# weimengmeng1999/AdapterSIS

Hardware: AMD Instinct MI355X
Metric: training images/sec, ViT-L/14 588^2 adapter fine-tune (higher is better)
Workload: dtype f16; 1 GPU; vit_large/14 frozen + CAViT/CACNN adapters (n_last_blocks=4) + FeatureDecoder, 588x588, batch 12/GPU, reference_exact train.py step (fwd + decoder bwd + all-reduce + SGD), random-init weights; global_batch=12, image_size=588, parallelism=dp1, split_precision_convs=True, split_attn_out=False, precise_level=0, fold_attn_scale=True, fused_qkv=False, dead_cacnn_elided=True, c1_elided=True, ln_fold=True, mx_conv=True, mx_dense=True, conv_halo=True, fuse_cls_up=False, skipped_optimizer_steps=0

## Files before the change

### adaptersis_amd/_lib.py

```python
from __future__ import annotations

import ctypes as C
import os

_HERE = os.path.dirname(os.path.abspath(__file__))
LIB_PATH = os.path.join(_HERE, "lib", "libasis_hip.so")

ASIS_F16, ASIS_BF16, ASIS_F32 = 0, 1, 2
ASIS_EINVAL, ASIS_ELAUNCH = -1, -2
ACT_NONE, ACT_GELU, ACT_RELU, ACT_SILU_MUL, ACT_GELU_GRAD = 0, 1, 2, 3, 4


class AsisError(RuntimeError):
    pass


class GemmDesc(C.Structure):
    _fields_ = [
        ("A", C.c_void_p), ("B", C.c_void_p), ("C", C.c_void_p),
        ("lda", C.c_int64), ("ldb", C.c_int64), ("ldc", C.c_int64),
        ("strideA", C.c_int64), ("strideB", C.c_int64), ("strideC", C.c_int64),
        ("batch", C.c_int32), ("M", C.c_int32), ("N", C.c_int32), ("K", C.c_int32),
        ("bias_n", C.c_void_p), ("bias_m", C.c_void_p), ("scale_n", C.c_void_p), ("res", C.c_void_p),
        ("ldr", C.c_int64), ("strideR", C.c_int64),
        ("act", C.c_int32), ("out_f32", C.c_int32), ("dtype", C.c_int32),
        ("conv", C.c_int32),
        ("B_", C.c_int32), ("H", C.c_int32), ("W", C.c_int32), ("Cin", C.c_int32), ("OH", C.c_int32),
        ("OW", C.c_int32), ("KH", C.c_int32), ("KW", C.c_int32), ("stride", C.c_int32), ("pad", C.c_int32),
        ("stats", C.c_void_p),
        ("A_lo", C.c_void_p), ("B_lo", C.c_void_p),
        ("aux", C.c_void_p), ("ld_aux", C.c_int64),
        ("ksplit", C.c_int32),
        ("mx_amax_a", C.c_void_p), ("mx_amax_b", C.c_void_p),
        ("C_lo", C.c_void_p), ("rowstats", C.c_void_p), ("res16", C.c_void_p), ("res16_lo", C.c_void_p), ("ldr16", C.c_int64),
        ("ln_mr", C.c_void_p), ("ln_cs", C.c_void_p), ("ln_cols", C.c_int32),
    ]


class WgradDesc(C.Structure):
    _fields_ = [
        ("dy", C.c_void_p), ("x", C.c_void_p), ("out", C.c_void_p),
        ("ld_dy", C.c_int64), ("P", C.c_int64),
        ("dtype", C.c_int32), ("Cout", C.c_int32), ("CoP", C.c_int32), ("Cin", C.c_int32),
        ("B_", C.c_int32), ("H", C.c_int32), ("W", C.c_int32), ("OH", C.c_int32), ("OW", C.c_int32),
        ("KH", C.c_int32), ("KW", C.c_int32), ("stride", C.c_int32), ("pad", C.c_int32),
        ("splits", C.c_int32), ("k_per_split", C.c_int64),
    ]


_lib = None


def lib() -> C.CDLL:
    global _lib
    if _lib is not None:
        return _lib
    if not os.path.exists(LIB_PATH):
        raise AsisError(
            f"{LIB_PATH} is missing: build it with `python -m adaptersis_amd.build` "
            "(hipcc --offload-arch=gfx950). adaptersis_amd has no fallback path.")
    _lib = C.CDLL(LIB_PATH)
    _lib.asis_last_error.restype = C.c_char_p
    _declare(_lib)
    return _lib


_vp, _i, _i64, _f, _d = C.c_void_p, C.c_int, C.c_int64, C.c_float, C.c_double
SIGNATURES = {
    "asis_version": [],
    "asis_device_count": [],
    "asis_gemm": [_vp, C.POINTER(GemmDesc)],
    "asis_gemm_tiles_m": [_i],
    "asis_absmax_f32": [_vp, _vp, _i64, _i, _i64, _vp, _i],
    "asis_bn_relu_absmax": [_vp, _vp, _vp, _vp, _i64, _i, _i, _vp],
    "asis_absmax_16": [_vp, _i, _vp, _i64, _i, _i64, _vp],
    "asis_conv3x3_halo_mx_tiles": [_i, _i, _i],
    "asis_conv3x3_halo_mx": [_vp, _i, _vp, _vp, _vp, _vp, _vp, _vp, _vp, _vp, _vp, _i, _i, _i, _i, _i],
    "asis_mx_from_pair": [_vp, _i, _vp, _vp, _i64, _vp, _i64, _i64, _i, _vp, _i],
    "asis_bn_relu_upsample_mx": [_vp, _i, _vp, _vp, _vp, _vp, _vp, _vp, _i, _i, _i, _i, _i],
    "asis_pack_conv_weight_mx": [_vp, _i, _vp, _vp, _i, _i, _i, _i, _i, _i64, _vp],
    "asis_pack_conv_weight_pair": [_vp, _i, _vp, _vp, _vp, _i, _i, _i, _i, _i, _i64, _vp],
    "asis_decoder_input_mx": [_vp, _i, _vp, _i64, _vp, _i64, _vp, _i64, _vp, _vp, _vp, _i, _i, _i, _i, _i, _i],
    "asis_ln_stats_finalize": [_vp, _vp, _i64, _i, _i, _f, _vp],
    "asis_split_stats": [_vp, _i, _vp, _i64, _vp, _vp, _i64, _vp, _i64, _i, _f],
    "asis_gemm_set_option": [C.c_char_p, _i],
    "asis_layernorm": [_vp, _i, _vp, _i64, _vp, _vp, _f, _vp, _i64, _i, _i64, _i],
    "asis_layernorm_mx": [_vp, _i, _vp, _i64, _vp, _vp, _f, _vp, _vp, _i64, _vp, _i64, _i],
    "asis_attention_fwd_seg": [_vp, _i, _vp, _vp, _i64, _vp, _i64, _vp, _i64, _i, _i, _i, _i, _i, _f, _vp],
    "asis_attention_fwd_split": [_vp, _i, _vp, _vp, _i64, _vp, _i64, _vp, _vp, _i64, _i, _i, _i, _i, _i, _f, _vp],
    "asis_attention_fwd_prescaled": [_vp, _i, _vp, _vp, _i64, _vp, _i64, _vp, _vp, _i64, _i, _i, _i, _i, _i, _vp],
    "asis_attention_fwd_qkv": [_vp, _i, _vp, _vp, _vp, _i64, _vp, _vp, _i64, _i, _i, _i, _i, _i, _f, _i, _vp],
    "asis_attention_fwd_qkv_mx": [_vp, _i, _vp, _vp, _vp, _i64, _vp, _vp, _i64, _i, _i, _i, _i, _i, _f, _i, _vp, _vp],
    "asis_attention_fwd_lse": [_vp, _i, _vp, _vp, _i64, _vp, _i64, _vp, _i64, _i, _i, _i, _f, _vp],
    "asis_transpose_tokens": [_vp, _i, _vp, _i64, _vp, _i64, _i, _i, _i],
    "asis_attention_bwd_rows": [_vp, _i, _vp, _vp, _vp, _i64, _vp, _i64, _vp, _i64, _vp, _vp, _vp, _vp, _vp, _i64, _i, _i, _i, _i,
                                _i, _f],
    "asis_msda_bwd": [_vp, _i, _vp, _vp, _i64, _vp, _vp, _vp, _vp, _vp, _vp, _i, _i, _i, _i, _i, _i, _i],
    "asis_msda_vgrad_cap": [_i, _i, _i],
    "asis_msda_value_grad": [_vp, _i, _vp, _i64, _vp, _vp, _vp, _vp, _vp, _vp, _vp, _vp, _vp, _i, _i, _i, _i, _i, _i, _i],
    "asis_msda_sampling_matrix": [_vp, _i, _vp, _i64, _vp, _vp, _vp, _vp, _i64, _i, _i, _i, _i, _i, _i],
    "asis_dwconv_bwd_nblk": [_i64],
    "asis_dwconv_gelu_bwd": [_vp, _i, _vp, _vp, _vp, _vp, _vp, _i, _vp, _vp, _vp, _vp, _i, _i, _i],
    "asis_rowblock_nblk": [_i64],
    "asis_layernorm_bwd": [_vp, _vp, _i64, _vp, _i64, _vp, _f, _vp, _i64, _vp, _i64, _vp, _i64, _i],
    "asis_gelu16": [_vp, _i, _vp, _vp, _vp, _i64],
    "asis_gelu_split": [_vp, _i, _vp, _vp, _vp, _i64],
    "asis_cast_colsum": [_vp, _i, _vp, _i64, _vp, _i64, _f, _vp, _i64, _i],
    "asis_swiglu_bwd": [_vp, _i, _vp, _vp, _vp, _i64, _i],
    "asis_colsum": [_vp, _i, _vp, _i64, _vp, _i64, _i],
    "asis_ls_linear_finish": [_vp, _vp, _vp, _vp, _vp, _vp, _f, _vp, _vp, _vp, _i, _i],
    "asis_attention_fwd": [_vp, _i, _vp, _vp, _i64, _vp, _i64, _vp, _i64, _i, _i, _i, _f],
    "asis_im2col_patch": [_vp, _i, _vp, _i, _i, _i, _i, _vp, _i64],
    "asis_im2col_patch_split": [_vp, _i, _vp, _i, _i, _i, _i, _vp, _vp, _i64],
    "asis_cast_pad": [_vp, _i, _vp, _i64, _vp, _i64, _i64, _i, _f, _i],
    "asis_add_cls_pos": [_vp, _vp, _vp, _vp, _vp, _i, _i, _i],
    "asis_msda_fwd": [_vp, _i, _vp, _vp, _i64, _vp, _vp, _vp, _vp, _i, _i, _i, _i, _i, _i, _i],
    "asis_msda_fwd_split": [_vp, _i, _vp, _vp, _i64, _vp, _vp, _vp, _vp, _vp, _i, _i, _i, _i, _i, _i, _i],
    "asis_dwconv_gelu": [_vp, _i, _vp, _vp, _vp, _vp, _vp, _i, _vp, _i, _i, _i],
    "asis_conv3x3_c3": [_vp, _vp, _vp, _vp, _i, _i, _i, _i, _i, _i],
    "asis_conv3x3_smallcout_fwd": [_vp, _i, _vp, _vp, _vp, _vp, _vp, _i, _i, _i, _i, _i],
    "asis_conv3x3_smallcout_fwd_up": [_vp, _i, _vp, _vp, _vp, _vp, _vp, _vp, _i, _i, _i, _i, _i],
    "asis_conv3x3_smallcout_wgrad_up": [_vp, _i, _vp, _i, _vp, _vp, _vp, _vp, _i, _i, _i, _i, _i, _i],
    "asis_conv3x3_smallcout_dgrad": [_vp, _i, _vp, _vp, _i, _vp, _vp, _i, _i, _i, _i, _i],
    "asis_conv3x3_smallcout_wgrad": [_vp, _i, _vp, _i, _vp, _vp, _i, _i, _i, _i, _i, _i],
    "asis_colstats_nparts": [_i64],
    "asis_colstats": [_vp, _vp, _i64, _i, _vp],
    "asis_reduce_partials": [_vp, _vp, _i, _i, _vp],
    "asis_bn_finalize": [_vp, _vp, _d, _i, _vp, _vp, _f, _f, _vp, _vp, _vp, _vp, _vp, _vp, _vp],
    "asis_bn_eval_affine": [_vp, _vp, _vp, _vp, _vp, _f, _i, _vp, _vp],
    "asis_bn_act": [_vp, _i, _vp, _vp, _vp, _i, _vp, _vp, _i64, _i],
    "asis_bn_act_mx": [_vp, _i, _vp, _vp, _vp, _i, _vp, _vp, _vp, _i64, _i],
    "asis_bn_relu_maxpool": [_vp, _i, _vp, _vp, _vp, _vp, _vp, _i, _i, _i, _i],
    "asis_bn_relu_upsample": [_vp, _i, _vp, _vp, _vp, _vp, _vp, _i, _i, _i, _i, _i],
    "asis_pack_conv_weight": [_vp, _i, _vp, _vp, _i, _i, _i, _i, _i, _i64, _i],
    "asis_decoder_input": [_vp, _i, _vp, _i64, _vp, _i64, _vp, _i64, _vp, _vp, _i, _i, _i, _i, _i, _i],
    "asis_swiglu": [_vp, _i, _vp, _vp, _i64, _i],
    "asis_swiglu_split": [_vp, _i, _vp, _vp, _vp, _i64, _i],
    "asis_copy_channels": [_vp, _vp, _i64, _vp, _i64, _i64, _i64],
    "asis_add_f32": [_vp, _vp, _vp, _vp, _i64, _i, _i64, _i64, _i64],
    "asis_maxpool2_fwd": [_vp, _i, _vp, _vp, _vp, _vp, _vp, _i, _i, _i, _i],
    "asis_maxpool2_bwd": [_vp, _vp, _vp, _vp, _i, _i, _i, _i],
    "asis_cls_l2norm": [_vp, _vp, _vp, _vp, _i, _i, _i, _i],
    "asis_cls_l2norm_bwd": [_vp, _vp, _vp, _vp, _vp, _i, _i, _i, _i],
    "asis_mask_logits_fwd": [_vp, _vp, _vp, _vp, _vp, _f, _vp, _vp, _vp, _i, _i, _i, _i],
    "asis_mask_logits_nblk": [_i, _i],
    "asis_mask_logits_bwd": [_vp, _vp, _vp, _vp, _vp, _vp, _vp, _f, _vp, _vp, _vp, _i, _i, _i, _i],
    "asis_mask_dchat": [_vp, _vp, _vp, _vp, _vp, _i, _i, _i, _i],
    "asis_nearest_add_relu": [_vp, _i, _vp, _vp, _vp, _vp, _vp, _vp, _i, _i, _i, _i, _i, _i],
    "asis_nearest_sum": [_vp, _vp, _vp, _vp, _vp, _i, _i, _i, _i, _i, _i],
    "asis_convt2x2_scatter": [_vp, _i, _vp, _vp, _vp, _i, _i, _i, _i, _i, _i, _i, _i, _i, _i],
    "asis_convt2x2_gather": [_vp, _i, _vp, _vp, _vp, _i, _i, _i, _i, _i, _i, _i, _i, _i, _i],
    "asis_convt2x2_bias_nblk": [_i64],
    "asis_conv1x1_dgrad_small": [_vp, _i, _vp, _vp, _i64, _vp, _vp, _i64, _i, _i],
    "asis_convt2x2_bias_grad": [_vp, _vp, _vp, _i, _i, _i, _i, _i, _i, _i, _i, _i, _i],
    "asis_dice_nblk": [_i, _i],
    "asis_seg_loss_fwd": [_vp, _vp, _vp, _vp, _i, _i, _i, _i, _i, _i, _i, _i, _f, _i, _f, _vp, _vp, _vp, _vp],
    "asis_seg_loss_bwd": [_vp, _vp, _vp, _vp, _vp, _i, _i, _i, _i, _i, _i, _i, _i, _i, _vp],
    "asis_dice_fwd": [_vp, _vp, _vp, _i, _i, _i, _i, _i, _i, _i, _f, _i, _f, _vp, _vp, _vp, _vp],
    "asis_dice_bwd": [_vp, _vp, _vp, _vp, _i, _i, _i, _i, _i, _i, _i, _vp],
    "asis_ce_acc_nblk": [_i64],
    "asis_ce_acc_counts": [_vp, _vp, _vp, _vp, _i, _i, _i, _i, _i, _i, _vp, _vp],
    "asis_ce_acc": [_vp, _vp, _vp, _vp, _i, _i, _i, _i, _i, _i, _vp],
    "asis_resize_bilinear_fwd": [_vp, _vp, _i, _i, _i, _i, _i, _i, _vp],
    "asis_resize_bwd_nblk": [_i64],
    "asis_resize_bilinear_bwd": [_vp, _i, _vp, _i, _i, _i, _i, _i, _i, _i, _vp, _vp, _vp],
    "asis_reduce_rows": [_vp, _vp, _i, _i, _f, _vp],
    "asis_ew_blocks": [_i64],
    "asis_bn_bwd_nblk": [_i64, _i],
    "asis_maxpool_bn_relu_bwd": [_vp, _vp, _vp, _vp, _vp, _vp, _vp, _vp, _vp, _i, _i, _i, _i],
    "asis_dilate2": [_vp, _i, _vp, _vp, _vp, _vp, _i, _i, _i, _i, _i, _i],
    "asis_upsample_bn_relu_bwd": [_vp, _vp, _vp, _vp, _vp, _vp, _vp, _vp, _vp, _i, _i, _i, _i, _i],
    "asis_bn_bwd_apply": [_vp, _i, _vp, _vp, _vp, _vp, _vp, _vp, _vp, _d, _vp, _vp, _vp, _i64, _i],
    "asis_bn_bwd_apply_mx": [_vp, _i, _vp, _vp, _vp, _vp, _vp, _vp, _vp, _d, _vp, _vp, _vp, _vp, _i64, _i],
    "asis_bn_bwd_absmax": [_vp, _vp, _vp, _vp, _vp, _vp, _vp, _vp, _d, _vp, _i64, _i],
    "asis_wgrad_splits": [_i64, _i, _i],
    "asis_wgrad": [_vp, C.POINTER(WgradDesc)],
    "asis_conv3x3_wgrad_halo_nblk": [_i, _i, _i, _i, _i],
    "asis_conv3x3_wgrad_halo": [_vp, _i, _vp, _i64, _vp, _vp, _i, _i, _i, _i, _i, _i],
    "asis_sgd_momentum": [_vp, _vp, _vp, _vp, _i64, _f, _f, _f, _f, _i],
    "asis_augment": [_vp] * 13 + [_i, _i],
    "asis_augment_geo_u8": [_vp] * 12 + [_i, _i],
    "asis_clahe": [_vp] * 13 + [_i, _i, _i],
    "asis_frame_resize": [_vp] * 5 + [_i, _vp, _vp, _i] + [_vp] * 6 + [_i] * 5,
    "asis_predict_mask": [_vp, _vp] + [_i] * 6 + [_vp] * 9,
    "asis_surface_stats": [_vp] * 5 + [_i] * 6 + [_vp, _i] + [_vp] * 6 + [_i],
    "asis_dropout_f32": [_vp, _vp, _vp, _vp, _i64, C.c_uint64, _i, _f, _f, _vp, _i],
    "asis_dropout_t16": [_vp, _i, _vp, _vp, _i64, C.c_uint64, _i, _f, _i],
    "asis_dropout_mask": [_vp, _vp, _i64, C.c_uint64, _i, _f],
    "asis_softmax_dropout_fwd": [_vp, _i, _vp, _vp, _vp, _i64, _i, _i, _f, C.c_uint64, _i, _f],
    "asis_softmax_dropout_bwd": [_vp, _i, _vp, _vp, _vp, _vp, _i64, _i, _i, _f, C.c_uint64, _i, _f],
    "asis_grad_guard": [_vp, _vp, _i64, _vp, _i],
    "asis_sgd_momentum_guarded": [_vp, _vp, _vp, _vp, _i64, _f, _f, _f, _f, _i, _vp, _i],
    "asis_scale_f32": [_vp, _vp, _i64, _f],
    "asis_zero": [_vp, _vp, _i64],
    "asis_grad_pack_bf16": [_vp, _vp, _i64, _vp],
    "asis_grad_unpack_bf16": [_vp, _vp, _i64, _vp],
}


def _declare(l: C.CDLL) -> None:
    for name, argtypes in SIGNATURES.items():
        fn = getattr(l, name)
        fn.argtypes = argtypes
        fn.restype = C.c_int


def check(rc: int, what: str = "") -> None:
    if rc == 0:
        return
    msg = lib().asis_last_error().decode(errors="replace")
    if rc == -1:
        raise ValueError(f"{what}: {msg}" if what else msg)
    raise AsisError(f"{what}: {msg}" if what else msg)
```

### adaptersis_amd/config.py

```python
import os

import torch

operand_dtype = torch.bfloat16 if os.environ.get("ASIS_OPERAND", "f16").lower() in ("bf16", "bfloat16") else torch.float16
loss_scale = float(os.environ.get("ASIS_LOSS_SCALE", 65536.0 if operand_dtype == torch.float16 else 1.0))


def set_operand_dtype(dt: torch.dtype) -> None:
    global operand_dtype
    if dt not in (torch.float16, torch.bfloat16):
        raise ValueError("operand dtype must be float16 or bfloat16")
    operand_dtype = dt

split_conv = os.environ.get("ASIS_SPLIT_CONV", "1") != "0"

precise_attention = os.environ.get("ASIS_PRECISE", "0") not in ("0", "")
fold_attn_scale = os.environ.get("ASIS_FOLD_SCALE", "1") not in ("0", "")
fused_qkv = os.environ.get("ASIS_FUSED_QKV", "0") not in ("0", "")

encoder_stream = os.environ.get("ASIS_ENC_STREAM", "1") not in ("0", "")

vt_stream = os.environ.get("ASIS_VT_STREAM", "1") not in ("0", "")

wgrad_stream = os.environ.get("ASIS_WGRAD_STREAM", "1") not in ("0", "")

unsplit_layers = set(filter(None, os.environ.get("ASIS_UNSPLIT", "").split(",")))

dual_stream = os.environ.get("ASIS_DUAL_STREAM", "1") not in ("0", "")

attn_rows = os.environ.get("ASIS_ATTN_ROWS", "1") != "0"

_so = os.environ.get("ASIS_SPLIT_O", "auto").lower()
split_attn_out_policy = None if _so == "auto" else (_so not in ("0", ""))
split_attn_out = bool(split_attn_out_policy)

_pl = os.environ.get("ASIS_PRECISE_LEVEL", "auto").lower() or "auto"
precise_level_policy = None if _pl == "auto" else int(_pl)
precise_level = int(precise_level_policy or 0)
_pa = os.environ.get("ASIS_PRECISE_ADAPTERS", "auto").lower() or "auto"


def precise_adapters_on() -> bool:
    if _pa != "auto":
        return _pa not in ("0", "")
    return operand_dtype == torch.bfloat16 and precise_level >= 2


_pp = os.environ.get("ASIS_PRECISE_PARTS", "auto").lower() or "auto"
precise_parts_policy = None if _pp == "auto" else frozenset(filter(None, _pp.replace("w12", "fc1").replace("w3", "fc2").split(",")))
precise_parts = precise_parts_policy if precise_parts_policy is not None else frozenset(("qkv", "proj", "fc1", "fc2"))
trunk_streams = int(os.environ.get("ASIS_TRUNK_STREAMS", "2") or 2)

elide_dead_cacnn = os.environ.get("ASIS_ELIDE_DEAD_CACNN", "1") not in ("0", "")
elide_c1 = os.environ.get("ASIS_ELIDE_C1", "1") not in ("0", "")
share_patch_embed = os.environ.get("ASIS_SHARE_PATCH_EMBED", "1") not in ("0", "")

ln_fold = os.environ.get("ASIS_LN_FOLD", "1") not in ("0", "")

_mx = os.environ.get("ASIS_MX_CONV", "1")
mx_conv_all = _mx == "2"
mx_conv = _mx not in ("0", "")


def mx_conv_on() -> bool:
    return mx_conv and (mx_conv_all or operand_dtype == torch.float16)


mx_dense = os.environ.get("ASIS_MX_DENSE", "1") not in ("0", "")


def mx_dense_on() -> bool:
    return mx_dense and operand_dtype == torch.float16
```

### adaptersis_amd/csrc/gemm.hip

```cpp
#include <stdlib.h>

#include "asis_common.h"

namespace {

constexpr int BM = 128, BN = 128, BK = 64, NTHREADS = 256;

template <typename T, bool CONV>
__global__ __launch_bounds__(NTHREADS, 2) void gemm_kernel(const asis_gemm_desc d) {
  typedef typename T16<T>::v8 v8;
  __shared__ __attribute__((aligned(16))) T lds[2 * (BM + BN) * BK];

  const int tid = threadIdx.x;
  const int lane = tid & 63;
  const int wid = tid >> 6;
  const int wr = wid >> 1, wc = wid & 1;

  const int tiles_n = (d.N + BN - 1) / BN;
  const int bid = xcd_remap(blockIdx.x, gridDim.x);
  const int tile_m = bid / tiles_n;
  const int tile_n = bid - tile_m * tiles_n;
  const int m0 = tile_m * BM, n0 = tile_n * BN;
  const int bz = blockIdx.y;

  const T* __restrict__ A = reinterpret_cast<const T*>(d.A) + (int64_t)bz * d.strideA;
  const T* __restrict__ B = reinterpret_cast<const T*>(d.B) + (int64_t)bz * d.strideB;

  const int lrow = tid >> 3;
  const int lchk = tid & 7;
  int64_t a_off[4];
  int a_ih0[4], a_iw0[4];
  bool a_ok[4], b_ok[4];
  int64_t b_off[4];
#pragma unroll
  for (int i = 0; i < 4; ++i) {
    const int m = m0 + lrow + 32 * i;
    a_ok[i] = m < d.M;
    if (CONV) {
      const int mm = a_ok[i] ? m : 0;
      const int ohw = d.OH * d.OW;
      const int b = mm / ohw;
      const int rem = mm - b * ohw;
      const int oh = rem / d.OW;
      const int ow = rem - oh * d.OW;
      a_ih0[i] = oh * d.stride - d.pad;
      a_iw0[i] = ow * d.stride - d.pad;
      a_off[i] = (int64_t)b * d.H * d.W;
    } else {
      a_off[i] = (int64_t)m * d.lda;
      a_ih0[i] = a_iw0[i] = 0;
    }
    const int n = n0 + lrow + 32 * i;
    b_ok[i] = n < d.N;
    b_off[i] = (int64_t)n * d.ldb;
  }

  uint4 ra[4], rb[4];
  auto load_tile = [&](int k0) {
    const int kk = k0 + lchk * 8;
    const bool kok = kk < d.K;
    int kh = 0, kw = 0, ci = kk;
    if (CONV) {
      const int tap = kk / d.Cin;
      ci = kk - tap * d.Cin;
      kh = tap / d.KW;
      kw = tap - kh * d.KW;
    }
#pragma unroll
    for (int i = 0; i < 4; ++i) {
      uint4 v = make_uint4(0, 0, 0, 0);
      if (CONV) {
        const int ih = a_ih0[i] + kh, iw = a_iw0[i] + kw;
        if (a_ok[i] && kok && (unsigned)ih < (unsigned)d.H && (unsigned)iw < (unsigned)d.W)
          v = *reinterpret_cast<const uint4*>(A + (a_off[i] + (int64_t)ih * d.W + iw) * d.Cin + ci);
      } else {
        if (a_ok[i] && kok) v = *reinterpret_cast<const uint4*>(A + a_off[i] + kk);
      }
      ra[i] = v;
      uint4 w = make_uint4(0, 0, 0, 0);
      if (b_ok[i] && kok) w = *reinterpret_cast<const uint4*>(B + b_off[i] + kk);
      rb[i] = w;
    }
  };
  auto store_tile = [&](int buf) {
    T* As = lds + buf * ((BM + BN) * BK);
    T* Bs = As + BM * BK;
#pragma unroll
    for (int i = 0; i < 4; ++i) {
      const int row = lrow + 32 * i;
      const int sw = (lchk ^ ((row >> 1) & 7)) << 3;
      *reinterpret_cast<uint4*>(As + row * BK + sw) = ra[i];
      *reinterpret_cast<uint4*>(Bs + row * BK + sw) = rb[i];
    }
  };

  f32x16 acc[2][2];
#pragma unroll
  for (int i = 0; i < 2; ++i)
#pragma unroll
    for (int j = 0; j < 2; ++j)
#pragma unroll
      for (int r = 0; r < 16; ++r) acc[i][j][r] = 0.f;

  const int nt = (d.K + BK - 1) / BK;
  load_tile(0);
  store_tile(0);
  __syncthreads();

  const int fr = lane & 31, fh = lane >> 5;
  for (int t = 0; t < nt; ++t) {
    const int buf = t & 1;
    if (t + 1 < nt) load_tile((t + 1) * BK);
    const T* As = lds + buf * ((BM + BN) * BK);
    const T* Bs = As + BM * BK;
#pragma unroll
    for (int ks = 0; ks < 4; ++ks) {
      v8 af[2], bf[2];
      const int chunk = 2 * ks + fh;
#pragma unroll
      for (int i = 0; i < 2; ++i) {
        const int row = wr * 64 + i * 32 + fr;
        af[i] = __builtin_bit_cast(v8, *reinterpret_cast<const uint4*>(As + row * BK + ((chunk ^ ((row >> 1) & 7)) << 3)));
        const int col = wc * 64 + i * 32 + fr;
        bf[i] = __builtin_bit_cast(v8, *reinterpret_cast<const uint4*>(Bs + col * BK + ((chunk ^ ((col >> 1) & 7)) << 3)));
      }
#pragma unroll
      for (int i = 0; i < 2; ++i)
#pragma unroll
        for (int j = 0; j < 2; ++j) acc[i][j] = T16<T>::mfma32(af[i], bf[j], acc[i][j]);
    }
    if (t + 1 < nt) store_tile(buf ^ 1);
    __syncthreads();
  }

  const int64_t cbase = (int64_t)bz * d.strideC;
  const float* __restrict__ res = d.res ? d.res + (int64_t)bz * d.strideR : nullptr;
  float csum[2] = {0.f, 0.f}, csq[2] = {0.f, 0.f};
#pragma unroll
  for (int j = 0; j < 2; ++j) {
    const int col = n0 + wc * 64 + j * 32 + fr;
    const bool cok = col < d.N;
    const float bn = (d.bias_n && cok) ? d.bias_n[col] : 0.f;
    const float sc = (d.scale_n && cok) ? d.scale_n[col] : 1.f;
#pragma unroll
    for (int i = 0; i < 2; ++i) {
#pragma unroll
      for (int r = 0; r < 16; ++r) {
        const int row = m0 + wr * 64 + i * 32 + (r & 3) + 8 * (r >> 2) + 4 * fh;
        if (row < d.M && cok) {
          float v = acc[i][j][r] + bn;
          if (d.bias_m) v += d.bias_m[row];
          if (d.act == ASIS_ACT_GELU) v = gelu_erf(v);
          else if (d.act == ASIS_ACT_RELU) v = fmaxf(v, 0.f);
          v *= sc;
          if (res) v += res[(int64_t)row * d.ldr + col];
          if (d.out_f32) reinterpret_cast<float*>(d.C)[cbase + (int64_t)row * d.ldc + col] = v;
          else reinterpret_cast<T*>(d.C)[cbase + (int64_t)row * d.ldc + col] = to_t16<T>(v);
          csum[j] += v;
          csq[j] += v * v;
        }
      }
    }
  }
  if (d.stats) {
    float* red = reinterpret_cast<float*>(lds);
#pragma unroll
    for (int j = 0; j < 2; ++j) {
      float s = csum[j] + __shfl_xor(csum[j], 32, 64);
      float q = csq[j] + __shfl_xor(csq[j], 32, 64);
      if (fh == 0) {
        red[(wr * 2 + 0) * BN + wc * 64 + j * 32 + fr] = s;
        red[(wr * 2 + 1) * BN + wc * 64 + j * 32 + fr] = q;
      }
    }
    __syncthreads();
    if (tid < BN) {
      const int col = n0 + tid;
      if (col < d.N) {
        d.stats[((int64_t)tile_m * 2 + 0) * d.N + col] = red[0 * BN + tid] + red[2 * BN + tid];
        d.stats[((int64_t)tile_m * 2 + 1) * d.N + col] = red[1 * BN + tid] + red[3 * BN + tid];
      }
    }
  }
}

#include "gemm_big.h"
#include "gemm_p8.h"

static int g_gemm_p8 = -1;
static bool ph8_m16_on() { static const int v = [] { const char* e = getenv("ASIS_GEMM_8P_M16"); return e ? atoi(e) : 1; }(); return v != 0; }

template <typename T>
int launch(hipStream_t s, const asis_gemm_desc& d) {
  static const int group_m = [] { const char* e = getenv("ASIS_GEMM_GROUPM"); return e && atoi(e) > 0 ? atoi(e) : 4; }();
  static const int big_mode = [] { const char* e = getenv("ASIS_GEMM_BIG"); return e ? atoi(e) : 1; }();
  const bool vec_ok = (d.N % 4 == 0) && (d.ldc % 4 == 0);
  const bool split = d.A_lo != nullptr || d.B_lo != nullptr;
  if (d.act == ASIS_ACT_GELU_GRAD) {
    const bool ok = big_mode && !d.conv && !split && !d.stats && d.aux && d.K % 32 == 0 && d.M >= 256 && d.N >= 128 && vec_ok &&
                    d.ld_aux % 4 == 0 && d.batch == 1 && (reinterpret_cast<uintptr_t>(d.aux) & 7) == 0 &&
                    (reinterpret_cast<uintptr_t>(d.C) & 15) == 0 && !d.bias_m;
    if (!ok) return ASIS_EINVAL;
  }
  if (d.act == ASIS_ACT_SILU_MUL) {
    auto al16 = [](const void* p) { return (reinterpret_cast<uintptr_t>(p) & 15) == 0; };
    const bool mxs = d.mx_amax_a && d.mx_amax_b && d.A_lo && d.B_lo;
    const bool ok = big_mode && ph8_m16_on() && !d.conv && (mxs || !split) && !d.out_f32 && !d.res && !d.res16 && !d.C_lo && !d.rowstats &&
                    !d.stats && !d.scale_n && !d.bias_m && !d.ln_mr && !d.aux && d.batch == 1 && d.ksplit <= 1 && d.K % 64 == 0 && d.M >= 256 &&
                    d.N >= 256 && d.N % 32 == 0 && d.ldc % 8 == 0 && d.ldc >= d.N / 2 && al16(d.C) && (!d.bias_n || al16(d.bias_n)) &&
                    (int64_t)d.N * d.ldb < (1ll << 31);
    if (!ok) return ASIS_EINVAL;
    dim3 g8(((d.M + 255) / 256) * ((d.N + 255) / 256), 1), block(512);
    if (mxs) hipLaunchKernelGGL((gemm_big_kernel<T, 2, 4, 4, 2, 2, 0, false, true, 64, 1, true, true, 0, true>), g8, block, 0, s, d, group_m);
    else hipLaunchKernelGGL((gemm_big_kernel<T, 2, 4, 4, 2, 2, 0, false, false, 64, 1, true, true>), g8, block, 0, s, d, group_m);
    return 0;
  }
  if (d.ksplit > 1 && !(big_mode && d.conv)) return ASIS_EINVAL;
  {
    if (g_gemm_p8 < 0) { const char* e = getenv("ASIS_GEMM_P8"); g_gemm_p8 = e ? atoi(e) : 1; }
    const int p8 = g_gemm_p8;
    const int64_t p8_tiles = (int64_t)((d.M + 255) / 256) * ((d.N + 255) / 256);
    const int kparts = 1 + (d.A_lo ? 1 : 0) + (d.B_lo ? 1 : 0);
    auto al = [](const void* p, int a) { return (reinterpret_cast<uintptr_t>(p) & (a - 1)) == 0; };
    if (p8 && big_mode && ph8_m16_on() && !d.conv && !d.stats && d.batch == 1 && !d.bias_m && !d.ln_cols && !d.C_lo && !d.rowstats && !d.res16 &&
        !d.mx_amax_a && !d.mx_amax_b &&
        d.ksplit <= 1 && d.K % 64 == 0 &&
        d.M >= 256 && d.N >= 256 && p8_tiles >= (p8 == 2 ? 16 : 256) && d.K >= 128 && (p8 >= 2 || d.K * kparts <= 2048) &&
        (int64_t)d.M * d.lda * 2 < (1ll << 32) && (int64_t)d.N * d.ldb * 2 < (1ll << 32) && d.N % 8 == 0 && d.ldc % 8 == 0 &&
        al(d.C, 16) && (!d.res || (al(d.res, 16) && d.ldr % 4 == 0)) && (!d.bias_n || al(d.bias_n, 16)) && (!d.scale_n || al(d.scale_n, 16)) &&
        (d.act != ASIS_ACT_GELU_GRAD || (d.aux && al(d.aux, 8) && d.ld_aux % 4 == 0))) {
      const int nwg = p8_tiles >= 256 ? 256 : (int)(p8_tiles / 8) * 8;
      if (d.ln_mr) hipLaunchKernelGGL((gemm_p8_kernel<T, 1>), dim3(nwg), dim3(512), 0, s, d, group_m);
      else hipLaunchKernelGGL((gemm_p8_kernel<T, 0>), dim3(nwg), dim3(512), 0, s, d, group_m);
      return 0;
    }
  }
  const bool lnx = d.C_lo || d.rowstats || d.res16 || d.ln_mr;
  if (lnx) {
    static const int ph8x = [] { const char* e = getenv("ASIS_GEMM_8P"); return e ? atoi(e) : 1; }();
    const bool ph8_ok = ph8x && ph8_m16_on() && big_mode && !split && !d.conv && !d.stats && d.K % 64 == 0 && d.M >= 256 && d.N >= 256 &&
                        (ph8x == 2 || d.K >= 2048 || (ph8x == 1 && d.K >= 1024 && (int64_t)((d.M + 255) / 256) * ((d.N + 255) / 256) * d.batch >= 128)) &&
                        d.N % 8 == 0 && d.ldc % 8 == 0 && (!d.res16 || (d.res16_lo && d.ldr16 % 8 == 0 && d.ldr16 >= d.N && asis_aligned16(d.res16) && asis_aligned16(d.res16_lo))) &&
                        (!d.C_lo || !d.out_f32) && (!d.ln_mr || d.ln_cs) &&
                        (!(d.C_lo || d.rowstats || d.res16) ||
                         ((!d.res || (d.ldr % 8 == 0 && asis_aligned16(d.res))) && (!d.C_lo || asis_aligned16(d.C_lo)) && asis_aligned16(d.C) &&
                          (!d.bias_n || asis_aligned16(d.bias_n)) && (!d.scale_n || asis_aligned16(d.scale_n)) && d.batch == 1 && !d.bias_m &&
                          d.act == ASIS_ACT_NONE && !d.ln_mr));
    if (!ph8_ok) return ASIS_EINVAL;
  }
  if (split) {
    const bool ok = big_mode && d.K % BK == 0 && d.M >= 256 && d.N >= 32 && vec_ok && (d.out_f32 || !d.conv) &&
                    (!d.conv || (d.Cin % BK == 0 && d.A_lo && d.B_lo));
    if (!ok) return ASIS_EINVAL;
    const int bm = 256, bn = d.N > 64 ? 128 : 64;
    if (d.ksplit > 1 && (d.batch != 1 || d.stats || (d.KH * d.KW) % d.ksplit != 0 || !d.out_f32 || d.res)) return ASIS_EINVAL;
    dim3 grid(((d.M + bm - 1) / bm) * ((d.N + bn - 1) / bn), d.ksplit > 1 ? d.ksplit : d.batch), block(512);
    if (d.mx_amax_a || d.mx_amax_b) {
      if (!(d.mx_amax_a && d.mx_amax_b && d.A_lo && d.B_lo)) return ASIS_EINVAL;
      if (!d.conv) {
        if (!(d.K % 64 == 0 && d.N >= 256 && d.batch == 1 && d.ksplit <= 1 && !d.stats && (int64_t)d.N * d.ldb < (1ll << 31))) return ASIS_EINVAL;
        dim3 g8(((d.M + 255) / 256) * ((d.N + 255) / 256), 1);
        hipLaunchKernelGGL((gemm_big_kernel<T, 2, 4, 4, 2, 2, 0, false, true, 64, 1, true, true, 0, true>), g8, block, 0, s, d, group_m);
        return 0;
      }
      if ((int64_t)d.B_ * d.H * d.W * d.Cin >= (1ll << 31) || (int64_t)d.N * d.ldb >= (1ll << 31) || d.H >= 65536 || d.W >= 65536) return ASIS_EINVAL;
      static const int mx_ph8 = [] { const char* e = getenv("ASIS_MX_PH8"); return e ? atoi(e) : 1; }();
      if (mx_ph8 && d.N >= 256 && (d.N % 256 == 0 || d.N >= 1024) && d.batch == 1) {
        dim3 g8(((d.M + 255) / 256) * ((d.N + 255) / 256), d.ksplit > 1 ? d.ksplit : 1);
        hipLaunchKernelGGL((gemm_big_kernel<T, 2, 4, 4, 2, 2, 0, true, true, 64, 1, true, true, 0, true>), g8, block, 0, s, d, group_m);
      } else if (bn == 64 && d.ksplit <= 1 && d.M >= 512) {
        dim3 g512(((d.M + 511) / 512) * ((d.N + 63) / 64), 1);
        hipLaunchKernelGGL((gemm_big_kernel<T, 8, 1, 2, 2, 2, 0, true, true, 64, 1, false, true, 0, true>), g512, block, 0, s, d, group_m);
      } else if (bn == 128) {
        hipLaunchKernelGGL((gemm_big_kernel<T, 4, 2, 2, 2, 3, 0, true, true, 64, 1, false, true, 0, true>), grid, block, 0, s, d, group_m);
      } else {
        hipLaunchKernelGGL((gemm_big_kernel<T, 8, 1, 1, 2, 3, 0, true, true, 64, 1, false, true, 0, true>), grid, block, 0, s, d, group_m);
      }
      return 0;
    }
    static const int conv32 = [] { const char* e = getenv("ASIS_CONV_BK32"); return e ? atoi(e) : 0; }();
    static const int t512 = [] { const char* e = getenv("ASIS_CONV_T512"); return e ? atoi(e) : 1; }();
    static const int cm16 = [] { const char* e = getenv("ASIS_CONV_M16"); return e ? atoi(e) : 0; }();
    static const int conv8p = [] { const char* e = getenv("ASIS_CONV_8P"); return e ? atoi(e) : 1; }();
    if (d.conv && conv8p && d.N >= 256 && (d.N % 256 == 0 || d.N >= 1024) && d.batch == 1) {
      dim3 g8(((d.M + 255) / 256) * ((d.N + 255) / 256), d.ksplit > 1 ? d.ksplit : 1);
      hipLaunchKernelGGL((gemm_big_kernel<T, 2, 4, 4, 2, 2, 0, true, true, 64, 1, true, true>), g8, block, 0, s, d, group_m);
      return 0;
    }
    if (d.conv && bn == 64 && t512 && d.ksplit <= 1 && d.M >= 512) {
      dim3 g512(((d.M + 511) / 512) * ((d.N + 63) / 64), 1);
      if (cm16) hipLaunchKernelGGL((gemm_big_kernel<T, 8, 1, 2, 2, 2, 0, true, true, 64, 1, false, true>), g512, block, 0, s, d, group_m);
      else hipLaunchKernelGGL((gemm_big_kernel<T, 8, 1, 2, 2, 2, 0, true, true, 64, 1>), g512, block, 0, s, d, group_m);
      return 0;
    }
    if (d.conv) {
      if (conv32 && bn == 128) hipLaunchKernelGGL((gemm_big_kernel<T, 4, 2, 2, 2, 3, 0, true, true, 32, 4>), grid, block, 0, s, d, group_m);
      else if (bn == 128 && cm16) hipLaunchKernelGGL((gemm_big_kernel<T, 4, 2, 2, 2, 3, 0, true, true, 64, 2, false, true>), grid, block, 0, s, d, group_m);
      else if (bn == 128) hipLaunchKernelGGL((gemm_big_kernel<T, 4, 2, 2, 2, 3, 0, true, true>), grid, block, 0, s, d, group_m);
      else hipLaunchKernelGGL((gemm_big_kernel<T, 8, 1, 1, 2, 3, 0, true, true>), grid, block, 0, s, d, group_m);
    } else {
      if (bn == 128) hipLaunchKernelGGL((gemm_big_kernel<T, 4, 2, 2, 2, 3, 0, false, true>), grid, block, 0, s, d, group_m);
      else hipLaunchKernelGGL((gemm_big_kernel<T, 8, 1, 1, 2, 3, 0, false, true>), grid, block, 0, s, d, group_m);
    }
    return 0;
  }
  static const int m16 = [] { const char* e = getenv("ASIS_GEMM_M16"); return e ? atoi(e) : 1; }();
  static const int ph8 = [] { const char* e = getenv("ASIS_GEMM_8P"); return e ? atoi(e) : 1; }();
  static const int ph8_mink = [] { const char* e = getenv("ASIS_GEMM_8P_MINK"); return e ? atoi(e) : 1024; }();
  if (ph8 && (ph8 == 2 || d.K >= 2048 || (ph8 == 1 && d.K >= ph8_mink && (int64_t)((d.M + 255) / 256) * ((d.N + 255) / 256) * d.batch >= 128)) && big_mode && !d.conv && !d.stats && d.K % 64 == 0 && d.M >= 256 && d.N >= 256) {
    dim3 grid(((d.M + 255) / 256) * ((d.N + 255) / 256), d.batch), block(512);
    static const int ph8_m16 = [] { const char* e = getenv("ASIS_GEMM_8P_M16"); return e ? atoi(e) : 1; }();
    static const int ph8_slab32 = [] { const char* e = getenv("ASIS_GEMM_8P_SLAB32"); return e ? atoi(e) : 0; }();
    const int group_m_f = group_m | (ph8_slab32 ? 0x10000 : 0);
    if (ph8_m16) {
      if (lnx) hipLaunchKernelGGL((gemm_big_kernel<T, 2, 4, 4, 2, 2, 0, false, false, 64, 1, true, true, 1>), grid, block, 0, s, d, group_m);
      else hipLaunchKernelGGL((gemm_big_kernel<T, 2, 4, 4, 2, 2, 0, false, false, 64, 1, true, true>), grid, block, 0, s, d, group_m_f);
      return 0;
    }
    hipLaunchKernelGGL((gemm_big_kernel<T, 2, 4, 4, 2, 2, 0, false, false, 64, 1, true>), grid, block, 0, s, d, group_m);
    return 0;
  }
  if (big_mode && !d.conv && !d.stats && d.K % 32 == 0 && d.M >= 256 && d.N >= 128) {
    const int bm = 256, bn = (big_mode == 2 && d.N >= 2048) ? 256 : 128;
    dim3 grid(((d.M + bm - 1) / bm) * ((d.N + bn - 1) / bn), d.batch), block(512);
    if (big_mode == 2 && bn == 256) hipLaunchKernelGGL((gemm_big_kernel<T, 2, 4, 4, 2, 2>), grid, block, 0, s, d, group_m);
    else if (big_mode >= 2) hipLaunchKernelGGL((gemm_big_kernel<T, 4, 2, 2, 2, 3>), grid, block, 0, s, d, group_m);
    else if (m16) hipLaunchKernelGGL((gemm_big_kernel<T, 4, 2, 2, 2, 3, 0, false, false, 32, 4, false, true>), grid, block, 0, s, d, group_m);
    else hipLaunchKernelGGL((gemm_big_kernel<T, 4, 2, 2, 2, 3, 0, false, false, 32, 4>), grid, block, 0, s, d, group_m);
    return 0;
  }
  if (big_mode && d.conv && d.Cin % BK == 0 && d.M >= 256 && d.N >= 32 && vec_ok && d.out_f32) {
    const int bm = 256, bn = d.N > 64 ? 128 : 64;
    if (d.ksplit > 1 && (d.stats || (d.KH * d.KW) % d.ksplit != 0 || d.res)) return ASIS_EINVAL;
    dim3 grid(((d.M + bm - 1) / bm) * ((d.N + bn - 1) / bn), d.ksplit > 1 ? d.ksplit : 1), block(512);
    static const int conv8p = [] { const char* e = getenv("ASIS_CONV_8P"); return e ? atoi(e) : 1; }();
    if (conv8p && d.N >= 256 && (d.N % 256 == 0 || d.N >= 1024) && d.batch == 1) {
      dim3 g8(((d.M + 255) / 256) * ((d.N + 255) / 256), d.ksplit > 1 ? d.ksplit : 1);
      hipLaunchKernelGGL((gemm_big_kernel<T, 2, 4, 4, 2, 2, 0, true, false, 64, 1, true, true>), g8, block, 0, s, d, group_m);
      return 0;
    }
    if (bn == 128) hipLaunchKernelGGL((gemm_big_kernel<T, 4, 2, 2, 2, 3, 0, true>), grid, block, 0, s, d, group_m);
    else hipLaunchKernelGGL((gemm_big_kernel<T, 8, 1, 1, 2, 3, 0, true>), grid, block, 0, s, d, group_m);
    return 0;
  }
  if (d.ksplit > 1) return ASIS_EINVAL;
  const int tiles_m = (d.M + BM - 1) / BM, tiles_n = (d.N + BN - 1) / BN;
  dim3 grid(tiles_m * tiles_n, d.batch), block(NTHREADS);
  if (d.conv)
    hipLaunchKernelGGL((gemm_kernel<T, true>), grid, block, 0, s, d);
  else
    hipLaunchKernelGGL((gemm_kernel<T, false>), grid, block, 0, s, d);
  return 0;
}

}

extern "C" int asis_gemm_tiles_m(int M) { return (M + BM - 1) / BM; }

extern "C" int asis_gemm_set_option(const char* name, int value) {
  ASIS_REQUIRE(name != nullptr, "asis_gemm_set_option: null name");
  if (strcmp(name, "p8") == 0) { g_gemm_p8 = value; return ASIS_OK; }
  ASIS_FAIL(ASIS_EINVAL, "asis_gemm_set_option: unknown option '%s'", name);
}


extern "C" int asis_gemm(void* stream, const asis_gemm_desc* dp) {
  ASIS_REQUIRE(dp != nullptr, "asis_gemm: null descriptor");
  asis_gemm_desc d = *dp;
  ASIS_REQUIRE(d.A && d.B && d.C, "asis_gemm: null operand pointer");
  ASIS_REQUIRE(d.M > 0 && d.N > 0 && d.K > 0, "asis_gemm: M,N,K must be positive (got %d,%d,%d)", d.M, d.N, d.K);
  ASIS_DT_OK(d.dtype, "asis_gemm");
  ASIS_REQUIRE(d.K % 8 == 0, "asis_gemm: K=%d must be a multiple of 8", d.K);
  ASIS_REQUIRE(d.ldb % 8 == 0 && d.ldb >= d.K, "asis_gemm: ldb=%ld must be a multiple of 8 and >= K", (long)d.ldb);
  ASIS_REQUIRE(asis_aligned16(d.A) && asis_aligned16(d.B), "asis_gemm: A and B must be 16-byte aligned");
  ASIS_REQUIRE(d.strideA % 8 == 0 && d.strideB % 8 == 0, "asis_gemm: batch strides must be multiples of 8");
  ASIS_REQUIRE(d.ldc >= (d.act == ASIS_ACT_SILU_MUL ? d.N / 2 : d.N), "asis_gemm: ldc=%ld < N=%d", (long)d.ldc, d.N);
  ASIS_REQUIRE(d.act >= 0 && d.act <= ASIS_ACT_GELU_GRAD, "asis_gemm: bad act %d", d.act);
  if (d.batch <= 0) d.batch = 1;
  ASIS_REQUIRE(d.batch <= 65535, "asis_gemm: batch %d too large", d.batch);
  if (d.res) ASIS_REQUIRE(d.ldr >= d.N, "asis_gemm: ldr=%ld < N", (long)d.ldr);
  if (d.conv) {
    ASIS_REQUIRE(d.batch == 1, "asis_gemm: conv mode needs batch == 1 (batch is folded into M)");
    ASIS_REQUIRE(d.Cin % 8 == 0 && d.Cin > 0, "asis_gemm: conv Cin=%d must be a multiple of 8", d.Cin);
    ASIS_REQUIRE(d.KH > 0 && d.KW > 0 && d.stride > 0 && d.pad >= 0, "asis_gemm: bad conv geometry");
    ASIS_REQUIRE(d.K == d.KH * d.KW * d.Cin, "asis_gemm: conv K=%d != KH*KW*Cin=%d", d.K, d.KH * d.KW * d.Cin);
    ASIS_REQUIRE(d.OH == (d.H + 2 * d.pad - d.KH) / d.stride + 1 && d.OW == (d.W + 2 * d.pad - d.KW) / d.stride + 1,
                 "asis_gemm: conv output size mismatch");
    ASIS_REQUIRE((int64_t)d.B_ * d.OH * d.OW == d.M, "asis_gemm: conv M=%d != B*OH*OW", d.M);
  } else {
    ASIS_REQUIRE(d.lda % 8 == 0 && d.lda >= d.K, "asis_gemm: lda=%ld must be a multiple of 8 and >= K", (long)d.lda);
  }
  if (d.stats) ASIS_REQUIRE(d.batch == 1, "asis_gemm: stats need batch == 1");
  if (d.res16) ASIS_REQUIRE(d.res16_lo && !d.res && d.ldr16 % 4 == 0 && d.ldr16 >= d.N && (reinterpret_cast<uintptr_t>(d.res16) & 7) == 0 &&
                            (reinterpret_cast<uintptr_t>(d.res16_lo) & 7) == 0, "asis_gemm: res16 needs res16_lo, no fp32 res, ldr16 %% 4 == 0, 8-byte aligned planes");
  if (d.C_lo) ASIS_REQUIRE(!d.out_f32 && (reinterpret_cast<uintptr_t>(d.C_lo) & 7) == 0, "asis_gemm: C_lo is the second plane of a 16-bit output");
  if (d.ln_mr) ASIS_REQUIRE(d.ln_cs && (reinterpret_cast<uintptr_t>(d.ln_mr) & 7) == 0 && asis_aligned16(d.ln_cs), "asis_gemm: ln_mr needs ln_cs (16-byte aligned)");
  if (d.rowstats) ASIS_REQUIRE(d.batch == 1 && (reinterpret_cast<uintptr_t>(d.rowstats) & 7) == 0, "asis_gemm: rowstats need batch == 1");
  if (d.rowstats) ASIS_REQUIRE(d.N % 64 == 0, "asis_gemm: rowstats need N %% 64 == 0 (N = %d)", (int)d.N);
  const int64_t tiles = (int64_t)asis_cdiv(d.M, BM) * asis_cdiv(d.N, BN);
  ASIS_REQUIRE(tiles < (1ll << 31), "asis_gemm: too many tiles");
  hipStream_t s = reinterpret_cast<hipStream_t>(stream);
  ASIS_REQUIRE(!d.conv || (d.A_lo == nullptr) == (d.B_lo == nullptr), "asis_gemm: a split convolution needs both A_lo and B_lo");
  ASIS_REQUIRE((!d.A_lo || asis_aligned16(d.A_lo)) && (!d.B_lo || asis_aligned16(d.B_lo)), "asis_gemm: split halves must be 16-byte aligned");
  int rc = 0;
  if (int bad = asis_dispatch16(d.dtype, "asis_gemm", [&](auto t) { rc = launch<decltype(t)>(s, d); })) return bad;
  if (rc != 0 && d.act == ASIS_ACT_SILU_MUL)
    ASIS_FAIL(ASIS_EINVAL, "asis_gemm: ASIS_ACT_SILU_MUL needs a dense 16-bit-output launch on the 8-phase form (include/asis_hip.h: K %% 64 == 0, "
                           "M >= 256, N >= 256, N %% 32 == 0, ldc %% 8 == 0, plain or MX split operands, bias only)");
  if (rc != 0) ASIS_FAIL(ASIS_EINVAL, "asis_gemm: split-precision operands / ASIS_ACT_GELU_GRAD / ksplit need the large-tile path (K %% 64 "
                                        "== 0 (GELU_GRAD: 32), M >= 256, N >= 32 (128), N and ldc multiples of 4, fp32 output for "
                                        "split; conv: Cin %% 64 == 0)");
  ASIS_CHECK_LAUNCH("asis_gemm");
  return ASIS_OK;
}
```

### adaptersis_amd/csrc/gemm_big.h

```cpp
#pragma once
#include <type_traits>

#include "asis_common.h"

namespace {
__device__ __attribute__((aligned(16))) uint4 g_zero_page[1];

template <typename T, int WM, int WN, int TM, int TN, int NS, int DBG = 0, bool CONV = false, bool SPLIT = false, int BKT = 64,
          int OCC = 2, bool PH8 = false, bool M16 = false, int LNF = 0, bool MXC = false>
__global__ __launch_bounds__(WM * WN * 64, OCC) void gemm_big_kernel(const asis_gemm_desc d, const int GROUP_M_FLAGS) {
  const int GROUP_M = GROUP_M_FLAGS & 0xffff;
  static_assert(!PH8 || (WM == 2 && WN == 4 && TM == 4 && TN == 2 && NS == 2 && BKT == 64),
                "the 8-phase main loop is written for the 256x256x64 tile, 2x4 waves of 128x64");
  static_assert(!MXC || (SPLIT && M16 && BKT == 64 && (CONV || PH8)), "the MX correction pass is built for split operands on 16x16 MFMAs");
  typedef int v4i_ __attribute__((ext_vector_type(4)));
  typedef int v8i_ __attribute__((ext_vector_type(8)));
  auto cat8 = [](auto lo8, auto hi8) -> v8i_ {
    return __builtin_shufflevector(__builtin_bit_cast(v4i_, lo8), __builtin_bit_cast(v4i_, hi8), 0, 1, 2, 3, 4, 5, 6, 7);
  };
  const int mx_sc = MXC ? mx_code<T>(*d.mx_amax_a, *d.mx_amax_b) : 0;
  auto mfma_mx = [](f32x4& acc, v8i_ a, v8i_ b, int sa, int sb) {
    asm volatile("v_mfma_scale_f32_16x16x128_f8f6f4 %0, %1, %2, %0, %3, %4 op_sel_hi:[0,0,0]" : "+v"(acc) : "v"(a), "v"(b), "v"(sa), "v"(sb));
  };
  const int mx_one = 127;
  typedef typename T16<T>::v8 v8;
  constexpr int BM2 = WM * TM * 32, BN2 = WN * TN * 32;
  constexpr int BKB = BKT;
  constexpr int CPR = BKB / 8;
  constexpr int RPI = 64 / CPR;
  constexpr int SWS = (CPR == 8) ? 1 : 2;
  constexpr int STAGE = (BM2 + BN2) * BKB;
  constexpr int NWV = WM * WN;
  constexpr int GA = BM2 / RPI / NWV, GB = BN2 / RPI / NWV;
  constexpr int G = GA + GB;
  __shared__ __attribute__((aligned(16))) T lds[NS * STAGE];

  const int tid = threadIdx.x, lane = tid & 63;
  const int wid = __builtin_amdgcn_readfirstlane(tid >> 6);
  const int wm = wid / WN, wn = wid - wm * WN;
  uint64_t dbg_c0 = 0, dbg_r0 = 0;
  if (DBG & 4) asm volatile("s_memtime %0\n\ts_memrealtime %1\n\ts_waitcnt lgkmcnt(0)" : "=s"(dbg_c0), "=s"(dbg_r0)::"memory");
  const int tiles_n = (d.N + BN2 - 1) / BN2;
  const int bid = xcd_remap(blockIdx.x, gridDim.x);
  const int tiles_m = (d.M + BM2 - 1) / BM2;
  const int band = bid / (GROUP_M * tiles_n);
  const int first_m = band * GROUP_M;
  const int band_m = (tiles_m - first_m) < GROUP_M ? (tiles_m - first_m) : GROUP_M;
  const int in_band = bid - band * GROUP_M * tiles_n;
  const int tile_n = in_band / band_m;
  const int tile_m = first_m + (in_band - tile_n * band_m);
  const int m0 = tile_m * BM2, n0 = tile_n * BN2;
  const int bz = blockIdx.y;
  const T* __restrict__ A = reinterpret_cast<const T*>(d.A) + (int64_t)bz * d.strideA;
  const T* __restrict__ B = reinterpret_cast<const T*>(d.B) + (int64_t)bz * d.strideB;

  const T* asrc[GA];
  const T* bsrc[GB];
  int a_ih0[GA], a_iw0[GA];
  uint32_t a_pix[GA], a_hw[GA], b_off[GB];
  const int lr = lane / CPR, lc = lane % CPR;
  auto swz = [&](int row) -> int { return (M16 && CPR == 4) ? ((-(row >> 2)) & 3) : ((row >> SWS) & (CPR - 1)); };
  auto grp_a = [&](int j) -> int {
    if (PH8) { const int g = wid * 2 + (j & 1); return (g < 8 ? 0 : 128) + (j >> 1) * 64 + (g & 7) * 8; }
    return (wid * GA + j) * RPI;
  };
  auto grp_b = [&](int j) -> int {
    if (PH8) { const int g = wid * 2 + (j & 1); return (g >> 2) * 64 + (j >> 1) * 32 + (g & 3) * 8; }
    return (wid * GB + j) * RPI;
  };
#pragma unroll
  for (int j = 0; j < GA; ++j) {
    const int row = grp_a(j) + lr;
    int gr = m0 + row;
    gr = gr < d.M ? gr : d.M - 1;
    if (CONV) {
      const int ohw = d.OH * d.OW;
      const int b = gr / ohw;
      const int rem = gr - b * ohw;
      const int oh = rem / d.OW, ow = rem - oh * d.OW;
      a_ih0[j] = oh * d.stride - d.pad;
      a_iw0[j] = ow * d.stride - d.pad;
      asrc[j] = A + (int64_t)b * d.H * d.W * d.Cin + ((lc ^ swz(row)) << 3);
      a_pix[j] = (uint32_t)(b * d.H * d.W * d.Cin + ((lc ^ swz(row)) << 3));
      a_hw[j] = ((uint32_t)(oh * d.stride) << 16) | (uint32_t)(ow * d.stride);
    } else {
      a_ih0[j] = a_iw0[j] = 0;
      asrc[j] = A + (int64_t)gr * d.lda + ((lc ^ swz(row)) << 3);
    }
  }
#pragma unroll
  for (int j = 0; j < GB; ++j) {
    const int row = grp_b(j) + lr;
    int gr = n0 + row;
    gr = gr < d.N ? gr : d.N - 1;
    bsrc[j] = B + (int64_t)gr * d.ldb + ((lc ^ swz(row)) << 3);
    b_off[j] = (uint32_t)(gr * (int)d.ldb + ((lc ^ swz(row)) << 3));
  }
  const int64_t a_lo_off = (SPLIT && d.A_lo) ? (reinterpret_cast<const T*>(d.A_lo) - reinterpret_cast<const T*>(d.A)) : 0;
  const int64_t b_lo_off = (SPLIT && d.B_lo) ? (reinterpret_cast<const T*>(d.B_lo) - reinterpret_cast<const T*>(d.B)) : 0;
  const int nparts = !SPLIT ? 1 : (MXC ? 2 : (CONV ? 3 : ((d.A_lo && d.B_lo) ? 3 : 2)));
  auto part_offs = [&](int part, int64_t& aoff, int64_t& boff) {
    aoff = (part == 1 && d.A_lo) ? a_lo_off : 0;
    boff = ((part == 2) || (part == 1 && !d.A_lo)) ? b_lo_off : 0;
  };
  const int ksp = d.ksplit > 1 ? d.ksplit : 1;
  const int nt1 = d.K / ksp / BKB;
  const int kt_base = ksp > 1 ? bz * nt1 : 0;
  const int ntap_part = CONV ? (d.KH * d.KW) / ksp : 1;
  const int tap_base = (CONV && ksp > 1) ? bz * ntap_part : 0;
  typedef __attribute__((address_space(3))) void* lds_ptr;
  typedef const __attribute__((address_space(1))) void* glb_ptr;
  auto issue = [&](int t) {
    T* st = lds + (t % NS) * STAGE;
    int kt = t;
    int64_t aoff = 0, boff = 0;
    int k0;
    if (CONV) {
      int tt = t, part = 0;
      if (SPLIT && MXC) {
        tt = t >> 1;
        part = t & 1;
        aoff = part ? a_lo_off : 0;
        boff = part ? b_lo_off : 0;
      } else if (SPLIT) {
        tt = t / 3;
        part = t - 3 * tt;
        aoff = part == 1 ? a_lo_off : 0;
        boff = part == 2 ? b_lo_off : 0;
      }
      const int c = tt / ntap_part, tl = tt - c * ntap_part;
      k0 = (tap_base + tl) * d.Cin + c * BKB;
    } else {
      if (SPLIT && MXC) {
        kt = t >> 1;
        aoff = (t & 1) ? a_lo_off : 0;
        boff = (t & 1) ? b_lo_off : 0;
      } else if (SPLIT) {
        const int part = t / nt1;
        kt = t - part * nt1;
        part_offs(part, aoff, boff);
      }
      k0 = (kt + kt_base) * BKB;
    }
    if (CONV) {
      const int tap = k0 / d.Cin, ci0 = k0 - tap * d.Cin;
      const int kh = tap / d.KW, kw = tap - kh * d.KW;
#pragma unroll
      for (int j = 0; j < GA; ++j) {
        const T* src;
        if constexpr (MXC) {
          const int ih = (int)(a_hw[j] >> 16) - d.pad + kh, iw = (int)(a_hw[j] & 0xffffu) - d.pad + kw;
          src = ((unsigned)ih < (unsigned)d.H && (unsigned)iw < (unsigned)d.W)
                    ? A + aoff + (a_pix[j] + (uint32_t)((ih * d.W + iw) * d.Cin + ci0))
                    : reinterpret_cast<const T*>(g_zero_page);
        } else {
          const int ih = a_ih0[j] + kh, iw = a_iw0[j] + kw;
          src = ((unsigned)ih < (unsigned)d.H && (unsigned)iw < (unsigned)d.W)
                    ? asrc[j] + aoff + ((int64_t)ih * d.W + iw) * d.Cin + ci0
                    : reinterpret_cast<const T*>(g_zero_page);
        }
        __builtin_amdgcn_global_load_lds((glb_ptr)src, (lds_ptr)(st + grp_a(j) * BKB), 16, 0, 0);
      }
    } else {
#pragma unroll
      for (int j = 0; j < GA; ++j)
        __builtin_amdgcn_global_load_lds((glb_ptr)(asrc[j] + aoff + k0), (lds_ptr)(st + grp_a(j) * BKB), 16, 0, 0);
    }
#pragma unroll
    for (int j = 0; j < GB; ++j) {
      const T* src = MXC ? B + boff + (b_off[j] + (uint32_t)k0) : bsrc[j] + boff + k0;
      __builtin_amdgcn_global_load_lds((glb_ptr)src, (lds_ptr)(st + BM2 * BKB + grp_b(j) * BKB), 16, 0, 0);
    }
  };

  f32x16 acc[M16 ? 1 : TM][M16 ? 1 : TN];
  f32x4 acc16[M16 ? TM * 2 : 1][M16 ? TN * 2 : 1];
  if constexpr (M16) {
#pragma unroll
    for (int i = 0; i < TM * 2; ++i)
#pragma unroll
      for (int j = 0; j < TN * 2; ++j) acc16[i][j] = f32x4{0.f, 0.f, 0.f, 0.f};
  } else {
#pragma unroll
  for (int i = 0; i < TM; ++i)
#pragma unroll
    for (int j = 0; j < TN; ++j)
#pragma unroll
      for (int r = 0; r < 16; ++r) acc[i][j][r] = 0.f;
  }

  const int nt = nparts * nt1;
  const int fr = lane & 31, fh = lane >> 5;
  if constexpr (PH8) {
    int sk0 = kt_base * BKB, s_part = 0, s_kt = 0;
    int64_t s_aoff = 0, s_boff = 0;
    int s_tl = 0, s_c = 0;
    const int kh0 = CONV ? tap_base / d.KW : 0, kw0 = CONV ? tap_base - kh0 * d.KW : 0;
    int s_kh = kh0, s_kw = kw0;
    if (CONV) sk0 = tap_base * d.Cin;
    auto advance_src = [&]() {
      if (CONV) {
        if (SPLIT && MXC) {
          ++s_part;
          s_aoff = s_part == 1 ? a_lo_off : 0;
          s_boff = s_part == 1 ? b_lo_off : 0;
          if (s_part < 2) return;
          s_part = 0;
        } else if (SPLIT) {
          ++s_part;
          s_aoff = s_part == 1 ? a_lo_off : 0;
          s_boff = s_part == 2 ? b_lo_off : 0;
          if (s_part < 3) return;
          s_part = 0;
          s_aoff = s_boff = 0;
        }
        if (++s_tl == ntap_part) {
          s_tl = 0; ++s_c; s_kh = kh0; s_kw = kw0;
        } else if (++s_kw == d.KW) {
          s_kw = 0; ++s_kh;
        }
        sk0 = (tap_base + s_tl) * d.Cin + s_c * BKB;
      } else if constexpr (MXC) {
        ++s_part;
        s_aoff = s_part == 1 ? a_lo_off : 0;
        s_boff = s_part == 1 ? b_lo_off : 0;
        if (s_part < 2) return;
        s_part = 0;
        ++s_kt;
        sk0 = (s_kt + kt_base) * BKB;
      } else {
        if (++s_kt == nt1) {
          s_kt = 0; ++s_part;
          part_offs(s_part, s_aoff, s_boff);
        }
        sk0 = (s_kt + kt_base) * BKB;
      }
    };
    auto dma_a = [&](int t, int j) {
      const T* src;
      if constexpr (CONV && MXC) {
        const int ih = (int)(a_hw[j] >> 16) - d.pad + s_kh, iw = (int)(a_hw[j] & 0xffffu) - d.pad + s_kw;
        src = ((unsigned)ih < (unsigned)d.H && (unsigned)iw < (unsigned)d.W)
                  ? A + s_aoff + (a_pix[j] + (uint32_t)((ih * d.W + iw) * d.Cin + s_c * BKB))
                  : reinterpret_cast<const T*>(g_zero_page);
      } else if (CONV) {
        const int ih = a_ih0[j] + s_kh, iw = a_iw0[j] + s_kw;
        src = ((unsigned)ih < (unsigned)d.H && (unsigned)iw < (unsigned)d.W)
                  ? asrc[j] + s_aoff + ((int64_t)ih * d.W + iw) * d.Cin + s_c * BKB
                  : reinterpret_cast<const T*>(g_zero_page);
      } else {
        src = asrc[j] + s_aoff + sk0;
      }
      __builtin_amdgcn_global_load_lds((glb_ptr)src, (lds_ptr)(lds + (t & 1) * STAGE + grp_a(j) * BKB), 16, 0, 0);
    };
    auto dma_b = [&](int t, int j) {
      const T* src = MXC ? B + s_boff + (b_off[j] + (uint32_t)sk0) : bsrc[j] + s_boff + sk0;
      __builtin_amdgcn_global_load_lds((glb_ptr)src, (lds_ptr)(lds + (t & 1) * STAGE + BM2 * BKB + grp_b(j) * BKB), 16, 0, 0);
    };
#pragma unroll
    for (int j = 0; j < 4; ++j) {
      dma_a(0, j);
      dma_b(0, j);
    }
    advance_src();
    asm volatile("s_waitcnt vmcnt(0)" ::: "memory");
    __builtin_amdgcn_s_barrier();
    if (wm == 1) __builtin_amdgcn_s_barrier();
    v8 af[2][4], b0f[4], b1f[4];
    const int r16 = lane & 15, q16 = lane >> 4;
    auto rd_a = [&](const T* As, int rh) {
      if constexpr (M16) {
#pragma unroll
        for (int t4 = 0; t4 < 4; ++t4) {
          const int row = (wm * TM + rh * 2) * 32 + t4 * 16 + r16;
#pragma unroll
          for (int ks = 0; ks < 2; ++ks)
            af[t4 >> 1][(t4 & 1) * 2 + ks] =
                __builtin_bit_cast(v8, *reinterpret_cast<const uint4*>(As + row * BKB + (((4 * ks + q16) ^ ((row >> 1) & 7)) << 3)));
        }
      } else {
#pragma unroll
      for (int i = 0; i < 2; ++i) {
        const int row = (wm * TM + rh * 2 + i) * 32 + fr;
#pragma unroll
        for (int ks = 0; ks < 4; ++ks)
          af[i][ks] = __builtin_bit_cast(v8, *reinterpret_cast<const uint4*>(As + row * BKB + (((2 * ks + fh) ^ ((row >> 1) & 7)) << 3)));
      }
      }
    };
    auto rd_b = [&](const T* Bs, int ch, v8* bf) {
      if constexpr (M16) {
#pragma unroll
        for (int jj = 0; jj < 2; ++jj) {
          const int col = (wn * TN + ch) * 32 + jj * 16 + r16;
#pragma unroll
          for (int ks = 0; ks < 2; ++ks)
            bf[jj * 2 + ks] = __builtin_bit_cast(v8, *reinterpret_cast<const uint4*>(Bs + col * BKB + (((4 * ks + q16) ^ ((col >> 1) & 7)) << 3)));
        }
      } else {
      const int col = (wn * TN + ch) * 32 + fr;
#pragma unroll
      for (int ks = 0; ks < 4; ++ks)
        bf[ks] = __builtin_bit_cast(v8, *reinterpret_cast<const uint4*>(Bs + col * BKB + (((2 * ks + fh) ^ ((col >> 1) & 7)) << 3)));
      }
    };
    auto mma = [&](int rh, int ch, const v8* bf) {
      asm volatile("s_waitcnt lgkmcnt(0)" ::: "memory");
      __builtin_amdgcn_s_setprio(1);
      if constexpr (M16) {
#pragma unroll
        for (int ks = 0; ks < 2; ++ks)
#pragma unroll
          for (int t4 = 0; t4 < 4; ++t4)
#pragma unroll
            for (int jj = 0; jj < 2; ++jj)
              acc16[rh * 4 + t4][ch * 2 + jj] = T16<T>::mfma16(bf[jj * 2 + ks], af[t4 >> 1][(t4 & 1) * 2 + ks], acc16[rh * 4 + t4][ch * 2 + jj]);
      } else {
#pragma unroll
      for (int ks = 0; ks < 4; ++ks)
#pragma unroll
        for (int i = 0; i < 2; ++i) acc[rh * 2 + i][ch] = T16<T>::mfma32(bf[ks], af[i][ks], acc[rh * 2 + i][ch]);
      }
      __builtin_amdgcn_s_setprio(0);
    };
    v8i_ af8[4], b0f8[2], b1f8[2];
    auto rd_a8 = [&](const T* As, int rh) {
#pragma unroll
      for (int t4 = 0; t4 < 4; ++t4) {
        const int row = (wm * TM + rh * 2) * 32 + t4 * 16 + r16;
        af8[t4] = cat8(*reinterpret_cast<const v4i_*>(As + row * BKB + (((q16) ^ ((row >> 1) & 7)) << 3)),
                       *reinterpret_cast<const v4i_*>(As + row * BKB + (((4 + q16) ^ ((row >> 1) & 7)) << 3)));
      }
    };
    auto rd_b8 = [&](const T* Bs, int ch, v8i_* bf8) {
#pragma unroll
      for (int jj = 0; jj < 2; ++jj) {
        const int col = (wn * TN + ch) * 32 + jj * 16 + r16;
        bf8[jj] = cat8(*reinterpret_cast<const v4i_*>(Bs + col * BKB + (((q16) ^ ((col >> 1) & 7)) << 3)),
                       *reinterpret_cast<const v4i_*>(Bs + col * BKB + (((4 + q16) ^ ((col >> 1) & 7)) << 3)));
      }
    };
    auto half8 = [](v8i_ x, int ks) -> v8 {
      return ks ? __builtin_bit_cast(v8, __builtin_shufflevector(x, x, 4, 5, 6, 7)) : __builtin_bit_cast(v8, __builtin_shufflevector(x, x, 0, 1, 2, 3));
    };
    auto mma8 = [&](int rh, int ch, const v8i_* bf8, auto mx_tag) {
      asm volatile("s_waitcnt lgkmcnt(0)" ::: "memory");
      __builtin_amdgcn_sched_barrier(0);
      __builtin_amdgcn_s_setprio(1);
      if constexpr (decltype(mx_tag)::value) {
#pragma unroll
        for (int t4 = 0; t4 < 4; ++t4)
#pragma unroll
          for (int jj = 0; jj < 2; ++jj) mfma_mx(acc16[rh * 4 + t4][ch * 2 + jj], bf8[jj], af8[t4], mx_sc, mx_one);
      } else {
#pragma unroll
        for (int ks = 0; ks < 2; ++ks)
#pragma unroll
          for (int t4 = 0; t4 < 4; ++t4)
#pragma unroll
            for (int jj = 0; jj < 2; ++jj)
              acc16[rh * 4 + t4][ch * 2 + jj] = T16<T>::mfma16(half8(bf8[jj], ks), half8(af8[t4], ks), acc16[rh * 4 + t4][ch * 2 + jj]);
      }
      __builtin_amdgcn_s_setprio(0);
    };
    auto RA = [&](const T* As, int rh) { if constexpr (MXC) rd_a8(As, rh); else rd_a(As, rh); };
    auto RB = [&](const T* Bs, int ch, int which) {
      if constexpr (MXC) rd_b8(Bs, ch, which ? b1f8 : b0f8); else rd_b(Bs, ch, which ? b1f : b0f);
    };
    auto ktile = [&](int t, auto mx_tag) {
      auto MM = [&](int rh, int ch, int which) {
        if constexpr (MXC) mma8(rh, ch, which ? b1f8 : b0f8, mx_tag); else mma(rh, ch, which ? b1f : b0f);
      };
      const T* As = lds + (t & 1) * STAGE;
      const T* Bs = As + BM2 * BKB;
      const bool more = t + 1 < nt;
      RA(As, 0);
      RB(Bs, 0, 0);
      if (more) { dma_a(t + 1, 0); dma_a(t + 1, 1); asm volatile("s_waitcnt vmcnt(4)" ::: "memory"); }
      else asm volatile("s_waitcnt vmcnt(2)" ::: "memory");
      __builtin_amdgcn_s_barrier();
      MM(0, 0, 0);
      __builtin_amdgcn_s_barrier();
      RB(Bs, 1, 1);
      if (more) { dma_b(t + 1, 0); dma_b(t + 1, 1); asm volatile("s_waitcnt vmcnt(4)" ::: "memory"); }
      else asm volatile("s_waitcnt vmcnt(0)" ::: "memory");
      __builtin_amdgcn_s_barrier();
      MM(0, 1, 1);
      __builtin_amdgcn_s_barrier();
      RA(As, 1);
      if (more) { dma_b(t + 1, 2); dma_b(t + 1, 3); }
      __builtin_amdgcn_s_barrier();
      MM(1, 1, 1);
      __builtin_amdgcn_s_barrier();
      if (more) { dma_a(t + 1, 2); dma_a(t + 1, 3); asm volatile("s_waitcnt vmcnt(4)" ::: "memory"); }
      advance_src();
      __builtin_amdgcn_s_barrier();
      MM(1, 0, 0);
      __builtin_amdgcn_s_barrier();
    };
    if constexpr (MXC) {
      for (int t = 0; t < nt; t += 2) {
        ktile(t, std::false_type{});
        ktile(t + 1, std::true_type{});
      }
    } else {
      for (int t = 0; t < nt; ++t) ktile(t, std::false_type{});
    }
    if (wm == 0) __builtin_amdgcn_s_barrier();
  } else {
#pragma unroll
  for (int s = 0; s < NS - 1; ++s)
    if (s < nt) issue(s);

  for (int t = 0; t < nt; ++t) {
    if (nt - t - 1 >= NS - 2) asm volatile("s_waitcnt vmcnt(%0)" ::"n"((NS - 2) * G) : "memory");
    else asm volatile("s_waitcnt vmcnt(0)" ::: "memory");
    __builtin_amdgcn_s_barrier();
    if (!(DBG & 1) && t + NS - 1 < nt) issue(t + NS - 1);
    const T* As = lds + (t % NS) * STAGE;
    const T* Bs = As + BM2 * BKB;
    if (MXC && (t & 1)) {
      if constexpr (MXC) {
        const int r16 = lane & 15, q16 = lane >> 4;
        v8 af0[TM * 2], af1[TM * 2], bf0[TN * 2], bf1[TN * 2];
#pragma unroll
        for (int i = 0; i < TM * 2; ++i) {
          const int row = (wm * TM * 2 + i) * 16 + r16;
          af0[i] = __builtin_bit_cast(v8, *reinterpret_cast<const uint4*>(As + row * BKB + (((q16) ^ swz(row)) << 3)));
          af1[i] = __builtin_bit_cast(v8, *reinterpret_cast<const uint4*>(As + row * BKB + (((4 + q16) ^ swz(row)) << 3)));
        }
#pragma unroll
        for (int j = 0; j < TN * 2; ++j) {
          const int col = (wn * TN * 2 + j) * 16 + r16;
          bf0[j] = __builtin_bit_cast(v8, *reinterpret_cast<const uint4*>(Bs + col * BKB + (((q16) ^ swz(col)) << 3)));
          bf1[j] = __builtin_bit_cast(v8, *reinterpret_cast<const uint4*>(Bs + col * BKB + (((4 + q16) ^ swz(col)) << 3)));
        }
        asm volatile("s_waitcnt lgkmcnt(0)" ::: "memory");
        __builtin_amdgcn_sched_barrier(0);
#pragma unroll
        for (int i = 0; i < TM * 2; ++i)
#pragma unroll
          for (int j = 0; j < TN * 2; ++j)
            mfma_mx(acc16[i][j], cat8(bf0[j], bf1[j]), cat8(af0[i], af1[i]), mx_sc, mx_one);
      }
    } else if constexpr (M16) {
      const int r16 = lane & 15, q16 = lane >> 4;
#pragma unroll
      for (int ks = 0; ks < BKB / 32; ++ks) {
        v8 af[TM * 2], bf[TN * 2];
#pragma unroll
        for (int i = 0; i < TM * 2; ++i) {
          const int row = (wm * TM * 2 + i) * 16 + r16;
          af[i] = __builtin_bit_cast(v8, *reinterpret_cast<const uint4*>(As + row * BKB + (((4 * ks + q16) ^ swz(row)) << 3)));
        }
#pragma unroll
        for (int j = 0; j < TN * 2; ++j) {
          const int col = (wn * TN * 2 + j) * 16 + r16;
          bf[j] = __builtin_bit_cast(v8, *reinterpret_cast<const uint4*>(Bs + col * BKB + (((4 * ks + q16) ^ swz(col)) << 3)));
        }
#pragma unroll
        for (int i = 0; i < TM * 2; ++i)
#pragma unroll
          for (int j = 0; j < TN * 2; ++j) acc16[i][j] = T16<T>::mfma16(bf[j], af[i], acc16[i][j]);
      }
    } else if (!(DBG & 2)) {
      v8 af[2][TM], bf[2][TN];
      auto fetch = [&](int ks, int slot) {
        const int chunk = 2 * ks + fh;
#pragma unroll
        for (int i = 0; i < TM; ++i) {
          const int row = (wm * TM + i) * 32 + fr;
          af[slot][i] = __builtin_bit_cast(v8, *reinterpret_cast<const uint4*>(As + row * BKB + ((chunk ^ ((row >> SWS) & (CPR - 1))) << 3)));
        }
#pragma unroll
        for (int j = 0; j < TN; ++j) {
          const int col = (wn * TN + j) * 32 + fr;
          bf[slot][j] = __builtin_bit_cast(v8, *reinterpret_cast<const uint4*>(Bs + col * BKB + ((chunk ^ ((col >> SWS) & (CPR - 1))) << 3)));
        }
      };
      constexpr int KS = BKB / 16;
      fetch(0, 0);
#pragma unroll
      for (int ks = 0; ks < KS; ++ks) {
        if (ks < KS - 1) fetch(ks + 1, (ks + 1) & 1);
#pragma unroll
        for (int i = 0; i < TM; ++i)
#pragma unroll
          for (int j = 0; j < TN; ++j)
            acc[i][j] = T16<T>::mfma32(bf[ks & 1][j], af[ks & 1][i], acc[i][j]);
      }
    }
  }
  }

  if (DBG & 4) {
    if (blockIdx.x == gridDim.x / 2 && tid == 0) {
      uint64_t c1, r1;
      asm volatile("s_memtime %0\n\ts_memrealtime %1\n\ts_waitcnt lgkmcnt(0)" : "=s"(c1), "=s"(r1)::"memory");
      uint64_t* o = reinterpret_cast<uint64_t*>(d.C);
      o[0] = c1 - dbg_c0;
      o[1] = r1 - dbg_r0;
    }
    float z = 0.f;
    if constexpr (M16) {
#pragma unroll
      for (int i = 0; i < TM * 2; ++i)
#pragma unroll
        for (int j = 0; j < TN * 2; ++j)
#pragma unroll
          for (int r = 0; r < 4; ++r) z += acc16[i][j][r];
    } else {
#pragma unroll
    for (int i = 0; i < TM; ++i)
#pragma unroll
      for (int j = 0; j < TN; ++j)
#pragma unroll
        for (int r = 0; r < 16; ++r) z += acc[i][j][r];
    }
    if (z == 123.456f) reinterpret_cast<float*>(d.C)[tid] = z;
    return;
  }
  const int64_t cbase = (int64_t)bz * d.strideC;
  const float* __restrict__ res = d.res ? d.res + (int64_t)bz * d.strideR : nullptr;
  const bool vec = ((d.N & 3) == 0) && ((d.ldc & 3) == 0) && ((cbase & 3) == 0) && (!res || (d.ldr & 3) == 0) &&
                   ((reinterpret_cast<uintptr_t>(d.C) & 15) == 0) && (!res || (reinterpret_cast<uintptr_t>(res) & 15) == 0) &&
                   (!d.bias_n || (reinterpret_cast<uintptr_t>(d.bias_n) & 15) == 0) &&
                   (!d.scale_n || (reinterpret_cast<uintptr_t>(d.scale_n) & 15) == 0);
  if constexpr (M16 && PH8) {
    if (vec && !d.out_f32 && !res && !d.res16 && !d.C_lo && !d.rowstats && !d.stats && !d.scale_n && d.act != ASIS_ACT_GELU_GRAD && !(DBG & 8) &&
        (d.N & 7) == 0 && (d.ldc & 7) == 0 && (cbase & 7) == 0 && !(GROUP_M_FLAGS >> 16)) {
      constexpr int SW16 = TN * 32 + 8;
      __syncthreads();
      T* slab16 = reinterpret_cast<T*>(lds) + wid * (32 * SW16);
      const int r16 = lane & 15, q16 = lane >> 4;
      const int rr8 = lane >> 3, c8 = lane & 7;
      const bool ln_on = LNF != 0 && !CONV && d.ln_mr != nullptr, ln_c = ln_on && d.ln_cols != 0;
      const float2* const mrp = reinterpret_cast<const float2*>(d.ln_mr) + (ln_c ? (int64_t)bz * (d.strideB / d.ldb) : 0);
      float4 bj[TN * 2], cj[TN * 2];
      float2 mc[TN * 2][4];
#pragma unroll
      for (int j = 0; j < TN * 2; ++j) {
        const int colj = n0 + (wn * TN * 2 + j) * 16 + 4 * q16;
        bj[j] = (d.bias_n && kt_base == 0 && colj < d.N) ? *reinterpret_cast<const float4*>(d.bias_n + colj) : make_float4(0.f, 0.f, 0.f, 0.f);
        cj[j] = (ln_on && !ln_c && colj < d.N) ? *reinterpret_cast<const float4*>(d.ln_cs + colj) : make_float4(0.f, 0.f, 0.f, 0.f);
#pragma unroll
        for (int e = 0; e < 4; ++e) {
          mc[j][e] = make_float2(0.f, 1.f);
          if (ln_c) mc[j][e] = mrp[colj + e < d.N ? colj + e : d.N - 1];
        }
      }
      const bool sg = d.act == ASIS_ACT_SILU_MUL;
      const int colr = sg ? (n0 >> 1) + wn * TN * 16 + (lane & 3) * 8 : n0 + wn * TN * 32 + c8 * 8;
      const bool cokr = colr < (sg ? (d.N >> 1) : d.N);
      T* const Cw = reinterpret_cast<T*>(d.C) + cbase + colr;
#pragma unroll
      for (int i = 0; i < TM; ++i) {
#pragma unroll
        for (int ii = 0; ii < 2; ++ii) {
          float bm1 = 0.f, nmean = -0.f, rstd = 1.f, csr = 0.f;
          const int rowb = m0 + (wm * TM + i) * 32 + ii * 16 + r16;
          const int rowbc = rowb < d.M ? rowb : d.M - 1;
          if (d.bias_m) bm1 = d.bias_m[rowbc];
          if (ln_on && !ln_c) {
            const float2 mr = mrp[rowbc];
            nmean = -mr.x;
            rstd = mr.y;
          }
          if (ln_c) csr = d.ln_cs[rowbc];
          float4 vg = make_float4(0.f, 0.f, 0.f, 0.f);
#pragma unroll
          for (int j = 0; j < TN * 2; ++j) {
            float4 v;
            if (ln_c) {
              v = make_float4(__builtin_fmaf(__builtin_fmaf(-mc[j][0].x, csr, acc16[2 * i + ii][j][0]), mc[j][0].y, bj[j].x + bm1),
                              __builtin_fmaf(__builtin_fmaf(-mc[j][1].x, csr, acc16[2 * i + ii][j][1]), mc[j][1].y, bj[j].y + bm1),
                              __builtin_fmaf(__builtin_fmaf(-mc[j][2].x, csr, acc16[2 * i + ii][j][2]), mc[j][2].y, bj[j].z + bm1),
                              __builtin_fmaf(__builtin_fmaf(-mc[j][3].x, csr, acc16[2 * i + ii][j][3]), mc[j][3].y, bj[j].w + bm1));
            } else if (ln_on) {
              v = make_float4(__builtin_fmaf(__builtin_fmaf(nmean, cj[j].x, acc16[2 * i + ii][j][0]), rstd, bj[j].x + bm1),
                              __builtin_fmaf(__builtin_fmaf(nmean, cj[j].y, acc16[2 * i + ii][j][1]), rstd, bj[j].y + bm1),
                              __builtin_fmaf(__builtin_fmaf(nmean, cj[j].z, acc16[2 * i + ii][j][2]), rstd, bj[j].z + bm1),
                              __builtin_fmaf(__builtin_fmaf(nmean, cj[j].w, acc16[2 * i + ii][j][3]), rstd, bj[j].w + bm1));
            } else {
              v = make_float4(acc16[2 * i + ii][j][0] + bj[j].x + bm1, acc16[2 * i + ii][j][1] + bj[j].y + bm1,
                              acc16[2 * i + ii][j][2] + bj[j].z + bm1, acc16[2 * i + ii][j][3] + bj[j].w + bm1);
            }
            if (sg) {
              if (j & 1) {
                uint2 pk;
                pk.x = pack2<T>(silu_mul(vg.x, v.x), silu_mul(vg.y, v.y));
                pk.y = pack2<T>(silu_mul(vg.z, v.z), silu_mul(vg.w, v.w));
                *reinterpret_cast<uint2*>(slab16 + (ii * 16 + r16) * SW16 + 16 * (j >> 1) + 4 * q16) = pk;
              } else {
                vg = v;
              }
              continue;
            }
            if (d.act == ASIS_ACT_GELU) gelu_erf4(v.x, v.y, v.z, v.w);
            else if (d.act == ASIS_ACT_RELU) { v.x = fmaxf(v.x, 0.f); v.y = fmaxf(v.y, 0.f); v.z = fmaxf(v.z, 0.f); v.w = fmaxf(v.w, 0.f); }
            uint2 pk;
            pk.x = pack2<T>(v.x, v.y);
            pk.y = pack2<T>(v.z, v.w);
            *reinterpret_cast<uint2*>(slab16 + (ii * 16 + r16) * SW16 + 16 * j + 4 * q16) = pk;
          }
        }
        if (sg) {
#pragma unroll
          for (int p = 0; p < 2; ++p) {
            const int lrow = p * 16 + (lane >> 2);
            const int row = m0 + (wm * TM + i) * 32 + lrow;
            const uint4 w = *reinterpret_cast<const uint4*>(slab16 + lrow * SW16 + (lane & 3) * 8);
            if (row < d.M && cokr) *reinterpret_cast<uint4*>(Cw + (int64_t)row * d.ldc) = w;
          }
          continue;
        }
#pragma unroll
        for (int p = 0; p < 4; ++p) {
          const int lrow = p * 8 + rr8;
          const int row = m0 + (wm * TM + i) * 32 + lrow;
          const uint4 w = *reinterpret_cast<const uint4*>(slab16 + lrow * SW16 + c8 * 8);
          if (row < d.M && cokr) *reinterpret_cast<uint4*>(Cw + (int64_t)row * d.ldc) = w;
        }
      }
      return;
    }
  }
  if constexpr (LNF != 0 && M16 && PH8 && !CONV && !SPLIT) {
    if (d.C_lo || d.rowstats || d.res16) {
      constexpr int SW = TN * 32 + 4;
      __syncthreads();
      float* slab = reinterpret_cast<float*>(lds) + wid * (32 * SW);
      const int rr = lane >> 3, c8 = lane & 7;
      const int col = n0 + wn * TN * 32 + c8 * 8;
      const bool cok = col < d.N;
      const int colc = cok ? col : 0;
      float4 ba = make_float4(0.f, 0.f, 0.f, 0.f), bb = ba, sa = make_float4(1.f, 1.f, 1.f, 1.f), sb = sa;
      if (cok && d.bias_n) { ba = *reinterpret_cast<const float4*>(d.bias_n + col); bb = *reinterpret_cast<const float4*>(d.bias_n + col + 4); }
      if (cok && d.scale_n) { sa = *reinterpret_cast<const float4*>(d.scale_n + col); sb = *reinterpret_cast<const float4*>(d.scale_n + col + 4); }
      const bool res_planes = d.res16 != nullptr;
      const float* const zp = reinterpret_cast<const float*>(g_zero_page);
      const float* const resp = d.res ? d.res + colc : zp;
      const int64_t ldr_e = d.res ? d.ldr : 0;
      const T* const r16h = reinterpret_cast<const T*>(d.res16) + colc;
      const T* const r16l = reinterpret_cast<const T*>(d.res16_lo) + colc;
      T* const Clo = reinterpret_cast<T*>(d.C_lo);
      float* const rstats = d.rowstats;
      const int sgroups = (d.N + 63) >> 6, sgrp = (n0 + wn * TN * 32) >> 6;
#pragma unroll
      for (int i = 0; i < TM; ++i) {
#pragma unroll
        for (int ii = 0; ii < 2; ++ii)
#pragma unroll
          for (int j = 0; j < TN * 2; ++j)
            *reinterpret_cast<float4*>(slab + (ii * 16 + (lane & 15)) * SW + 16 * j + 4 * (lane >> 4)) =
                make_float4(acc16[2 * i + ii][j][0], acc16[2 * i + ii][j][1], acc16[2 * i + ii][j][2], acc16[2 * i + ii][j][3]);
        uint4 ra[4], rb[4];
#pragma unroll
        for (int q = 0; q < 4; ++q) {
          const int row = m0 + (wm * TM + i) * 32 + q * 8 + rr;
          const int rowc = row < d.M ? row : d.M - 1;
          if (res_planes) {
            ra[q] = *reinterpret_cast<const uint4*>(r16h + (int64_t)rowc * d.ldr16);
            rb[q] = *reinterpret_cast<const uint4*>(r16l + (int64_t)rowc * d.ldr16);
          } else {
            ra[q] = *reinterpret_cast<const uint4*>(resp + (int64_t)rowc * ldr_e);
            rb[q] = *reinterpret_cast<const uint4*>(resp + (int64_t)rowc * ldr_e + (d.res ? 4 : 0));
          }
        }
#pragma unroll
        for (int q = 0; q < 4; ++q) {
          const int lrow = q * 8 + rr;
          const int row = m0 + (wm * TM + i) * 32 + lrow;
          float4 va = *reinterpret_cast<const float4*>(slab + lrow * SW + c8 * 8);
          float4 vb = *reinterpret_cast<const float4*>(slab + lrow * SW + c8 * 8 + 4);
          float4 xa, xb;
          if (res_planes) {
            float h[8], l[8];
            unpack2<T>(ra[q].x, h[0], h[1]); unpack2<T>(ra[q].y, h[2], h[3]); unpack2<T>(ra[q].z, h[4], h[5]); unpack2<T>(ra[q].w, h[6], h[7]);
            unpack2<T>(rb[q].x, l[0], l[1]); unpack2<T>(rb[q].y, l[2], l[3]); unpack2<T>(rb[q].z, l[4], l[5]); unpack2<T>(rb[q].w, l[6], l[7]);
            xa = make_float4(h[0] + l[0], h[1] + l[1], h[2] + l[2], h[3] + l[3]);
            xb = make_float4(h[4] + l[4], h[5] + l[5], h[6] + l[6], h[7] + l[7]);
          } else {
            xa = __builtin_bit_cast(float4, ra[q]);
            xb = __builtin_bit_cast(float4, rb[q]);
          }
          float st_s = 0.f, st_q = 0.f;
          if (row < d.M && cok) {
            va.x = (va.x + ba.x) * sa.x + xa.x; va.y = (va.y + ba.y) * sa.y + xa.y; va.z = (va.z + ba.z) * sa.z + xa.z; va.w = (va.w + ba.w) * sa.w + xa.w;
            vb.x = (vb.x + bb.x) * sb.x + xb.x; vb.y = (vb.y + bb.y) * sb.y + xb.y; vb.z = (vb.z + bb.z) * sb.z + xb.z; vb.w = (vb.w + bb.w) * sb.w + xb.w;
            if (d.out_f32) {
              float* const cp = reinterpret_cast<float*>(d.C) + (int64_t)row * d.ldc + col;
              *reinterpret_cast<float4*>(cp) = va;
              *reinterpret_cast<float4*>(cp + 4) = vb;
            } else {
              uint4 ph;
              ph.x = pack2<T>(va.x, va.y); ph.y = pack2<T>(va.z, va.w); ph.z = pack2<T>(vb.x, vb.y); ph.w = pack2<T>(vb.z, vb.w);
              *reinterpret_cast<uint4*>(reinterpret_cast<T*>(d.C) + (int64_t)row * d.ldc + col) = ph;
              if (Clo) {
                uint4 pl;
                pl.x = pack2<T>(lo_part<T>(va.x), lo_part<T>(va.y)); pl.y = pack2<T>(lo_part<T>(va.z), lo_part<T>(va.w));
                pl.z = pack2<T>(lo_part<T>(vb.x), lo_part<T>(vb.y)); pl.w = pack2<T>(lo_part<T>(vb.z), lo_part<T>(vb.w));
                *reinterpret_cast<uint4*>(Clo + (int64_t)row * d.ldc + col) = pl;
              }
            }
            st_s = ((va.x + va.y) + (va.z + va.w)) + ((vb.x + vb.y) + (vb.z + vb.w));
            st_q = ((va.x * va.x + va.y * va.y) + (va.z * va.z + va.w * va.w)) + ((vb.x * vb.x + vb.y * vb.y) + (vb.z * vb.z + vb.w * vb.w));
          }
          if (rstats) {
            st_s = row8_sum(st_s);
            st_q = row8_sum(st_q);
            if (c8 == 0 && row < d.M && sgrp < sgroups) *reinterpret_cast<float2*>(rstats + ((int64_t)row * sgroups + sgrp) * 2) = make_float2(st_s, st_q);
          }
        }
      }
      return;
    }
  }
  if (vec) {
    constexpr int SW = TN * 32 + 4;
    constexpr int LPR = TN * 8;
    constexpr int RPP = 64 / LPR;
    __syncthreads();
    float* slab = reinterpret_cast<float*>(lds) + wid * (32 * SW);
    const int rr = lane / LPR, ch = lane - rr * LPR;
    const int col = n0 + wn * TN * 32 + ch * 4;
    const bool cok = col < d.N;
    float4 b4 = make_float4(0.f, 0.f, 0.f, 0.f), s4 = make_float4(1.f, 1.f, 1.f, 1.f);
    if (cok && d.bias_n && kt_base == 0) b4 = *reinterpret_cast<const float4*>(d.bias_n + col);
    if (cok && d.scale_n) s4 = *reinterpret_cast<const float4*>(d.scale_n + col);
    float4 st_s = make_float4(0.f, 0.f, 0.f, 0.f), st_q = st_s;
    constexpr int NP = 32 / RPP;
    const float* const zp = reinterpret_cast<const float*>(g_zero_page);
    const bool has_aux = d.act == ASIS_ACT_GELU_GRAD;
    const int colc = cok ? col : 0;
    const float* const resp = (res && !(DBG & 32)) ? res + colc : zp;
    const int64_t ldr_e = (res && !(DBG & 32)) ? d.ldr : 0;
    const float* const bmp = d.bias_m ? d.bias_m : zp;
    const int bm_e = d.bias_m ? 1 : 0;
#pragma unroll
    for (int i = 0; i < TM; ++i) {
      if constexpr (M16) {
#pragma unroll
        for (int ii = 0; ii < 2; ++ii)
#pragma unroll
          for (int j = 0; j < TN * 2; ++j)
            *reinterpret_cast<float4*>(slab + (ii * 16 + (lane & 15)) * SW + 16 * j + 4 * (lane >> 4)) =
                make_float4(acc16[2 * i + ii][j][0], acc16[2 * i + ii][j][1], acc16[2 * i + ii][j][2], acc16[2 * i + ii][j][3]);
      } else {
#pragma unroll
      for (int j = 0; j < TN; ++j)
#pragma unroll
        for (int g = 0; g < 4; ++g)
          *reinterpret_cast<float4*>(slab + fr * SW + 32 * j + 8 * g + 4 * fh) =
              make_float4(acc[i][j][4 * g + 0], acc[i][j][4 * g + 1], acc[i][j][4 * g + 2], acc[i][j][4 * g + 3]);
      }
      constexpr int PG = (OCC >= 4 && NP > 4) ? 4 : NP;
#pragma unroll
      for (int p0 = 0; p0 < NP; p0 += PG) {
        float4 r4[PG];
        float bmv[PG];
        uint2 pw[PG];
#pragma unroll
        for (int q = 0; q < PG; ++q) {
          const int row = m0 + (wm * TM + i) * 32 + (p0 + q) * RPP + rr;
          const int rowc = row < d.M ? row : d.M - 1;
          r4[q] = *reinterpret_cast<const float4*>(resp + (int64_t)rowc * ldr_e);
          bmv[q] = bmp[rowc * bm_e];
          pw[q] = make_uint2(0u, 0u);
        }
        if (has_aux) {
#pragma unroll
          for (int q = 0; q < PG; ++q) {
            const int row = m0 + (wm * TM + i) * 32 + (p0 + q) * RPP + rr;
            const int rowc = row < d.M ? row : d.M - 1;
            pw[q] = *reinterpret_cast<const uint2*>(reinterpret_cast<const T*>(d.aux) + (int64_t)rowc * d.ld_aux + colc);
          }
        }
#pragma unroll
        for (int q = 0; q < PG; ++q) {
          const int lrow = (p0 + q) * RPP + rr;
          const int row = m0 + (wm * TM + i) * 32 + lrow;
          float4 v = *reinterpret_cast<const float4*>(slab + lrow * SW + ch * 4);
          if (row < d.M && cok) {
            const float bm1 = bmv[q];
            v.x += b4.x + bm1; v.y += b4.y + bm1; v.z += b4.z + bm1; v.w += b4.w + bm1;
            if (d.act == ASIS_ACT_GELU) gelu_erf4(v.x, v.y, v.z, v.w);
            else if (has_aux) {
              float g0, g1, g2, g3;
              unpack2<T>(pw[q].x, g0, g1);
              unpack2<T>(pw[q].y, g2, g3);
              v.x *= gelu_erf_grad_fast(g0); v.y *= gelu_erf_grad_fast(g1); v.z *= gelu_erf_grad_fast(g2); v.w *= gelu_erf_grad_fast(g3);
            }
            else if (d.act == ASIS_ACT_RELU) { v.x = fmaxf(v.x, 0.f); v.y = fmaxf(v.y, 0.f); v.z = fmaxf(v.z, 0.f); v.w = fmaxf(v.w, 0.f); }
            v.x *= s4.x; v.y *= s4.y; v.z *= s4.z; v.w *= s4.w;
            v.x += r4[q].x; v.y += r4[q].y; v.z += r4[q].z; v.w += r4[q].w;
            if ((DBG & 8) && v.x != 123.456f) {
            } else if (d.out_f32) {
              *reinterpret_cast<float4*>(reinterpret_cast<float*>(d.C) + cbase + (int64_t)row * d.ldc + col) = v;
            } else {
              uint2 pk;
              pk.x = pack2<T>(v.x, v.y);
              pk.y = pack2<T>(v.z, v.w);
              *reinterpret_cast<uint2*>(reinterpret_cast<T*>(d.C) + cbase + (int64_t)row * d.ldc + col) = pk;
            }
            st_s.x += v.x; st_s.y += v.y; st_s.z += v.z; st_s.w += v.w;
            st_q.x += v.x * v.x; st_q.y += v.y * v.y; st_q.z += v.z * v.z; st_q.w += v.w * v.w;
          }
        }
      }
    }
    if (d.stats) {
      for (int o = LPR; o < 64; o <<= 1) {
        st_s.x += __shfl_xor(st_s.x, o, 64); st_s.y += __shfl_xor(st_s.y, o, 64);
        st_s.z += __shfl_xor(st_s.z, o, 64); st_s.w += __shfl_xor(st_s.w, o, 64);
        st_q.x += __shfl_xor(st_q.x, o, 64); st_q.y += __shfl_xor(st_q.y, o, 64);
        st_q.z += __shfl_xor(st_q.z, o, 64); st_q.w += __shfl_xor(st_q.w, o, 64);
      }
      __syncthreads();
      float* red = reinterpret_cast<float*>(lds);
      if (rr == 0) {
        *reinterpret_cast<float4*>(red + (wm * 2 + 0) * BN2 + wn * TN * 32 + ch * 4) = st_s;
        *reinterpret_cast<float4*>(red + (wm * 2 + 1) * BN2 + wn * TN * 32 + ch * 4) = st_q;
      }
      __syncthreads();
      if (tid < BN2 && n0 + tid < d.N) {
        float s = 0.f, q = 0.f;
#pragma unroll
        for (int w2 = 0; w2 < WM; ++w2) {
          s += red[(w2 * 2 + 0) * BN2 + tid];
          q += red[(w2 * 2 + 1) * BN2 + tid];
        }
        const int c = n0 + tid;
        constexpr int RB = BM2 / 128;
        const int64_t r0 = (int64_t)tile_m * RB;
        d.stats[(r0 * 2 + 0) * d.N + c] = s;
        d.stats[(r0 * 2 + 1) * d.N + c] = q;
#pragma unroll
        for (int e = 1; e < RB; ++e)
          if ((r0 + e) * 128 < d.M) {
            d.stats[((r0 + e) * 2 + 0) * d.N + c] = 0.f;
            d.stats[((r0 + e) * 2 + 1) * d.N + c] = 0.f;
          }
      }
    }
    return;
  }
  auto scalar_out = [&](int row, int c, float a, float bmv) {
    float x = a + (d.bias_n ? d.bias_n[c] : 0.f) + bmv;
    if (d.act == ASIS_ACT_GELU) x = gelu_erf(x);
    else if (d.act == ASIS_ACT_RELU) x = fmaxf(x, 0.f);
    if (d.scale_n) x *= d.scale_n[c];
    if (res) x += res[(int64_t)row * d.ldr + c];
    if (d.out_f32) reinterpret_cast<float*>(d.C)[cbase + (int64_t)row * d.ldc + c] = x;
    else reinterpret_cast<T*>(d.C)[cbase + (int64_t)row * d.ldc + c] = to_t16<T>(x);
  };
  if constexpr (M16) {
#pragma unroll
    for (int i = 0; i < TM * 2; ++i) {
      const int row = m0 + (wm * TM * 2 + i) * 16 + (lane & 15);
      if (row >= d.M) continue;
      const float bmv = d.bias_m ? d.bias_m[row] : 0.f;
#pragma unroll
      for (int j = 0; j < TN * 2; ++j)
#pragma unroll
        for (int e = 0; e < 4; ++e) {
          const int c = n0 + (wn * TN * 2 + j) * 16 + 4 * (lane >> 4) + e;
          if (c < d.N) scalar_out(row, c, acc16[i][j][e], bmv);
        }
    }
    return;
  }
#pragma unroll
  for (int i = 0; i < TM; ++i) {
    const int row = m0 + (wm * TM + i) * 32 + fr;
    const bool rok = row < d.M;
    const float bmv = (d.bias_m && rok) ? d.bias_m[row] : 0.f;
#pragma unroll
    for (int j = 0; j < TN; ++j) {
#pragma unroll
      for (int g = 0; g < 4; ++g) {
        const int col = n0 + (wn * TN + j) * 32 + 8 * g + 4 * fh;
        if (!rok || col >= d.N) continue;
#pragma unroll
        for (int e = 0; e < 4; ++e) {
          const int c = col + e;
          if (c < d.N) {
            float x = acc[i][j][4 * g + e] + (d.bias_n ? d.bias_n[c] : 0.f) + bmv;
            if (d.act == ASIS_ACT_GELU) x = gelu_erf(x);
            else if (d.act == ASIS_ACT_RELU) x = fmaxf(x, 0.f);
            if (d.scale_n) x *= d.scale_n[c];
            if (res) x += res[(int64_t)row * d.ldr + c];
            if (d.out_f32) reinterpret_cast<float*>(d.C)[cbase + (int64_t)row * d.ldc + c] = x;
            else reinterpret_cast<T*>(d.C)[cbase + (int64_t)row * d.ldc + c] = to_t16<T>(x);
          }
        }
      }
    }
  }
}


}
```

### adaptersis_amd/dinov2/layers/blocks.py

```python
from __future__ import annotations

import contextlib
import math
import os
from typing import Callable, Optional, Tuple, Union

import torch
from torch import nn

from ... import config, ops


_VT_STREAMS = {}


def _vt_side_stream(device) -> "torch.cuda.Stream":
    key = (device.type, device.index)
    if key not in _VT_STREAMS:
        _VT_STREAMS[key] = torch.cuda.Stream(device=device)
    return _VT_STREAMS[key]


_PRECISE_FOLD_Q = os.environ.get("ASIS_PRECISE_FOLD_Q", "1") not in ("0", "")
_ATTN_MX_OUT = os.environ.get("ASIS_ATTN_MX_OUT", "1") not in ("0", "")
_LS_POW2_REFRESH = 64


def _pack(cache: dict, key: str, param: torch.Tensor, fn: Callable[[torch.Tensor], torch.Tensor]):
    tag = (param.data_ptr(), param._version, getattr(param, "_asis_gen", 0), config.operand_dtype, param.device)
    hit = cache.get(key)
    if hit is None or hit[0] != tag:
        with torch.no_grad():
            cache[key] = (tag, fn(param.detach()))
    return cache[key][1]


class _Packed(nn.Module):
    def __init__(self):
        super().__init__()
        self._cache = {}

    def _w16(self, key: str, param: torch.Tensor, rows: Optional[torch.Tensor] = None) -> torch.Tensor:
        if rows is not None:
            return _pack(self._cache, key + ".sg", param,
                         lambda p: ops.cast_pad(p.reshape(p.shape[0], -1).float()[rows].contiguous(), dtype=config.operand_dtype))
        return _pack(self._cache, key, param,
                     lambda p: ops.cast_pad(p.reshape(p.shape[0], -1).contiguous().float(), dtype=config.operand_dtype))

    def _w16lo(self, key: str, param: torch.Tensor) -> Optional[torch.Tensor]:
        if not config.precise_attention:
            return None
        return _pack(self._cache, key + ".lo", param,
                     lambda p: ops.cast_pad(p.reshape(p.shape[0], -1).contiguous().float(), dtype=config.operand_dtype, part=1))

    def _f32(self, key: str, param: Optional[torch.Tensor]) -> Optional[torch.Tensor]:
        if param is None:
            return None
        return _pack(self._cache, key, param, lambda p: p.float().contiguous())

    def _pack2(self, key: str, w: torch.Tensor, gamma: Optional[torch.Tensor], fn):
        tag = tuple((t.data_ptr(), t._version, getattr(t, "_asis_gen", 0)) for t in (w, gamma) if t is not None) + \
            (config.operand_dtype,)
        hit = self._cache.get(key)
        if hit is None or hit[0] != tag:
            with torch.no_grad():
                self._cache[key] = (tag, fn())
        return self._cache[key][1]

    def _wT16(self, key: str, w: torch.Tensor, gamma: Optional[torch.Tensor] = None, pow2: int = 0) -> torch.Tensor:
        def make():
            wf = w.detach().float()
            if gamma is not None:
                wf = wf * (gamma.detach().float() * (2.0 ** pow2))[:, None]
            return ops.cast_pad(wf.t().contiguous(), dtype=config.operand_dtype)
        return self._pack2(key + (f"@{pow2}" if pow2 else ""), w, gamma, make)

    def _ls_pow2(self, key: str, gamma: Optional[torch.Tensor]) -> int:
        if gamma is None:
            return 0
        tag = (gamma.data_ptr(), gamma.device, config.operand_dtype)
        ver, gen = gamma._version, getattr(gamma, "_asis_gen", 0)
        ent = self._cache.get(key)
        if ent is not None and ent[0] == tag and ent[1][1] == ver:
            st = ent[1]
            if st[2] == gen:
                return st[0]
            if st[3] + 1 < _LS_POW2_REFRESH:
                st[2], st[3] = gen, st[3] + 1
                return st[0]
        m = float(gamma.detach().abs().max())
        k = 0 if not (m > 0.0 and m < float("inf")) else -int(math.floor(math.log2(m)))
        if ent is not None and ent[0] == tag and ent[1][0] != k:
            for stale in [c for c in self._cache if c.endswith(f"@{ent[1][0]}") or c.endswith(f"@{-ent[1][0]}")]:
                del self._cache[stale]
        self._cache[key] = (tag, [k, ver, gen, 0])
        return k

    def _nw_pow2(self, key: str, w: torch.Tensor, pow2: int) -> torch.Tensor:
        if pow2 == 0:
            return self._f32(key, w)
        return _pack(self._cache, f"{key}@{pow2}", w, lambda p: (p.float() * (2.0 ** pow2)).contiguous())

    def _linear_bwd(self, prefix: str, lin: nn.Linear, gamma: Optional[nn.Parameter], gname: Optional[str], dy16, dy_cs,
                    a16, inv_scale: float, grads: Optional[dict]):
        if grads is None:
            return
        N, K = lin.weight.shape
        R = a16.shape[0]
        G = ops.wgrad(dy16.view(1, R, 1, N), a16.view(1, R, 1, K), N, 1, 1, 1, 0, 1.0).view(N, K)
        cs = ops.reduce_rows(dy_cs)
        ops.ls_linear_finish(G, lin.weight.detach() if gamma is not None else None,
                             lin.bias.detach() if lin.bias is not None else None,
                             gamma.detach() if gamma is not None else None, cs, inv_scale, grads[prefix + ".weight"],
                             grads.get(prefix + ".bias") if lin.bias is not None else None,
                             grads[gname] if gamma is not None else None)



def make_2tuple(x):
    if isinstance(x, tuple):
        assert len(x) == 2
        return x
    assert isinstance(x, int)
    return (x, x)


class PatchEmbed(_Packed):

    def __init__(self, img_size=224, patch_size=16, in_chans=3, embed_dim=768, norm_layer=None,
                 flatten_embedding=True):
        super().__init__()
        image_HW, patch_HW = make_2tuple(img_size), make_2tuple(patch_size)
        if in_chans != 3 or patch_HW[0] != patch_HW[1]:
            raise ValueError("PatchEmbed: only 3-channel images and square patches are supported")
        self.img_size, self.patch_size = image_HW, patch_HW
        self.patches_resolution = (image_HW[0] // patch_HW[0], image_HW[1] // patch_HW[1])
        self.num_patches = self.patches_resolution[0] * self.patches_resolution[1]
        self.in_chans, self.embed_dim, self.flatten_embedding = in_chans, embed_dim, flatten_embedding
        self.proj = nn.Conv2d(in_chans, embed_dim, kernel_size=patch_HW, stride=patch_HW)
        self.norm = norm_layer(embed_dim) if norm_layer else nn.Identity()
        if norm_layer:
            raise ValueError("PatchEmbed: norm_layer is not used on this path (vision_transformer.py:104)")

    def tokens(self, x: torch.Tensor, out: Optional[torch.Tensor] = None):
        B, _, H, W = x.shape
        P = self.patch_size[0]
        K = 3 * P * P
        dt = config.operand_dtype
        bias = self._f32("b", self.proj.bias)
        if config.split_conv:
            ldk = (K + 63) // 64 * 64
            flat = lambda p: p.reshape(p.shape[0], -1).contiguous().float()
            w_hi = _pack(self._cache, "w64", self.proj.weight, lambda p: ops.cast_pad(flat(p), ldk, dt))
            w_lo = _pack(self._cache, "w64lo", self.proj.weight, lambda p: ops.cast_pad(flat(p), ldk, dt, part=1))
            a, a_lo = ops.im2col_patch(x.contiguous().float(), P, ldk, dt, split=True)
            if out is None:
                out = torch.empty((a.shape[0], self.embed_dim), device=x.device, dtype=torch.float32)
            ops.gemm_split(a, a_lo, w_hi, w_lo, out=out, bias_n=bias)
        else:
            ldk = (K + 7) // 8 * 8
            w16 = _pack(self._cache, "w", self.proj.weight,
                        lambda p: ops.cast_pad(p.reshape(p.shape[0], -1).contiguous().float(), ldk, dt))
            a = ops.im2col_patch(x.contiguous().float(), P, ldk, dt)
            out = ops.gemm(a, w16, out=out, out_f32=True, bias_n=bias)
        return out.view(B, (H // P) * (W // P), self.embed_dim), a

    def forward(self, x: torch.Tensor) -> torch.Tensor:
        B, _, H, W = x.shape
        P = self.patch_size[0]
        assert H % P == 0, f"Input image height {H} is not a multiple of patch height {P}"
        assert W % P == 0, f"Input image width {W} is not a multiple of patch width: {P}"
        out, _ = self.tokens(x)
        if not self.flatten_embedding:
            out = out.reshape(-1, H // P, W // P, self.embed_dim)
        return out


class LayerScale(nn.Module):

    def __init__(self, dim: int, init_values: Union[float, torch.Tensor] = 1e-5, inplace: bool = False):
        super().__init__()
        self.inplace = inplace
        self.gamma = nn.Parameter(init_values * torch.ones(dim))


class Attention(_Packed):

    def __init__(self, dim, num_heads=8, qkv_bias=False, proj_bias=True, attn_drop=0.0, proj_drop=0.0):
        super().__init__()
        if dim % num_heads or dim // num_heads != 64:
            raise ValueError("attention kernel supports head dim 64 (every DINOv2 arch): "
                             f"got dim={dim}, heads={num_heads}")
        if attn_drop or proj_drop:
            raise ValueError("dropout is 0 on the AdapterSIS path (models/__init__.py:14-29)")
        self.num_heads = num_heads
        self.scale = (dim // num_heads) ** -0.5
        self.qkv = nn.Linear(dim, dim * 3, bias=qkv_bias)
        self.proj = nn.Linear(dim, dim, bias=proj_bias)

    def _qkv_folded(self):
        c = self.scale * 1.4426950408889634
        D = self.qkv.weight.shape[1]

        def scaled(p):
            w = p.reshape(p.shape[0], -1).float().clone()
            w[:D] *= c
            return w.contiguous()
        w = _pack(self._cache, "qkv.fold", self.qkv.weight, lambda p: ops.cast_pad(scaled(p), dtype=config.operand_dtype))
        wlo = None
        if config.precise_attention:
            wlo = _pack(self._cache, "qkv.fold.lo", self.qkv.weight,
                        lambda p: ops.cast_pad(scaled(p), dtype=config.operand_dtype, part=1))
        bias = None
        if self.qkv.bias is not None:
            bias = _pack(self._cache, "qkv_b.fold", self.qkv.bias, lambda p: scaled(p).reshape(-1))
        return w, bias, wlo

    def _qkv_ln_folded(self, norm: nn.LayerNorm):
        c = self.scale * 1.4426950408889634 if config.fold_attn_scale else 1.0
        D = self.qkv.weight.shape[1]
        ps = [p for p in (self.qkv.weight, self.qkv.bias, norm.weight, norm.bias) if p is not None]
        tag = tuple((t.data_ptr(), t._version, getattr(t, "_asis_gen", 0)) for t in ps) + (config.operand_dtype, c)
        hit = self._cache.get("qkv.lnfold")
        if hit is None or hit[0] != tag:
            with torch.no_grad():
                w = self.qkv.weight.detach().float().clone()
                w[:D] *= c
                b = self.qkv.bias.detach().float().clone() if self.qkv.bias is not None else torch.zeros(3 * D, device=w.device)
                b[:D] *= c
                b = b + w @ norm.bias.detach().float()
                w16 = ops.cast_pad((w * norm.weight.detach().float()[None, :]).contiguous(), dtype=config.operand_dtype)
                self._cache["qkv.lnfold"] = (tag, (w16, b.contiguous(), w16.float().sum(1).contiguous()))
        return self._cache["qkv.lnfold"][1]

    def attend(self, xn: torch.Tensor, B: int, N: int) -> torch.Tensor:
        return self.attend_rows(xn, [(B, N)])[0]

    def attend_rows(self, xn: torch.Tensor, segs, ln=None):
        D = xn.shape[1]
        if ln is not None:
            norm, mr = ln
            w, bias, cs = self._qkv_ln_folded(norm)
            scale = None if config.fold_attn_scale else self.scale
            o = torch.empty((xn.shape[0], D), device=xn.device, dtype=xn.dtype)
            o_lo = torch.empty_like(o) if config.split_attn_out else None
            one_launch = len(segs) == 2
            ldv_all = (max(n for _, n in segs) + 63) // 64 * 64
            vt_all = torch.empty((sum(b for b, _ in segs), D, ldv_all), device=xn.device, dtype=xn.dtype)
            spare = xn.untyped_storage().nbytes() // xn.element_size() - (xn.storage_offset() + xn.shape[0] * D)
            side = None
            if one_launch and config.vt_stream:
                main = torch.cuda.current_stream()
                side = _vt_side_stream(xn.device)
                side.wait_stream(main)
            else:
                qk = ops.gemm(xn, w[: 2 * D], bias_n=bias[: 2 * D], ln=(mr, cs[: 2 * D], False))
            r0 = b0 = 0
            for B, N in segs:
                r1 = r0 + B * N
                vt = vt_all[b0:b0 + B]
                N4 = (N + 7) // 8 * 8
                if spare < (N4 - N) * D:
                    raise ValueError("attend_rows(ln=...): the hi plane needs 8 spare rows behind it")
                with (torch.cuda.stream(side) if side is not None else contextlib.nullcontext()):
                    ops.gemm(w[2 * D:], xn[r0:r1].as_strided((B, N4, D), (N * D, D, 1)),
                             out=vt.as_strided((B, D, N4), (D * ldv_all, ldv_all, 1)), bias_m=bias[2 * D:], ln=(mr[r0:], cs[2 * D:], True))
                if not one_launch:
                    ops.attention_fwd(qk[r0:r1, :D], qk[r0:r1, D:], vt, B, self.num_heads, N, scale, out=o[r0:r1],
                                      out_lo=None if o_lo is None else o_lo[r0:r1])
                r0, b0 = r1, b0 + B
            if side is not None:
                qk = ops.gemm(xn, w[: 2 * D], bias_n=bias[: 2 * D], ln=(mr, cs[: 2 * D], False))
                main.wait_stream(side)
                mr.record_stream(side)
            if one_launch:
                (B1, N1), (B2, N2) = segs
                ops.attention_fwd_seg(qk[:, :D], qk[:, D:], vt_all, B1, N1, B2, N2, self.num_heads, scale, out=o, out_lo=o_lo)
            if r0 != xn.shape[0]:
                raise ValueError("attend_rows: segments do not cover the rows")
            return o, o_lo
        if config.fold_attn_scale:
            w, bias, wlo = self._qkv_folded()
            scale = None
        else:
            w = self._w16("qkv", self.qkv.weight)
            bias = self._f32("qkv_b", self.qkv.bias)
            wlo = self._w16lo("qkv", self.qkv.weight)
            scale = self.scale
        o = torch.empty((xn.shape[0], D), device=xn.device, dtype=xn.dtype)
        o_lo = torch.empty_like(o) if config.split_attn_out else None
        if config.fused_qkv and len(segs) <= 2:
            if sum(b * n for b, n in segs) != xn.shape[0]:
                raise ValueError("attend_rows: segments do not cover the rows")
            qkv = ops.gemm(xn, w, bias_n=bias, b_lo=wlo)
            ops.attention_fwd_qkv(qkv, list(segs), self.num_heads, scale, o, out_lo=o_lo)
            return o, o_lo
        one_launch = len(segs) == 2
        ldv_all = (max(n for _, n in segs) + 63) // 64 * 64
        vt_all = torch.empty((sum(b for b, _ in segs), D, ldv_all), device=xn.device, dtype=xn.dtype) if one_launch else None
        spare = xn.untyped_storage().nbytes() // xn.element_size() - (xn.storage_offset() + xn.shape[0] * D)
        side = None
        if one_launch and config.vt_stream and xn.is_cuda:
            main = torch.cuda.current_stream()
            side = _vt_side_stream(xn.device)
            side.wait_stream(main)
        else:
            qk = ops.gemm(xn, w[: 2 * D], bias_n=None if bias is None else bias[: 2 * D], b_lo=None if wlo is None else wlo[: 2 * D])
        r0 = b0 = 0
        for B, N in segs:
            r1 = r0 + B * N
            ldvt = ldv_all if one_launch else (N + 63) // 64 * 64
            vt = vt_all[b0:b0 + B] if one_launch else torch.empty((B, D, ldvt), device=xn.device, dtype=xn.dtype)
            N4 = (N + 3) // 4 * 4 if spare >= 4 * D else N
            with (torch.cuda.stream(side) if side is not None else contextlib.nullcontext()):
                ops.gemm(w[2 * D:], xn[r0:r1].as_strided((B, N4, D), (N * D, D, 1)),
                         out=vt.as_strided((B, D, N4), (D * ldvt, ldvt, 1)), bias_m=None if bias is None else bias[2 * D:],
                         a_lo=None if wlo is None else wlo[2 * D:])
            if not one_launch:
                ops.attention_fwd(qk[r0:r1, :D], qk[r0:r1, D:], vt, B, self.num_heads, N, scale, out=o[r0:r1],
                                  out_lo=None if o_lo is None else o_lo[r0:r1])
            r0, b0 = r1, b0 + B
        if side is not None:
            qk = ops.gemm(xn, w[: 2 * D], bias_n=None if bias is None else bias[: 2 * D], b_lo=None if wlo is None else wlo[: 2 * D])
            main.wait_stream(side)
        if one_launch:
            (B1, N1), (B2, N2) = segs
            ops.attention_fwd_seg(qk[:, :D], qk[:, D:], vt_all, B1, N1, B2, N2, self.num_heads, scale, out=o, out_lo=o_lo)
        if r0 != xn.shape[0]:
            raise ValueError("attend_rows: segments do not cover the rows")
        return o, o_lo

    def forward(self, x: torch.Tensor) -> torch.Tensor:
        raise RuntimeError("Attention is driven by Block.forward (LayerNorm / LayerScale / residual are fused around it)")


class MemEffAttention(Attention):
    """`attention.py:72-89`: same maths as ``Attention``; here both are the fused flash kernel."""


class Mlp(_Packed):

    def __init__(self, in_features, hidden_features=None, out_features=None, act_layer=nn.GELU, drop=0.0, bias=True):
        super().__init__()
        out_features = out_features or in_features
        hidden_features = hidden_features or in_features
        self.fc1 = nn.Linear(in_features, hidden_features, bias=bias)
        self.fc2 = nn.Linear(hidden_features, out_features, bias=bias)


class SwiGLUFFN(_Packed):

    def __init__(self, in_features, hidden_features=None, out_features=None, act_layer=None, drop=0.0, bias=True):
        super().__init__()
        out_features = out_features or in_features
        hidden_features = hidden_features or in_features
        self.w12 = nn.Linear(in_features, 2 * hidden_features, bias=bias)
        self.w3 = nn.Linear(hidden_features, out_features, bias=bias)

    def sg_rows(self) -> torch.Tensor:
        return _pack(self._cache, "w12.sgrows", self.w12.weight, lambda p: ops.swiglu_rows(p.shape[0] // 2, p.device))

    def sg_bias(self) -> Optional[torch.Tensor]:
        if self.w12.bias is None:
            return None
        rows = self.sg_rows()
        return _pack(self._cache, "w12_b.sg", self.w12.bias, lambda p: p.float()[rows].contiguous())


class SwiGLUFFNFused(SwiGLUFFN):

    def __init__(self, in_features, hidden_features=None, out_features=None, act_layer=None, drop=0.0, bias=True):
        out_features = out_features or in_features
        hidden_features = hidden_features or in_features
        hidden_features = (int(hidden_features * 2 / 3) + 7) // 8 * 8
        super().__init__(in_features, hidden_features, out_features, bias=bias)


class Block(_Packed):

    def __init__(self, dim, num_heads, mlp_ratio=4.0, qkv_bias=False, proj_bias=True, ffn_bias=True, drop=0.0,
                 attn_drop=0.0, init_values=None, drop_path=0.0, act_layer=nn.GELU, norm_layer=nn.LayerNorm,
                 attn_class=Attention, ffn_layer=Mlp):
        super().__init__()
        if drop_path or drop:
            raise ValueError("stochastic depth / dropout are 0 on the AdapterSIS path")
        self.norm1 = norm_layer(dim)
        self.attn = attn_class(dim, num_heads=num_heads, qkv_bias=qkv_bias, proj_bias=proj_bias)
        self.ls1 = LayerScale(dim, init_values=init_values) if init_values else nn.Identity()
        self.norm2 = norm_layer(dim)
        self.mlp = ffn_layer(in_features=dim, hidden_features=int(dim * mlp_ratio), act_layer=act_layer, bias=ffn_bias)
        self.ls2 = LayerScale(dim, init_values=init_values) if init_values else nn.Identity()
        self.sample_drop_ratio = drop_path

    def forward(self, x: torch.Tensor) -> torch.Tensor:
        B, N, D = x.shape
        x2 = x.reshape(B * N, D)
        if x2.dtype != torch.float32 or not x2.is_contiguous():
            x2 = x2.float().contiguous()
        return self.forward_rows(x2, [(B, N)]).view(B, N, D)

    def _w16lo_any(self, owner, key: str, w: torch.Tensor, rows: Optional[torch.Tensor] = None):
        sel = (lambda t: t) if rows is None else (lambda t: t[rows])
        return _pack(owner._cache, key + (".sg" if rows is not None else "") + ".lo_any", w,
                     lambda p: ops.cast_pad(sel(p.reshape(p.shape[0], -1).float()).contiguous(), dtype=config.operand_dtype, part=1))

    def _w16mx_any(self, owner, key: str, w: torch.Tensor, rows: Optional[torch.Tensor] = None):
        return _pack(owner._cache, key + (".sg" if rows is not None else "") + ".mx_any", w,
                     lambda p: ops.mx_from_pair(owner._w16(key, w, rows), self._w16lo_any(owner, key, w, rows), wside=True))

    def _mx_ok(self, owner, key: str, lin: nn.Linear, M: int) -> bool:
        N, K = lin.weight.shape
        return config.mx_dense_on() and K % 64 == 0 and N >= 256 and M >= 256 and N * K < (1 << 31)

    def _split_lin(self, owner, key: str, lin: nn.Linear, a_hi, a_lo, a_mx=None, rows=None, **kw):
        w = owner._w16(key, lin.weight, rows)
        if self._mx_ok(owner, key, lin, a_hi.shape[0]):
            a_pl, amax_a = a_mx if a_mx is not None else ops.mx_from_pair(a_hi, a_lo)
            w_mx, amax_w = self._w16mx_any(owner, key, lin.weight, rows)
            return ops.gemm(a_hi, w, a_lo=a_pl, b_lo=w_mx, mx=(amax_a, amax_w), **kw)
        return ops.gemm(a_hi, w, a_lo=a_lo, b_lo=self._w16lo_any(owner, key, lin.weight, rows), **kw)

    def _ln_split(self, key: str, norm: nn.LayerNorm, x2: torch.Tensor, mx: bool):
        dt = config.operand_dtype
        w, b = self._f32(key + "w", norm.weight), self._f32(key + "b", norm.bias)
        if mx:
            amax = _pack(self._cache, key + ".amax", norm.weight,
                         lambda p: ((x2.shape[1] - 1) ** 0.5 * p.float().abs().max() + norm.bias.detach().float().abs().max()).reshape(1).contiguous())
            hi, pl = ops.layernorm_mx(x2, w, b, norm.eps, dt, amax)
            return hi, None, (pl, amax)
        xn32 = ops.layernorm(x2, w, b, norm.eps, torch.float32)
        D = x2.shape[1]
        return ops.cast_pad(xn32, D, dt), ops.cast_pad(xn32, D, dt, part=1), None

    def _forward_rows_precise(self, x2: torch.Tensor, segs) -> torch.Tensor:
        D = x2.shape[1]
        R = x2.shape[0]
        dt = config.operand_dtype
        a, m = self.attn, self.mlp
        g1 = self._f32("g1", self.ls1.gamma) if isinstance(self.ls1, LayerScale) else None
        g2 = self._f32("g2", self.ls2.gamma) if isinstance(self.ls2, LayerScale) else None
        parts = config.precise_parts
        n1w, n1b = self._f32("n1w", self.norm1.weight), self._f32("n1b", self.norm1.bias)
        fold_q = config.fold_attn_scale and "qkv" not in parts and _PRECISE_FOLD_Q
        if "qkv" in parts:
            xn, xn_lo, xn_mx = self._ln_split("n1", self.norm1, x2, self._mx_ok(a, "qkv", a.qkv, R))
            qkv = self._split_lin(a, "qkv", a.qkv, xn, xn_lo, xn_mx, bias_n=a._f32("qkv_b", a.qkv.bias))
        elif fold_q:
            qw, qb, _ = a._qkv_folded()
            qkv = ops.gemm(ops.layernorm(x2, n1w, n1b, self.norm1.eps, dt), qw, bias_n=qb)
        else:
            qkv = ops.gemm(ops.layernorm(x2, n1w, n1b, self.norm1.eps, dt), a._w16("qkv", a.qkv.weight), bias_n=a._f32("qkv_b", a.qkv.bias))
        o = torch.empty((R, D), device=x2.device, dtype=dt)
        o_lo = torch.empty_like(o) if "proj" in parts else None
        if sum(B * N for B, N in segs) != R:
            raise ValueError("forward_rows: segments do not cover the rows")
        o_mx = None
        if fold_q and len(segs) <= 2:
            if o_lo is not None and _ATTN_MX_OUT and self._mx_ok(a, "proj", a.proj, R):
                o_mx = ops.absmax16(qkv[:, 2 * D:3 * D])
            ops.attention_fwd_qkv(qkv, list(segs), a.num_heads, None, o, out_lo=o_lo, mx_amax=o_mx)
        else:
            r0 = 0
            for B, N in segs:
                r1 = r0 + B * N
                vt = ops.transpose_tokens(qkv[r0:r1, 2 * D:], B, N)
                ops.attention_fwd(qkv[r0:r1, :D], qkv[r0:r1, D:2 * D], vt, B, a.num_heads, N, None if fold_q else a.scale,
                                  out=o[r0:r1], out_lo=None if o_lo is None else o_lo[r0:r1])
                r0 = r1
        pkw = dict(out_f32=True, bias_n=a._f32("proj_b", a.proj.bias), scale_n=g1, res=x2)
        if o_mx is not None:
            x1 = self._split_lin(a, "proj", a.proj, o, None, a_mx=(o_lo, o_mx), **pkw)
        else:
            x1 = self._split_lin(a, "proj", a.proj, o, o_lo, **pkw) if o_lo is not None else ops.gemm(o, a._w16("proj", a.proj.weight), **pkw)
        n2w, n2b = self._f32("n2w", self.norm2.weight), self._f32("n2b", self.norm2.bias)
        lin_in, k_in = (m.fc1, "fc1") if isinstance(m, Mlp) else (m.w12, "w12")
        lin_out, k_out = (m.fc2, "fc2") if isinstance(m, Mlp) else (m.w3, "w3")
        ikw = dict(out_f32=True, bias_n=m._f32(k_in + "_b", lin_in.bias))
        split_out = "fc2" in parts
        mx_in = "fc1" in parts and self._mx_ok(m, k_in, lin_in, R)
        sg = (not isinstance(m, Mlp)) and not split_out and \
            ops.swiglu_fused_ok(R, lin_in.out_features // 2, lin_in.in_features, "fc1" in parts, mx_in)
        ge = isinstance(m, Mlp) and not split_out
        if sg:
            rows = m.sg_rows()
            ikw = dict(bias_n=m.sg_bias(), act=ops.ACT_SILU_MUL, rows=rows)
        elif ge:
            ikw = dict(bias_n=m._f32(k_in + "_b", lin_in.bias), act=ops.ACT_GELU)
        if "fc1" in parts:
            xn2, xn2_lo, xn2_mx = self._ln_split("n2", self.norm2, x1, mx_in)
            hpre = self._split_lin(m, k_in, lin_in, xn2, xn2_lo, xn2_mx, **ikw)
        else:
            rows = ikw.pop("rows", None)
            hpre = ops.gemm(ops.layernorm(x1, n2w, n2b, self.norm2.eps, dt), m._w16(k_in, lin_in.weight, rows), **ikw)
        if sg or ge:
            h, h_lo = hpre, None
        elif isinstance(m, Mlp):
            h, h_lo = ops.gelu_split(hpre, dt, split=split_out)
        else:
            h, h_lo = ops.swiglu(hpre, dt, split=True) if split_out else (ops.swiglu(hpre, dt), None)
        okw = dict(out_f32=True, bias_n=m._f32(k_out + "_b", lin_out.bias), scale_n=g2, res=x1)
        if split_out:
            return self._split_lin(m, k_out, lin_out, h, h_lo, **okw)
        return ops.gemm(h, m._w16(k_out, lin_out.weight), **okw)

    def _lin_ln_folded(self, key: str, lin: nn.Linear, norm: nn.LayerNorm):
        ps = [p for p in (lin.weight, lin.bias, norm.weight, norm.bias) if p is not None]
        tag = tuple((t.data_ptr(), t._version, getattr(t, "_asis_gen", 0)) for t in ps) + (config.operand_dtype,)
        hit = self._cache.get(key)
        if hit is None or hit[0] != tag:
            with torch.no_grad():
                w = lin.weight.detach().float()
                b = (lin.bias.detach().float() if lin.bias is not None else torch.zeros(w.shape[0], device=w.device)) + w @ norm.bias.detach().float()
                w16 = ops.cast_pad((w * norm.weight.detach().float()[None, :]).contiguous(), dtype=config.operand_dtype)
                self._cache[key] = (tag, (w16, b.contiguous(), w16.float().sum(1).contiguous()))
        return self._cache[key][1]

    def fold_ok(self, R: int, segs) -> bool:
        if not (config.ln_fold and config.operand_dtype == torch.float16 and config.precise_level < 2 and not config.precise_attention
                and not config.fused_qkv and isinstance(self.mlp, Mlp) and isinstance(self.ls1, LayerScale)
                and isinstance(self.ls2, LayerScale) and isinstance(self.norm1, nn.LayerNorm) and isinstance(self.norm2, nn.LayerNorm)):
            return False
        D, Hd = self.attn.qkv.weight.shape[1], self.mlp.fc1.weight.shape[0]
        if config.split_attn_out:
            return False
        ok = ops.ln_fold_supported(R, 2 * D, D) and ops.ln_fold_supported(R, D, D, producer=True)
        ok = ok and ops.ln_fold_supported(R, Hd, D) and ops.ln_fold_supported(R, D, Hd, producer=True)
        return ok and all(ops.ln_fold_supported(D, (N + 7) // 8 * 8, D, batch=B) for B, N in segs) and D % 64 == 0

    def forward_rows_fold(self, xin, segs, planes_out: bool):
        dt = config.operand_dtype
        a, m = self.attn, self.mlp
        g1, g2 = self._f32("g1", self.ls1.gamma), self._f32("g2", self.ls2.gamma)
        if isinstance(xin, tuple):
            hi, lo, mr = xin
            R, D = hi.shape
            o, o_lo = a.attend_rows(hi, segs, ln=(self.norm1, mr))
            res_kw = dict(res16=(hi, lo))
        else:
            R, D = xin.shape
            xn = torch.empty((R + 8, D), device=xin.device, dtype=dt)[:R]
            ops.layernorm(xin, self._f32("n1w", self.norm1.weight), self._f32("n1b", self.norm1.bias), self.norm1.eps, dt, out=xn)
            o, o_lo = a.attend_rows(xn, segs)
            res_kw = dict(res=xin)
        G = (D + 63) // 64
        x1h = torch.empty((R, D), device=o.device, dtype=dt)
        x1l = torch.empty((R, D), device=o.device, dtype=dt)
        st = torch.empty((R, G, 2), device=o.device, dtype=torch.float32)
        ops.gemm(o, a._w16("proj", a.proj.weight), out=x1h, out_lo=x1l, rowstats=st, bias_n=a._f32("proj_b", a.proj.bias), scale_n=g1,
                 a_lo=o_lo, **res_kw)
        mr1 = ops.ln_stats_finalize(st, D, self.norm2.eps)
        w1, b1, cs1 = self._lin_ln_folded("fc1.lnfold", m.fc1, self.norm2)
        h = ops.gemm(x1h, w1, bias_n=b1, act=ops.ACT_GELU, ln=(mr1, cs1, False))
        w2, b2 = m._w16("fc2", m.fc2.weight), m._f32("fc2_b", m.fc2.bias)
        if not planes_out:
            return ops.gemm(h, w2, out_f32=True, bias_n=b2, scale_n=g2, res16=(x1h, x1l))
        x3h = torch.empty((R + 8, D), device=o.device, dtype=dt)[:R]
        x3l = torch.empty((R, D), device=o.device, dtype=dt)
        st3 = torch.empty((R, G, 2), device=o.device, dtype=torch.float32)
        ops.gemm(h, w2, out=x3h, out_lo=x3l, rowstats=st3, bias_n=b2, scale_n=g2, res16=(x1h, x1l))
        return x3h, x3l, ops.ln_stats_finalize(st3, D, self.norm1.eps)

    def forward_rows(self, x2: torch.Tensor, segs) -> torch.Tensor:
        if config.precise_level >= 2:
            return self._forward_rows_precise(x2, segs)
        D = x2.shape[1]
        dt = config.operand_dtype
        g1 = self._f32("g1", self.ls1.gamma) if isinstance(self.ls1, LayerScale) else None
        g2 = self._f32("g2", self.ls2.gamma) if isinstance(self.ls2, LayerScale) else None
        xn = torch.empty((x2.shape[0] + 8, D), device=x2.device, dtype=dt)[: x2.shape[0]]
        ops.layernorm(x2, self._f32("n1w", self.norm1.weight), self._f32("n1b", self.norm1.bias), self.norm1.eps, dt, out=xn)
        o, o_lo = self.attn.attend_rows(xn, segs)
        x1 = ops.gemm(o, self.attn._w16("proj", self.attn.proj.weight), out_f32=True,
                      bias_n=self.attn._f32("proj_b", self.attn.proj.bias), scale_n=g1, res=x2, a_lo=o_lo,
                      b_lo=self.attn._w16lo("proj", self.attn.proj.weight))
        xn2 = ops.layernorm(x1, self._f32("n2w", self.norm2.weight), self._f32("n2b", self.norm2.bias),
                            self.norm2.eps, dt)
        m = self.mlp
        if isinstance(m, Mlp):
            h = ops.gemm(xn2, m._w16("fc1", m.fc1.weight), bias_n=m._f32("fc1_b", m.fc1.bias), act=ops.ACT_GELU)
            x3 = ops.gemm(h, m._w16("fc2", m.fc2.weight), out_f32=True, bias_n=m._f32("fc2_b", m.fc2.bias),
                          scale_n=g2, res=x1)
        else:
            if ops.swiglu_fused_ok(xn2.shape[0], m.w12.out_features // 2, m.w12.in_features, False, False):
                h = ops.gemm(xn2, m._w16("w12", m.w12.weight, m.sg_rows()), bias_n=m.sg_bias(), act=ops.ACT_SILU_MUL)
            else:
                h12 = ops.gemm(xn2, m._w16("w12", m.w12.weight), out_f32=True, bias_n=m._f32("w12_b", m.w12.bias))
                h = ops.swiglu(h12, dt)
            x3 = ops.gemm(h, m._w16("w3", m.w3.weight), out_f32=True, bias_n=m._f32("w3_b", m.w3.bias),
                          scale_n=g2, res=x1)
        return x3

    def forward_train(self, x: torch.Tensor):
        B, N, D = x.shape
        x2 = x.reshape(B * N, D)
        if x2.dtype != torch.float32 or not x2.is_contiguous():
            x2 = x2.float().contiguous()
        out, saved = self.forward_train_rows(x2, [(B, N)])
        return out.view(B, N, D), saved

    def forward_train_rows(self, x2: torch.Tensor, segs):
        dt = config.operand_dtype
        D = x2.shape[1]
        m = self.mlp
        g1 = self._f32("g1", self.ls1.gamma) if isinstance(self.ls1, LayerScale) else None
        g2 = self._f32("g2", self.ls2.gamma) if isinstance(self.ls2, LayerScale) else None
        a = self.attn
        xn = ops.layernorm(x2, self._f32("n1w", self.norm1.weight), self._f32("n1b", self.norm1.bias), self.norm1.eps, dt)
        qkv = ops.gemm(xn, a._w16("qkv", a.qkv.weight), bias_n=a._f32("qkv_b", a.qkv.bias), b_lo=a._w16lo("qkv", a.qkv.weight))
        o = torch.empty((x2.shape[0], D), device=x2.device, dtype=dt)
        o_lo = torch.empty_like(o) if config.split_attn_out else None
        if sum(B * N for B, N in segs) != x2.shape[0]:
            raise ValueError("forward_train_rows: segments do not cover the rows")
# ... 97 lines not shown
```

### adaptersis_amd/ops.py

```python
from __future__ import annotations

import ctypes as C
import os
from typing import Optional

import torch

from . import _lib
from ._lib import ACT_GELU, ACT_GELU_GRAD, ACT_NONE, ACT_RELU, ACT_SILU_MUL, GemmDesc, check, lib

T16_DEFAULT = torch.float16

PROFILE = None


def _launch_timed(kind: str, flops: float, fn, nbytes: float = 0.0):
    if PROFILE is None:
        return fn()
    s, e = torch.cuda.Event(enable_timing=True), torch.cuda.Event(enable_timing=True)
    s.record()
    rc = fn()
    e.record()
    PROFILE.append((kind, flops, s, e, nbytes))
    return rc


def _dt(dtype: torch.dtype) -> int:
    if dtype == torch.float16:
        return _lib.ASIS_F16
    if dtype == torch.bfloat16:
        return _lib.ASIS_BF16
    raise ValueError(f"operand dtype must be float16 or bfloat16, got {dtype}")


def _dev(*ts) -> None:
    for t in ts:
        if t is not None and not t.is_cuda:
            raise _lib.AsisError("adaptersis_amd ops run on an MI355X (HIP) device only; got a CPU tensor "
                                 "(there is no CPU fallback)")


def _p(t: Optional[torch.Tensor]):
    return None if t is None else t.data_ptr()


def _stream():
    return torch.cuda.current_stream().cuda_stream


def _f32c(t: Optional[torch.Tensor]) -> Optional[torch.Tensor]:
    if t is None:
        return None
    if t.dtype != torch.float32 or not t.is_contiguous():
        raise ValueError("expected a contiguous float32 tensor")
    return t


def _gemm_desc(a: torch.Tensor, b: torch.Tensor, *, out: Optional[torch.Tensor] = None, out_f32: bool = False,
               bias_n: Optional[torch.Tensor] = None, bias_m: Optional[torch.Tensor] = None,
               scale_n: Optional[torch.Tensor] = None, res: Optional[torch.Tensor] = None, act: int = ACT_NONE,
               stats: Optional[torch.Tensor] = None, a_lo: Optional[torch.Tensor] = None,
               b_lo: Optional[torch.Tensor] = None, aux: Optional[torch.Tensor] = None,
               out_lo: Optional[torch.Tensor] = None, rowstats: Optional[torch.Tensor] = None, res16=None, ln=None, mx=None):
    _dev(a, b, out, bias_n, bias_m, scale_n, res, stats, out_lo, rowstats)
    if a.dtype != b.dtype:
        raise ValueError("gemm operands must have the same 16-bit dtype")
    batch = 1
    if a.dim() == 3 or b.dim() == 3:
        batch = a.shape[0] if a.dim() == 3 else b.shape[0]
    M, K = a.shape[-2], a.shape[-1]
    N = b.shape[-2]
    if b.shape[-1] != K:
        raise ValueError(f"gemm: inner dims differ: a[...,{K}] vs b[...,{b.shape[-1]}]")
    if a.stride(-1) != 1 or b.stride(-1) != 1:
        raise ValueError("gemm: K must be contiguous in both operands")
    n_out = N // 2 if act == ACT_SILU_MUL else N
    if act == ACT_SILU_MUL and (out_f32 or batch != 1 or N % 32):
        raise ValueError("gemm: ACT_SILU_MUL writes a 16-bit [M, N / 2] matrix of one unbatched launch (N % 32 == 0)")
    if out is None:
        shape = (batch, M, n_out) if (a.dim() == 3 or b.dim() == 3) else (M, n_out)
        out = torch.empty(shape, device=a.device, dtype=torch.float32 if out_f32 else a.dtype)
    else:
        out_f32 = out.dtype == torch.float32
        if out.stride(-1) != 1 or out.shape[-1] != n_out:
            raise ValueError("gemm: out must be contiguous in its last dim, one column per output feature")
    d = GemmDesc()
    d.A, d.B, d.C = a.data_ptr(), b.data_ptr(), out.data_ptr()
    d.lda, d.ldb, d.ldc = a.stride(-2), b.stride(-2), out.stride(-2)
    d.strideA = a.stride(0) if a.dim() == 3 else 0
    d.strideB = b.stride(0) if b.dim() == 3 else 0
    d.strideC = out.stride(0) if out.dim() == 3 else 0
    d.batch, d.M, d.N, d.K = batch, M, N, K
    d.bias_n, d.bias_m, d.scale_n = _p(_f32c(bias_n)), _p(_f32c(bias_m)), _p(_f32c(scale_n))
    if res is not None:
        if res.dtype != torch.float32 or res.stride(-1) != 1:
            raise ValueError("gemm: res must be float32, contiguous in its last dim")
        d.res, d.ldr = res.data_ptr(), res.stride(-2)
        d.strideR = res.stride(0) if res.dim() == 3 else 0
    d.act, d.out_f32, d.dtype = act, int(out_f32), _dt(a.dtype)
    d.stats = _p(stats)
    if aux is not None:
        if aux.dtype != a.dtype or aux.shape[-2:] != (M, N) or aux.stride(-1) != 1:
            raise ValueError("gemm: aux must be a 16-bit [M, N] matrix of the operand dtype")
        d.aux, d.ld_aux = aux.data_ptr(), aux.stride(-2)
    flops = 2.0 * batch * M * N * K
    if (a_lo is None) != (b_lo is None) and not (K % 64 == 0 and M >= 256 and N >= 32 and N % 4 == 0 and out.stride(-2) % 4 == 0):
        a_lo = b_lo = None
    if a_lo is not None:
        if a_lo.stride() != a.stride():
            raise ValueError("gemm: split halves must share the layout of their hi parts")
        d.A_lo = a_lo.data_ptr()
    if b_lo is not None:
        if b_lo.stride() != b.stride():
            raise ValueError("gemm: split halves must share the layout of their hi parts")
        d.B_lo = b_lo.data_ptr()
    if mx is not None:
        if a_lo is None or b_lo is None:
            raise ValueError("gemm: mx needs both MX planes (a_lo and b_lo)")
        _dev(mx[0], mx[1])
        d.mx_amax_a, d.mx_amax_b = mx[0].data_ptr(), mx[1].data_ptr()
    if out_lo is not None:
        if out_lo.dtype != out.dtype or out_lo.stride() != out.stride() or out.dtype == torch.float32:
            raise ValueError("gemm: out_lo must be a 16-bit tensor with the layout of out")
        d.C_lo = out_lo.data_ptr()
    if rowstats is not None:
        if rowstats.dtype != torch.float32 or rowstats.numel() != M * ((N + 63) // 64) * 2 or not rowstats.is_contiguous():
            raise ValueError("gemm: rowstats must be a contiguous float32 [M, ceil(N / 64), 2] tensor")
        d.rowstats = rowstats.data_ptr()
    if res16 is not None:
        rh, rl = res16
        _dev(rh, rl)
        if rh.dtype != a.dtype or rl.dtype != a.dtype or rh.stride() != rl.stride() or rh.stride(-1) != 1 or rh.shape[-2:] != (M, N):
            raise ValueError("gemm: res16 = (hi, lo) 16-bit [M, N] planes of the operand dtype with equal strides")
        d.res16, d.res16_lo, d.ldr16 = rh.data_ptr(), rl.data_ptr(), rh.stride(-2)
    if ln is not None:
        mr, cs, cols = ln
        _dev(mr, cs)
        d.ln_mr, d.ln_cs, d.ln_cols = _f32c(mr).data_ptr(), _f32c(cs).data_ptr(), int(bool(cols))
    nbytes = batch * (2.0 * (M * K + N * K) + M * N * ((4 if (out_f32 or out_lo is not None) else 2) +
                                                    (4 if (res is not None or res16 is not None) else 0)))
    return d, out, flops, nbytes


def gemm(a: torch.Tensor, b: torch.Tensor, **kw) -> torch.Tensor:
    d, out, flops, nbytes = _gemm_desc(a, b, **kw)
    check(_launch_timed("gemm", flops, lambda: lib().asis_gemm(_stream(), C.byref(d)), nbytes), "asis_gemm")
    return out


def gemm_tiles_m(M: int) -> int:
    return lib().asis_gemm_tiles_m(int(M))


def gemm_set_option(name: str, value: int) -> None:
    check(lib().asis_gemm_set_option(name.encode(), int(value)), "asis_gemm_set_option")


def conv_gemm(x_nhwc: torch.Tensor, w_packed: torch.Tensor, KH: int, KW: int, stride: int, pad: int, *,
              out: Optional[torch.Tensor] = None, out_f32: bool = True, bias_n: Optional[torch.Tensor] = None,
              act: int = ACT_NONE, stats: Optional[torch.Tensor] = None, accumulate: bool = False,
              x_lo: Optional[torch.Tensor] = None, w_lo: Optional[torch.Tensor] = None, ksplit: int = 1, mx=None) -> torch.Tensor:
    _dev(x_nhwc, w_packed, out, bias_n, stats)
    if not x_nhwc.is_contiguous():
        raise ValueError("conv_gemm: x must be contiguous NHWC")
    Bn, H, W, Cin = x_nhwc.shape
    Cout, K = w_packed.shape
    OH = (H + 2 * pad - KH) // stride + 1
    OW = (W + 2 * pad - KW) // stride + 1
    if ksplit > 1:
        if out is not None or accumulate or not out_f32 or act != ACT_NONE or stats is not None:
            raise ValueError("conv_gemm: ksplit needs a fresh fp32 output without activation; take the BatchNorm "
                             "statistics from the sum with colstats()")
        parts = torch.empty((ksplit, Bn, OH, OW, Cout), device=x_nhwc.device, dtype=torch.float32)
        out = parts
    if out is None:
        out = torch.empty((Bn, OH, OW, Cout), device=x_nhwc.device, dtype=torch.float32 if out_f32 else x_nhwc.dtype)
    d = GemmDesc()
    d.A, d.B, d.C = x_nhwc.data_ptr(), w_packed.data_ptr(), out.data_ptr()
    if ksplit > 1:
        d.ksplit, d.strideC = ksplit, Bn * OH * OW * Cout
    d.lda, d.ldb, d.ldc = K, w_packed.stride(0), Cout
    d.batch, d.M, d.N, d.K = 1, Bn * OH * OW, Cout, K
    d.bias_n = _p(_f32c(bias_n))
    if accumulate:
        if out.dtype != torch.float32:
            raise ValueError("conv_gemm: accumulate needs an fp32 output")
        d.res, d.ldr = out.data_ptr(), Cout
    d.act, d.out_f32, d.dtype = act, int(out.dtype == torch.float32), _dt(x_nhwc.dtype)
    d.conv, d.B_, d.H, d.W, d.Cin, d.OH, d.OW = 1, Bn, H, W, Cin, OH, OW
    d.KH, d.KW, d.stride, d.pad = KH, KW, stride, pad
    d.stats = _p(stats)
    flops = 2.0 * d.M * Cout * K
    if x_lo is not None:
        d.A_lo, d.B_lo = x_lo.data_ptr(), w_lo.data_ptr()
    if mx is not None:
        d.mx_amax_a, d.mx_amax_b = _f32c(mx[0]).data_ptr(), _f32c(mx[1]).data_ptr()
    check(_launch_timed("conv", flops, lambda: lib().asis_gemm(_stream(), C.byref(d))), "asis_gemm(conv)")
    if ksplit > 1:
        out = torch.empty((Bn, OH, OW, Cout), device=x_nhwc.device, dtype=torch.float32)
        reduce_rows(parts.view(ksplit, -1), 1.0, out.view(-1))
    return out


_FUSED_SPLIT = os.environ.get("ASIS_GEMM_BIG", "1") != "0" and os.environ.get("ASIS_SPLIT_FUSED", "1") != "0"
CONV_HALO = os.environ.get("ASIS_CONV_HALO", "1") not in ("0", "")


def conv_gemm_split(x_hi, x_lo, w_hi, w_lo, KH: int, KW: int, stride: int, pad: int, *, bias_n=None, stats=None,
                    ksplit: int = 1, mx=None):
    if mx is None:
        _not_mx("conv_gemm_split", x_lo, w_lo)
    Bn, H, W, Cin = x_hi.shape
    OH, OW = (H + 2 * pad - KH) // stride + 1, (W + 2 * pad - KW) // stride + 1
    Cout = w_hi.shape[0]
    if Cin % 64 == 0 and Bn * OH * OW >= 256 and Cout >= 32 and Cout % 4 == 0 and _FUSED_SPLIT:
        return conv_gemm(x_hi, w_hi, KH, KW, stride, pad, bias_n=bias_n, stats=stats, x_lo=x_lo, w_lo=w_lo, ksplit=ksplit, mx=mx)
    if mx is not None:
        raise ValueError("conv_gemm_split: MX operands need the fused large-tile path (mx_conv_ok)")
    out = conv_gemm(x_hi, w_hi, KH, KW, stride, pad, bias_n=bias_n)
    conv_gemm(x_lo, w_hi, KH, KW, stride, pad, out=out, accumulate=True)
    conv_gemm(x_hi, w_lo, KH, KW, stride, pad, out=out, accumulate=True, stats=stats)
    return out


def conv_halo_ok(x_hi: torch.Tensor, Cout: int, stride: int, pad: int, force: bool = False) -> bool:
    return ((CONV_HALO or force) and x_hi.dtype == torch.float16 and stride == 1 and pad == 1 and x_hi.shape[3] % 64 == 0 and Cout in (64, 128)
            and x_hi.is_contiguous())


def conv3x3_halo_mx(x_hi, x_mx, w_hi, w_mx, mx, *, bias_n=None, want_stats: bool = False):
    _dev(x_hi, x_mx, w_hi, w_mx, bias_n, mx[0], mx[1])
    Bn, H, W, Cin = x_hi.shape
    Cout = w_hi.shape[0]
    if not (x_hi.is_contiguous() and x_mx.is_contiguous() and w_hi.is_contiguous() and w_mx.is_contiguous() and w_hi.shape[1] == 9 * Cin):
        raise ValueError("conv3x3_halo_mx: contiguous NHWC planes and [Cout, 9 Cin] packed weights expected")
    out = torch.empty((Bn, H, W, Cout), device=x_hi.device, dtype=torch.float32)
    stats = None
    if want_stats:
        stats = torch.empty((lib().asis_conv3x3_halo_mx_tiles(Bn, H, W), 2, Cout), device=x_hi.device, dtype=torch.float32)
    check(lib().asis_conv3x3_halo_mx(_stream(), _dt(x_hi.dtype), x_hi.data_ptr(), x_mx.data_ptr(), w_hi.data_ptr(), w_mx.data_ptr(),
                                     _p(_f32c(bias_n)), mx[0].data_ptr(), mx[1].data_ptr(), out.data_ptr(), _p(stats), Bn, H, W, Cin, Cout),
          "asis_conv3x3_halo_mx")
    return (out, stats) if want_stats else out


def gemm_split(a_hi, a_lo, b_hi, b_lo, *, out: torch.Tensor, bias_n=None):
    M, K, N = a_hi.shape[-2], a_hi.shape[-1], b_hi.shape[-2]
    if K % 64 == 0 and M >= 256 and N >= 32 and N % 4 == 0 and _FUSED_SPLIT:
        return gemm(a_hi, b_hi, out=out, bias_n=bias_n, a_lo=a_lo, b_lo=b_lo)
    gemm(a_hi, b_hi, out=out, bias_n=bias_n)
    gemm(a_lo, b_hi, out=out, res=out)
    gemm(a_hi, b_lo, out=out, res=out)
    return out


def ln_fold_supported(M: int, N: int, K: int, batch: int = 1, producer: bool = False) -> bool:
    if M < 256 or N < 256 or K % 64 or K < 128 or N % 8:
        return False
    tiles = ((M + 255) // 256) * ((N + 255) // 256)
    if not producer and batch == 1 and tiles >= 256 and K <= 2048:
        return True
    return K >= 2048 or (K >= 1024 and tiles * batch >= 128)


def ln_stats_finalize(rowstats: torch.Tensor, D: int, eps: float = 1e-6) -> torch.Tensor:
    _dev(rowstats)
    rows, groups = rowstats.shape[0], rowstats.shape[1]
    mr = torch.empty((rows + 8, 2), device=rowstats.device, dtype=torch.float32)[:rows]
    check(lib().asis_ln_stats_finalize(_stream(), _f32c(rowstats).data_ptr(), rows, groups, D, float(eps), mr.data_ptr()),
          "asis_ln_stats_finalize")
    return mr


def split_stats(x: torch.Tensor, dtype: torch.dtype, eps: float = 1e-6):
    _dev(x)
    if x.dtype != torch.float32 or x.dim() != 2 or x.stride(1) != 1:
        raise ValueError("split_stats: x must be float32 [rows, D] contiguous in D")
    rows, D = x.shape
    hi = torch.empty((rows + 8, D), device=x.device, dtype=dtype)[:rows]
    lo = torch.empty((rows, D), device=x.device, dtype=dtype)
    mr = torch.empty((rows + 8, 2), device=x.device, dtype=torch.float32)[:rows]
    check(lib().asis_split_stats(_stream(), _dt(dtype), x.data_ptr(), x.stride(0), hi.data_ptr(), lo.data_ptr(), D, mr.data_ptr(),
                                 rows, D, float(eps)), "asis_split_stats")
    return hi, lo, mr


def layernorm(x: torch.Tensor, w: torch.Tensor, b: torch.Tensor, eps: float = 1e-6,
              out_dtype: torch.dtype = T16_DEFAULT, out: Optional[torch.Tensor] = None) -> torch.Tensor:
    _dev(x, w, b, out)
    if x.dtype != torch.float32 or x.stride(-1) != 1:
        raise ValueError("layernorm: x must be float32 with a contiguous last dim")
    D = x.shape[-1]
    x2 = x.reshape(-1, D)
    if out is None:
        out = torch.empty(x.shape, device=x.device, dtype=out_dtype)
    o2 = out.view(-1, D)
    f32 = out.dtype == torch.float32
    check(lib().asis_layernorm(_stream(), _dt(out.dtype) if not f32 else 0, x2.data_ptr(), x2.stride(0),
                               _f32c(w).data_ptr(), _f32c(b).data_ptr(), float(eps), o2.data_ptr(), o2.stride(0),
                               int(f32), x2.shape[0], D), "asis_layernorm")
    return out


def layernorm_mx(x: torch.Tensor, w: torch.Tensor, b: torch.Tensor, eps: float, out_dtype: torch.dtype, amax: torch.Tensor):
    _dev(x, w, b, amax)
    if x.dtype != torch.float32 or x.dim() != 2 or x.stride(1) != 1:
        raise ValueError("layernorm_mx: x must be float32 [rows, D] with contiguous columns")
    R, D = x.shape
    hi = torch.empty((R, D), device=x.device, dtype=out_dtype)
    mx = torch.empty_like(hi)
    check(lib().asis_layernorm_mx(_stream(), _dt(out_dtype), x.data_ptr(), x.stride(0), _f32c(w).data_ptr(), _f32c(b).data_ptr(), float(eps),
                                  hi.data_ptr(), mx.data_ptr(), D, amax.data_ptr(), R, D), "asis_layernorm_mx")
    return hi, mx


def _check_out_lo(out: torch.Tensor, out_lo: Optional[torch.Tensor]) -> None:
    if out_lo is not None and (out_lo.shape != out.shape or out_lo.stride() != out.stride() or out_lo.dtype != out.dtype):
        raise ValueError("attention_fwd: out_lo must share the shape, layout and dtype of out")


def _attention_launch(q, k, vt, out, out_lo, B1, N1, B2, N2, H, scale, lse):
    if scale is None:
        check(lib().asis_attention_fwd_prescaled(_stream(), _dt(q.dtype), q.data_ptr(), k.data_ptr(), q.stride(0), vt.data_ptr(),
                                                 vt.stride(1), out.data_ptr(), _p(out_lo), out.stride(0), B1, N1, B2, N2, H,
                                                 _p(lse)), "asis_attention_fwd_prescaled")
    else:
        check(lib().asis_attention_fwd_split(_stream(), _dt(q.dtype), q.data_ptr(), k.data_ptr(), q.stride(0), vt.data_ptr(),
                                             vt.stride(1), out.data_ptr(), _p(out_lo), out.stride(0), B1, N1, B2, N2, H,
                                             float(scale), _p(lse)), "asis_attention_fwd")


def attention_fwd_qkv(qkv: torch.Tensor, segs, H: int, scale: Optional[float], out: torch.Tensor,
                      out_lo: Optional[torch.Tensor] = None, lse: Optional[torch.Tensor] = None,
                      mx_amax: Optional[torch.Tensor] = None) -> torch.Tensor:
    _dev(qkv, out, out_lo, lse, mx_amax)
    D = H * 64
    if qkv.dim() != 2 or qkv.shape[1] < 3 * D or qkv.stride(1) != 1 or len(segs) not in (1, 2):
        raise ValueError("attention_fwd_qkv: qkv must be [rows, >= 3*H*64] with contiguous rows, one or two segments")
    (B1, N1), (B2, N2) = (segs[0], segs[1]) if len(segs) == 2 else (segs[0], (0, 0))
    if qkv.shape[0] != B1 * N1 + B2 * N2:
        raise ValueError("attention_fwd_qkv: segments do not cover the rows")
    _check_out_lo(out, out_lo)
    es = qkv.element_size()
    if mx_amax is not None:
        if out_lo is None:
            raise ValueError("attention_fwd_qkv: mx_amax needs the second output plane")
        check(lib().asis_attention_fwd_qkv_mx(_stream(), _dt(qkv.dtype), qkv.data_ptr(), qkv.data_ptr() + D * es,
                                              qkv.data_ptr() + 2 * D * es, qkv.stride(0), out.data_ptr(), out_lo.data_ptr(), out.stride(0),
                                              B1, N1, B2, N2, H, 0.0 if scale is None else float(scale), int(scale is None), _p(lse),
                                              mx_amax.data_ptr()), "asis_attention_fwd_qkv_mx")
        return out
    check(lib().asis_attention_fwd_qkv(_stream(), _dt(qkv.dtype), qkv.data_ptr(), qkv.data_ptr() + D * es,
                                       qkv.data_ptr() + 2 * D * es, qkv.stride(0), out.data_ptr(), _p(out_lo), out.stride(0),
                                       B1, N1, B2, N2, H, 0.0 if scale is None else float(scale), int(scale is None), _p(lse)),
          "asis_attention_fwd_qkv")
    return out


def attention_fwd(q: torch.Tensor, k: torch.Tensor, vt: torch.Tensor, B: int, H: int, N: int, scale: Optional[float],
                  out: Optional[torch.Tensor] = None, lse: Optional[torch.Tensor] = None,
                  out_lo: Optional[torch.Tensor] = None) -> torch.Tensor:
    _dev(q, k, vt, out, lse, out_lo)
    if q.stride(0) != k.stride(0) or q.stride(1) != 1 or k.stride(1) != 1:
        raise ValueError("attention_fwd: q and k must share a row stride and be contiguous in the last dim")
    if out is None:
        out = torch.empty((B * N, H * 64), device=q.device, dtype=q.dtype)
    if lse is not None and (lse.dtype != torch.float32 or lse.numel() != B * H * N or not lse.is_contiguous()):
        raise ValueError("attention_fwd: lse must be contiguous float32 [B,H,N]")
    _check_out_lo(out, out_lo)
    _attention_launch(q, k, vt, out, out_lo, B, N, 0, 0, H, scale, lse)
    return out


def attention_fwd_seg(q: torch.Tensor, k: torch.Tensor, vt: torch.Tensor, B1: int, N1: int, B2: int, N2: int, H: int,
                      scale: Optional[float], out: torch.Tensor, out_lo: Optional[torch.Tensor] = None) -> torch.Tensor:
    _dev(q, k, vt, out, out_lo)
    _check_out_lo(out, out_lo)
    if q.stride(0) != k.stride(0) or q.stride(1) != 1 or k.stride(1) != 1 or q.shape[0] != B1 * N1 + B2 * N2:
        raise ValueError("attention_fwd_seg: q and k must be row views over both batches with one row stride")
    _attention_launch(q, k, vt, out, out_lo, B1, N1, B2, N2, H, scale, None)
    return out


def token_ld(N: int) -> int:
    return (N + 63) // 64 * 64


def transpose_tokens(src: torch.Tensor, B: int, N: int, out: Optional[torch.Tensor] = None) -> torch.Tensor:
    _dev(src, out)
    Cc = src.shape[1]
    if src.stride(1) != 1 or src.shape[0] != B * N:
        raise ValueError("transpose_tokens: expected a [B*N, C] row view")
    ldt = token_ld(N)
    if out is None:
        out = torch.empty((B, Cc, ldt), device=src.device, dtype=src.dtype)
    check(lib().asis_transpose_tokens(_stream(), _dt(src.dtype), src.data_ptr(), src.stride(0), out.data_ptr(), ldt, B, N,
                                      Cc), "asis_transpose_tokens")
    return out


def attention_bwd_rows(q, k, v, o, dO, lse, segs, H: int, scale: float, dqkv: Optional[torch.Tensor] = None) -> torch.Tensor:
    _dev(q, k, v, o, dO, lse, dqkv)
    Wd = H * 64
    if len(segs) not in (1, 2):
        raise ValueError("attention_bwd_rows: one or two stacked token batches")
    (B1, N1), (B2, N2) = segs[0], (segs[1] if len(segs) == 2 else (0, 0))
    R = B1 * N1 + B2 * N2
    if not (q.stride(0) == k.stride(0) == v.stride(0)) or q.stride(1) != 1 or q.shape[0] != R:
        raise ValueError("attention_bwd_rows: q, k, v must be [R, H*64] views sharing a row stride")
    if lse.dtype != torch.float32 or not lse.is_contiguous() or lse.numel() != R * H:
        raise ValueError("attention_bwd_rows: lse must be one contiguous float32 buffer of R * H values")
    if dqkv is None:
        dqkv = torch.empty((R, 3 * Wd), device=q.device, dtype=q.dtype)
    D = torch.empty(R * H, device=q.device, dtype=torch.float32)
    es = dqkv.element_size()
    check(lib().asis_attention_bwd_rows(_stream(), _dt(q.dtype), q.data_ptr(), k.data_ptr(), v.data_ptr(), q.stride(0),
                                        o.data_ptr(), o.stride(0), dO.data_ptr(), dO.stride(0), lse.data_ptr(), D.data_ptr(),
                                        dqkv.data_ptr(), dqkv.data_ptr() + Wd * es, dqkv.data_ptr() + 2 * Wd * es,
                                        dqkv.stride(0), B1, N1, B2, N2, H, float(scale)), "asis_attention_bwd_rows")
    return dqkv


def layernorm_bwd(dy: torch.Tensor, x: torch.Tensor, w: torch.Tensor, eps: float = 1e-6,
                  res: Optional[torch.Tensor] = None, out: Optional[torch.Tensor] = None):
    _dev(dy, x, w, res, out)
    R, D = x.shape
    for t in (dy, x, res, out):
        if t is not None and (t.dtype != torch.float32 or t.stride(-1) != 1 or t.shape != x.shape):
            raise ValueError("layernorm_bwd: float32 [R, D] row views of one shape expected")
    if out is None:
        out = torch.empty((R, D), device=x.device, dtype=torch.float32)
    nblk = lib().asis_rowblock_nblk(R)
    partial = torch.empty((nblk, 2, D), device=x.device, dtype=torch.float32)
    check(lib().asis_layernorm_bwd(_stream(), dy.data_ptr(), dy.stride(0), x.data_ptr(), x.stride(0), _f32c(w).data_ptr(),
                                   float(eps), _p(res), res.stride(0) if res is not None else 0, out.data_ptr(),
                                   out.stride(0), partial.data_ptr(), R, D), "asis_layernorm_bwd")
    return out, partial


def gelu16(pre: torch.Tensor, dpost: Optional[torch.Tensor] = None) -> torch.Tensor:
    _dev(pre, dpost)
    if not pre.is_contiguous() or (dpost is not None and (not dpost.is_contiguous() or dpost.shape != pre.shape)):
        raise ValueError("gelu16: contiguous operands of one shape expected")
    out = torch.empty_like(pre)
# ... 1202 lines not shown
```

### include/asis_hip.h

```cpp
#ifndef ASIS_HIP_H
#define ASIS_HIP_H

#include <stdint.h>

#ifdef __cplusplus
extern "C" {
#endif

#define ASIS_OK 0
#define ASIS_EINVAL (-1)
#define ASIS_ELAUNCH (-2)

#define ASIS_F16 0
#define ASIS_BF16 1
#define ASIS_F32 2

#define ASIS_ACT_NONE 0
#define ASIS_ACT_GELU 1
#define ASIS_ACT_RELU 2
#define ASIS_ACT_SILU_MUL 3
#define ASIS_ACT_GELU_GRAD 4

const char* asis_last_error(void);
int asis_version(void);
int asis_device_count(void);

typedef struct asis_gemm_desc {
  const void* A;
  const void* B;
  void* C;
  int64_t lda, ldb, ldc;
  int64_t strideA, strideB, strideC;
  int32_t batch;
  int32_t M, N, K;
  const float* bias_n;
  const float* bias_m;
  const float* scale_n;
  const float* res;
  int64_t ldr, strideR;
  int32_t act;
  int32_t out_f32;
  int32_t dtype;
  int32_t conv;
  int32_t B_, H, W, Cin, OH, OW, KH, KW, stride, pad;
  float* stats;
  const void* A_lo;
  const void* B_lo;
  const void* aux;
  int64_t ld_aux;
  int32_t ksplit;
  const float* mx_amax_a;
  const float* mx_amax_b;
  void* C_lo;
  float* rowstats;
  const void* res16;
  const void* res16_lo;
  int64_t ldr16;
  const float* ln_mr;
  const float* ln_cs;
  int32_t ln_cols;
} asis_gemm_desc;
int asis_ln_stats_finalize(void* stream, const float* rowstats, int64_t rows, int groups, int D, float eps, float* mr);
int asis_split_stats(void* stream, int dtype, const float* x, int64_t ldx, void* hi, void* lo, int64_t ld16, float* mr,
                     int64_t rows, int D, float eps);
int asis_gemm(void* stream, const asis_gemm_desc* d);
int asis_gemm_tiles_m(int M);
int asis_absmax_f32(void* stream, const float* x, int64_t rows, int cols, int64_t ld, float* amax, int reset);
int asis_bn_relu_absmax(void* stream, const float* x, const float* scale, const float* shift, int64_t P, int C, int relu, float* amax);
int asis_conv3x3_halo_mx_tiles(int B, int H, int W);
int asis_conv3x3_halo_mx(void* stream, int dtype, const void* x_hi, const void* x_mx, const void* w_hi, const void* w_mx, const float* bias,
                         const float* amax_a, const float* amax_b, float* out, float* stats, int B, int H, int W, int Cin, int Cout);
int asis_absmax_16(void* stream, int dtype, const void* x, int64_t rows, int cols, int64_t ld, float* amax);
int asis_mx_from_pair(void* stream, int dtype, const void* hi, const void* lo, int64_t ld_in, void* out_mx, int64_t ld_out, int64_t rows,
                      int cols, const float* amax, int wside);
int asis_gemm_set_option(const char* name, int value);

int asis_layernorm(void* stream, int dtype, const float* x, int64_t ldx, const float* w, const float* b, float eps,
                   void* y, int64_t ldy, int out_f32, int64_t rows, int D);
int asis_layernorm_mx(void* stream, int dtype, const float* x, int64_t ldx, const float* w, const float* b, float eps, void* y,
                      void* y_mx, int64_t ldy, const float* amax, int64_t rows, int D);

int asis_attention_fwd(void* stream, int dtype, const void* q, const void* k, int64_t ldqk, const void* vt,
                       int64_t ldvt, void* o, int64_t ldo, int B, int H, int N, float scale);
int asis_attention_fwd_seg(void* stream, int dtype, const void* q, const void* k, int64_t ldqk, const void* vt, int64_t ldvt,
                           void* o, int64_t ldo, int B1, int N1, int B2, int N2, int H, float scale, float* lse2);
int asis_attention_fwd_split(void* stream, int dtype, const void* q, const void* k, int64_t ldqk, const void* vt, int64_t ldvt,
                             void* o, void* o_lo, int64_t ldo, int B1, int N1, int B2, int N2, int H, float scale, float* lse2);
int asis_attention_fwd_prescaled(void* stream, int dtype, const void* q, const void* k, int64_t ldqk, const void* vt, int64_t ldvt,
                                 void* o, void* o_lo, int64_t ldo, int B1, int N1, int B2, int N2, int H, float* lse2);
int asis_attention_fwd_qkv(void* stream, int dtype, const void* q, const void* k, const void* v, int64_t ld, void* o, void* o_lo,
                           int64_t ldo, int B1, int N1, int B2, int N2, int H, float scale, int prescaled, float* lse2);
int asis_attention_fwd_qkv_mx(void* stream, int dtype, const void* q, const void* k, const void* v, int64_t ld, void* o, void* o_mx,
                              int64_t ldo, int B1, int N1, int B2, int N2, int H, float scale, int prescaled, float* lse2,
                              const float* amax);
int asis_attention_fwd_lse(void* stream, int dtype, const void* q, const void* k, int64_t ldqk, const void* vt,
                           int64_t ldvt, void* o, int64_t ldo, int B, int H, int N, float scale, float* lse2);
int asis_transpose_tokens(void* stream, int dtype, const void* src, int64_t ld, void* dst, int64_t ldt, int B, int N,
                          int C);
int asis_attention_bwd_rows(void* stream, int dtype, const void* q, const void* k, const void* v, int64_t ld, const void* o,
                            int64_t ldo, const void* dO, int64_t lddo, const float* lse2, float* D, void* dq, void* dk,
                            void* dv, int64_t lddq, int B1, int N1, int B2, int N2, int H, float scale);

int asis_im2col_patch(void* stream, int dtype, const float* img, int B, int Himg, int Wimg, int P, void* out,
                      int64_t ldk);
int asis_im2col_patch_split(void* stream, int dtype, const float* img, int B, int Himg, int Wimg, int P, void* out,
                            void* out_lo, int64_t ldk);

int asis_cast_pad(void* stream, int dtype, const float* src, int64_t ld_src, void* dst, int64_t ld_dst, int64_t rows,
                  int cols, float scale, int part);

int asis_add_cls_pos(void* stream, const float* x, const float* cls, const float* pos, float* out, int B, int N,
                     int D);

int asis_rowblock_nblk(int64_t rows);
int asis_layernorm_bwd(void* stream, const float* dy, int64_t lddy, const float* x, int64_t ldx, const float* w, float eps,
                       const float* res, int64_t ldr, float* dx, int64_t lddx, float* partial, int64_t rows, int D);
int asis_gelu16(void* stream, int dtype, const void* pre, const void* dpost, void* out, int64_t n);
int asis_gelu_split(void* stream, int dtype, const float* x, void* hi, void* lo, int64_t n);
int asis_swiglu_bwd(void* stream, int dtype, const float* x12, const void* dh, void* dx12, int64_t R, int Hd);
int asis_colsum(void* stream, int dtype, const void* x, int64_t ld, float* partial, int64_t rows, int C);
int asis_cast_colsum(void* stream, int dtype, const float* x, int64_t ldx, void* out, int64_t ldo, float scale,
                     float* partial, int64_t rows, int D);
int asis_ls_linear_finish(void* stream, const float* G, const float* W, const float* bias, const float* gamma,
                          const float* cs, float grad_scale, float* dW, float* db, float* dgamma, int N, int K);

int asis_msda_fwd(void* stream, int dtype, const void* value, const float* offaw, int64_t ld_offaw, const float* ref,
                  const int32_t* shapes, const int32_t* starts, void* out, int B, int Lq, int Lin, int M, int L, int P,
                  int Dh);
int asis_msda_fwd_split(void* stream, int dtype, const void* value, const float* offaw, int64_t ld_offaw, const float* ref,
                        const int32_t* shapes, const int32_t* starts, void* out, void* out_lo, int B, int Lq, int Lin, int M,
                        int L, int P, int Dh);

int asis_dwconv_gelu(void* stream, int dtype, const float* x, const float* w9, const float* bias,
                     const int32_t* shapes, const int32_t* starts, int L, void* out, int B, int Ntok, int C);

int asis_msda_bwd(void* stream, int dtype, const void* value, const float* offaw, int64_t ld_offaw, const float* ref,
                  const int32_t* shapes, const int32_t* starts, const float* dout, float* dvalue, float* doffaw, int B,
                  int Lq, int Lin, int M, int L, int P, int Dh);
int asis_msda_vgrad_cap(int Lq, int L, int P);
int asis_msda_value_grad(void* stream, int dtype, const float* offaw, int64_t ld_offaw, const float* ref, const int32_t* shapes,
                         const int32_t* starts, const void* dout16, const float* amax, int32_t* cnt, int32_t* offs, void* rec,
                         float* dvalue, int B, int Lq, int Lin, int M, int L, int P, int Dh);
int asis_msda_sampling_matrix(void* stream, int dtype, const float* offaw, int64_t ld_offaw, const float* ref,
                              const int32_t* shapes, const int32_t* starts, void* ST, int64_t ldt, int B, int Lq, int Lin,
                              int M, int L, int P);
int asis_dwconv_bwd_nblk(int64_t rows);
int asis_dwconv_gelu_bwd(void* stream, int dtype, const float* x, const float* w9, const float* bias, const int32_t* shapes,
                         const int32_t* starts, int L, const float* dy, float* g, float* partial, void* dx, int B, int Ntok,
                         int C);

int asis_conv3x3_c3(void* stream, const float* img, const float* w, float* out, int B, int H, int W, int Cout,
                    int stride, int pad);
int asis_conv3x3_smallcout_fwd(void* stream, int dtype, const void* x_hi, const void* x_lo, const float* w,
                               const float* bias, float* out, int B, int H, int W, int Cin, int Cout);
int asis_conv3x3_smallcout_dgrad(void* stream, int dtype, const void* dy_hi, const void* dy_lo, int CoP, const float* w,
                                 float* dx, int B, int H, int W, int Cin, int Cout);

int asis_conv3x3_smallcout_fwd_up(void* stream, int dtype, const float* raw, const float* scale, const float* shift, const float* w,
                                  const float* bias, float* out, int B, int H, int W, int Cin, int Cout);
int asis_conv3x3_smallcout_wgrad_up(void* stream, int dtype, const void* dy, int CoP, const float* raw, const float* scale,
                                    const float* shift, float* slabs, int nblk, int B, int H, int W, int Cin, int Cout);

int asis_conv3x3_smallcout_wgrad(void* stream, int dtype, const void* dy, int CoP, const void* x, float* slabs, int nblk,
                                 int B, int H, int W, int Cin, int Cout);
int asis_colstats_nparts(int64_t R);
int asis_colstats(void* stream, const float* x, int64_t R, int C, float* partial);
int asis_reduce_partials(void* stream, const float* partial, int nparts, int C, double* sums);
int asis_bn_finalize(void* stream, const double* sums, double count, int C, const float* gamma, const float* beta,
                     float eps, float momentum, float* running_mean, float* running_var, int64_t* num_batches_tracked,
                     float* scale, float* shift, float* mean_out, float* invstd_out);
int asis_bn_eval_affine(void* stream, const float* gamma, const float* beta, const float* running_mean,
                        const float* running_var, float eps, int C, float* scale, float* shift);
int asis_bn_act(void* stream, int dtype, const float* x, const float* scale, const float* shift, int relu, void* out,
                void* out_lo, int64_t R, int C);
int asis_bn_act_mx(void* stream, int dtype, const float* x, const float* scale, const float* shift, int relu, void* out, void* out_mx,
                   const float* amax, int64_t R, int C);
int asis_bn_relu_maxpool(void* stream, int dtype, const float* x, const float* scale, const float* shift, void* out,
                         void* out_lo, int B, int H, int W, int C);
int asis_bn_relu_upsample(void* stream, int dtype, const float* x, const float* scale, const float* shift, void* out,
                          void* out_lo, int B, int H, int W, int C, int factor);
int asis_bn_relu_upsample_mx(void* stream, int dtype, const float* x, const float* scale, const float* shift, void* out,
                             void* out_mx, const float* amax, int B, int H, int W, int C, int factor);
int asis_pack_conv_weight(void* stream, int dtype, const float* w, void* out, int Cout, int Cin, int KH, int KW,
                          int mode, int64_t ldo, int part);
int asis_pack_conv_weight_mx(void* stream, int dtype, const float* w, void* out_mx, int Cout, int Cin, int KH, int KW,
                             int mode, int64_t ldo, const float* amax);
int asis_pack_conv_weight_pair(void* stream, int dtype, const float* w, void* out_hi, void* out_lo, int Cout, int Cin, int KH,
                               int KW, int mode, int64_t ldo, const float* amax);
int asis_decoder_input(void* stream, int dtype, const float* xs, int64_t xs_bstride, const float* c4,
                       int64_t c4_bstride, const float* vit, int64_t vit_bstride, void* out, void* out_lo, int B, int h,
                       int w, int h4, int w4, int D);
int asis_decoder_input_mx(void* stream, int dtype, const float* xs, int64_t xs_bstride, const float* c4, int64_t c4_bstride,
                          const float* vit, int64_t vit_bstride, void* out, void* out_mx, const float* amax, int B, int h,
                          int w, int h4, int w4, int D);
int asis_swiglu(void* stream, int dtype, const float* x12, void* out, int64_t R, int Hd);
int asis_swiglu_split(void* stream, int dtype, const float* x12, void* out, void* out_lo, int64_t R, int Hd);
int asis_copy_channels(void* stream, const void* src, int64_t src_ld_bytes, void* dst, int64_t dst_ld_bytes, int64_t rows,
                       int64_t row_bytes);
int asis_add_f32(void* stream, const float* a, const float* b, float* out, int64_t n, int batch, int64_t stride_a,
                 int64_t stride_b, int64_t stride_out);

int asis_maxpool2_fwd(void* stream, int dtype, const void* x, const void* x_lo, void* out, void* out_lo, uint8_t* idx,
                      int B, int H, int W, int C);
int asis_maxpool2_bwd(void* stream, const float* dy, const uint8_t* idx, float* dx, int B, int H, int W, int C);
int asis_cls_l2norm(void* stream, const float* x, float* chat, float* inv_c, int B, int N, int C, int D);
int asis_cls_l2norm_bwd(void* stream, const float* dchat, const float* chat, const float* inv_c, float* dx, int B, int N, int C,
                        int D);
int asis_mask_logits_fwd(void* stream, const float* P, const float* chat, const float* gamma, const float* beta, float eps,
                         float* logits, float* cosm, float* inv_p, int B, int N, int C, int D);
int asis_mask_logits_nblk(int B, int N);
int asis_mask_logits_bwd(void* stream, const float* dlogits, const float* cosm, const float* inv_p, const float* P,
                         const float* chat, const float* gamma, float eps, float* dP, float* dcos, float* part, int B, int N, int C,
                         int D);
int asis_mask_dchat(void* stream, const float* dcos, const float* P, const float* inv_p, float* dchat, int B, int N, int C, int D);
int asis_nearest_add_relu(void* stream, int dtype, void* x, void* x_lo, const void* r, const void* r_lo, const int* ys,
                          const int* xs, int B, int H, int W, int h, int w, int C);
int asis_nearest_sum(void* stream, const float* g, float* dr, const int* y0, const int* x0, int B, int H, int W, int h, int w,
                     int C);
int asis_convt2x2_scatter(void* stream, int dtype, const float* G, void* dst, void* dst_lo, int B, int H, int W, int Cout,
                          int H2, int W2, int Ctot, int coff, int padT, int padL);
int asis_convt2x2_gather(void* stream, int dtype, const float* dcat, void* dG, void* dG_lo, int B, int H, int W, int Cout,
                         int H2, int W2, int Ctot, int coff, int padT, int padL);
int asis_convt2x2_bias_nblk(int64_t rows);
int asis_conv1x1_dgrad_small(void* stream, int dtype, const void* d_hi, const void* d_lo, int64_t ldd, const float* w, float* dU,
                             int64_t M, int Cq, int C);
int asis_convt2x2_bias_grad(void* stream, const float* dcat, float* partial, int B, int H, int W, int Cout, int H2, int W2,
                            int Ctot, int coff, int padT, int padL);

int asis_dice_nblk(int H, int W);
int asis_seg_loss_fwd(void* stream, const float* logits, const int64_t* target, const float* ce_weight, int B, int h,
                      int w, int H, int W, int C, int n_region, int mode, float eps, int n_ce, float grad_scale,
                      float* partial, float* sums, float* loss, float* coef);
int asis_seg_loss_bwd(void* stream, const float* logits, const int64_t* target, const float* coef, const float* ce_weight,
                      int B, int h, int w, int H, int W, int C, int n_region, int mode, int n_ce, float* dz);
int asis_dice_fwd(void* stream, const float* logits, const int64_t* target, int B, int h, int w, int H, int W, int C,
                  int n_softmax, float eps, int mode, float grad_scale, float* partial, float* sums, float* loss,
                  float* coef);
int asis_ce_acc_nblk(int64_t total_pixels);
int asis_ce_acc(void* stream, const float* logits, const int64_t* target, const float* weight, int B, int h, int w,
                int H, int W, int C, float* partial);
int asis_ce_acc_counts(void* stream, const float* logits, const int64_t* target, const float* weight, int B, int h, int w,
                       int H, int W, int C, float* partial, int32_t* counts);
int asis_dice_bwd(void* stream, const float* logits, const int64_t* target, const float* coef, int B, int h, int w,
                  int H, int W, int C, int n_softmax, float* dz);
int asis_resize_bilinear_fwd(void* stream, const float* x, int B, int h, int w, int H, int W, int C, float* out);
int asis_resize_bwd_nblk(int64_t total_pixels);
int asis_resize_bilinear_bwd(void* stream, int dtype, const float* dz, int B, int H, int W, int h, int w, int C, int CP,
                             void* out, void* out_lo, float* partial);
int asis_reduce_rows(void* stream, const float* partial, int n, int K, float scale, float* out);

int asis_ew_blocks(int64_t total_chunks);
int asis_bn_bwd_nblk(int64_t rows, int C);
int asis_upsample_bn_relu_bwd(void* stream, const float* dU, const float* x, const float* scale, const float* shift,
                              const float* mean, const float* invstd, float* g, float* partial, int B, int H, int W,
                              int C, int factor);
int asis_maxpool_bn_relu_bwd(void* stream, const float* dy, const float* x, const float* scale, const float* shift,
                             const float* mean, const float* invstd, float* g, float* partial, int B, int H, int W, int C);
int asis_dilate2(void* stream, int dtype, const void* in, const void* in_lo, void* out, void* out_lo, int B, int OH, int OW,
                 int Hd, int Wd, int C);
int asis_bn_bwd_apply(void* stream, int dtype, const float* g, const float* x, const float* mean, const float* invstd,
                      const float* gamma, const float* dgamma, const float* dbeta, double count, void* out,
                      void* out_lo, float* partial, int64_t R, int C);
int asis_bn_bwd_apply_mx(void* stream, int dtype, const float* g, const float* x, const float* mean, const float* invstd,
                         const float* gamma, const float* dgamma, const float* dbeta, double count, void* out, void* out_mx,
                         const float* amax, float* partial, int64_t R, int C);
int asis_bn_bwd_absmax(void* stream, const float* g, const float* x, const float* mean, const float* invstd, const float* gamma,
                       const float* dgamma, const float* dbeta, double count, float* amax, int64_t R, int C);

typedef struct asis_wgrad_desc {
  const void* dy;
  const void* x;
  float* out;
  int64_t ld_dy;
  int64_t P;
  int32_t dtype;
  int32_t Cout, CoP, Cin;
  int32_t B_, H, W, OH, OW, KH, KW, stride, pad;
  int32_t splits;
  int64_t k_per_split;
} asis_wgrad_desc;
int asis_wgrad_splits(int64_t P, int Cout, int Ntot);
int asis_wgrad(void* stream, const asis_wgrad_desc* d);
int asis_conv3x3_wgrad_halo_nblk(int B, int H, int W, int Cin, int Cout);
int asis_conv3x3_wgrad_halo(void* stream, int dtype, const void* dy, int64_t ld_dy, const void* x, float* slabs, int nblk, int B,
                            int H, int W, int Cin, int Cout);

int asis_sgd_momentum(void* stream, float* p, const float* g, float* buf, int64_t n, float lr, float momentum,
                      float weight_decay, float inv_scale, int first_step);
int asis_augment(void* stream, const uint8_t* img, const uint8_t* mask, const int32_t* geo, const int32_t* xofs,
                 const int32_t* yofs, const int16_t* xa, const int16_t* ya, const int32_t* mx, const int32_t* my,
                 const uint8_t* lut, float* out, int64_t* mask_out, int B, int S);
int asis_augment_geo_u8(void* stream, const uint8_t* img, const uint8_t* mask, const int32_t* geo, const int32_t* xofs,
                        const int32_t* yofs, const int16_t* xa, const int16_t* ya, const int32_t* mx, const int32_t* my,
                        uint8_t* out_u8, int64_t* mask_out, int B, int S);
int asis_clahe(void* stream, const uint8_t* rgb, const int32_t* clahe, const uint16_t* tab_gamma, const uint16_t* tab_cbrt,
               const uint16_t* tab_l2yf, const int32_t* tab_ab2xz, const uint8_t* tab_invgamma, const int32_t* coef_fwd,
               const int32_t* coef_inv, uint8_t* luts, const uint8_t* lut, float* out, int B, int S, int tiles);

int asis_frame_resize(void* stream, const uint8_t* img, const uint8_t* mask, const int32_t* xspan, const int32_t* xcoef, int kx,
                      const int32_t* yspan, const int32_t* ycoef, int ky, const int32_t* ix, const int32_t* iy, const uint8_t* lut,
                      uint8_t* tmp, uint8_t* out_img, uint8_t* out_mask, int B, int Hi, int Wi, int Ho, int Wo);

int asis_predict_mask(void* stream, const float* logits, int B, int h, int w, int C, int H, int W, const uint8_t* encode,
                      uint8_t* mask, const uint8_t* frames, const uint8_t* palette, const uint8_t* alpha, uint8_t* overlay,
                      const uint8_t* target, const uint8_t* lut, int64_t* counts);

int asis_surface_stats(void* stream, const uint8_t* pred, const uint8_t* target, const uint8_t* pred_lut, const uint8_t* lut, int B,
                       int H, int W, int C, int c0, int nc, const int32_t* thr, int T, uint8_t* edges, uint16_t* g,
                       double* partial, int64_t* ints, double* sums, int32_t* d2, int d2_side);

int asis_dropout_f32(void* stream, const float* x, const float* res, float* out, int64_t n, uint64_t seed, int site, float p,
                     float alpha, const float* bias_n, int ncols);
int asis_dropout_t16(void* stream, int dtype, void* x, void* x_lo, int64_t n, uint64_t seed, int site, float p, int rescale);
int asis_dropout_mask(void* stream, uint8_t* out, int64_t n, uint64_t seed, int site, float p);
int asis_softmax_dropout_fwd(void* stream, int dtype, const float* S, void* p16, void* pd16, int64_t rows, int N, int ld, float scale,
                             uint64_t seed, int site, float p);
int asis_softmax_dropout_bwd(void* stream, int dtype, const void* p16, const void* pd16, const float* dPd, void* ds16, int64_t rows,
                             int N, int ld, float scale, uint64_t seed, int site, float p);

int asis_grad_guard(void* stream, const float* g, int64_t n, int32_t* guard, int reset);
int asis_sgd_momentum_guarded(void* stream, float* p, const float* g, float* buf, int64_t n, float lr, float momentum,
                              float weight_decay, float inv_scale, int first_step, int32_t* guard, int count_skip);
int asis_scale_f32(void* stream, float* x, int64_t n, float a);
int asis_zero(void* stream, void* p, int64_t bytes);
int asis_grad_pack_bf16(void* stream, const float* g, int64_t n, void* out);
int asis_grad_unpack_bf16(void* stream, const void* in, int64_t n, float* g);

#ifdef __cplusplus
}
#endif
#endif
```

Before: 218.0 img/s.

## Compute V-transpose for both batch segments in one segmented GEMM launch

Adds a segmented-batch mode to the 8-phase big GEMM kernel, so two groups of batch items with different column counts (e.g. different token counts) share one dense A operand and run in a single launch. Work is spread over XCD-aware slots. The attention row path uses this for the V^T projection instead of looping over segments with separate launches. The aim is fewer kernel launches and better GPU fill for small per-segment grids. In exchange it needs spare rows behind the stacked operands, adds extra index math per block, and imposes shape constraints.

```diff
diff --git a/adaptersis_amd/_lib.py b/adaptersis_amd/_lib.py
--- a/adaptersis_amd/_lib.py
+++ b/adaptersis_amd/_lib.py
@@ -34,6 +34,7 @@
         ("mx_amax_a", C.c_void_p), ("mx_amax_b", C.c_void_p),
         ("C_lo", C.c_void_p), ("rowstats", C.c_void_p), ("res16", C.c_void_p), ("res16_lo", C.c_void_p), ("ldr16", C.c_int64),
         ("ln_mr", C.c_void_p), ("ln_cs", C.c_void_p), ("ln_cols", C.c_int32),
+        ("seg_B1", C.c_int32), ("seg_N1", C.c_int32), ("seg_B2", C.c_int32), ("seg_N2", C.c_int32), ("seg_round", C.c_int32),
     ]
 
 
diff --git a/adaptersis_amd/config.py b/adaptersis_amd/config.py
--- a/adaptersis_amd/config.py
+++ b/adaptersis_amd/config.py
@@ -21,6 +21,7 @@
 encoder_stream = os.environ.get("ASIS_ENC_STREAM", "1") not in ("0", "")
 
 vt_stream = os.environ.get("ASIS_VT_STREAM", "1") not in ("0", "")
+vt_one_launch = os.environ.get("ASIS_VT_ONE_LAUNCH", "1") not in ("0", "")
 
 wgrad_stream = os.environ.get("ASIS_WGRAD_STREAM", "1") not in ("0", "")
 
diff --git a/adaptersis_amd/csrc/gemm.hip b/adaptersis_amd/csrc/gemm.hip
--- a/adaptersis_amd/csrc/gemm.hip
+++ b/adaptersis_amd/csrc/gemm.hip
@@ -188,14 +188,43 @@
 #include "gemm_p8.h"
 
 static int g_gemm_p8 = -1;
+static int g_gemm_8p = -1;
+static int ph8_rule() {
+  if (g_gemm_8p < 0) { const char* e = getenv("ASIS_GEMM_8P"); g_gemm_8p = e ? atoi(e) : 1; }
+  return g_gemm_8p;
+}
 static bool ph8_m16_on() { static const int v = [] { const char* e = getenv("ASIS_GEMM_8P_M16"); return e ? atoi(e) : 1; }(); return v != 0; }
 
 template <typename T>
 int launch(hipStream_t s, const asis_gemm_desc& d) {
   static const int group_m = [] { const char* e = getenv("ASIS_GEMM_GROUPM"); return e && atoi(e) > 0 ? atoi(e) : 4; }();
   static const int big_mode = [] { const char* e = getenv("ASIS_GEMM_BIG"); return e ? atoi(e) : 1; }();
+  static const int ph8_mink = [] { const char* e = getenv("ASIS_GEMM_8P_MINK"); return e ? atoi(e) : 1024; }();
   const bool vec_ok = (d.N % 4 == 0) && (d.ldc % 4 == 0);
   const bool split = d.A_lo != nullptr || d.B_lo != nullptr;
+  if (d.seg_B2 > 0) {
+    const int rnd = d.seg_round - 1;
+    const int n1 = (d.seg_N1 + rnd) & ~rnd, n2 = (d.seg_N2 + rnd) & ~rnd;
+    const int tm = (d.M + 255) / 256, t1 = tm * ((n1 + 255) / 256), t2 = tm * ((n2 + 255) / 256);
+    const bool lnc = d.ln_mr != nullptr;
+    const int ph8 = ph8_rule();
+    const bool ok = big_mode && ph8_m16_on() && !d.conv && !split && !d.stats && !d.aux && !d.res && !d.res16 && !d.C_lo && !d.rowstats &&
+                    !d.scale_n && !d.bias_n && d.ksplit <= 1 && (d.act == ASIS_ACT_NONE || d.act == ASIS_ACT_RELU || d.act == ASIS_ACT_GELU) &&
+                    d.K % 64 == 0 && d.M >= 256 && d.seg_N1 >= 256 && d.seg_N2 >= 256 &&
+                    (ph8 == 2 || (ph8 && d.K >= 2048) || (ph8 == 1 && d.K >= ph8_mink && (int64_t)d.seg_B1 * t1 + (int64_t)d.seg_B2 * t2 >= 128)) &&
+                    (!lnc || (d.ln_cs && d.ln_cols && n1 % 8 == 0 && n2 % 8 == 0 && d.ldc % 8 == 0 && !d.out_f32));
+    if (!ok) return ASIS_EINVAL;
+    int slots = 0;
+    for (int x = 0; x < 8; ++x) {
+      const int c1 = x < d.seg_B1 ? (d.seg_B1 - x + 7) / 8 : 0, call = x < d.batch ? (d.batch - x + 7) / 8 : 0;
+      const int s = c1 * t1 + (call - c1) * t2;
+      slots = s > slots ? s : slots;
+    }
+    dim3 grid(8 * slots), block(512);
+    if (lnc) hipLaunchKernelGGL((gemm_big_kernel<T, 2, 4, 4, 2, 2, 0, false, false, 64, 1, true, true, 1, false, true>), grid, block, 0, s, d, group_m);
+    else hipLaunchKernelGGL((gemm_big_kernel<T, 2, 4, 4, 2, 2, 0, false, false, 64, 1, true, true, 0, false, true>), grid, block, 0, s, d, group_m);
+    return 0;
+  }
   if (d.act == ASIS_ACT_GELU_GRAD) {
     const bool ok = big_mode && !d.conv && !split && !d.stats && d.aux && d.K % 32 == 0 && d.M >= 256 && d.N >= 128 && vec_ok &&
                     d.ld_aux % 4 == 0 && d.batch == 1 && (reinterpret_cast<uintptr_t>(d.aux) & 7) == 0 &&
@@ -237,7 +266,7 @@
   }
   const bool lnx = d.C_lo || d.rowstats || d.res16 || d.ln_mr;
   if (lnx) {
-    static const int ph8x = [] { const char* e = getenv("ASIS_GEMM_8P"); return e ? atoi(e) : 1; }();
+    const int ph8x = ph8_rule();
     const bool ph8_ok = ph8x && ph8_m16_on() && big_mode && !split && !d.conv && !d.stats && d.K % 64 == 0 && d.M >= 256 && d.N >= 256 &&
                         (ph8x == 2 || d.K >= 2048 || (ph8x == 1 && d.K >= 1024 && (int64_t)((d.M + 255) / 256) * ((d.N + 255) / 256) * d.batch >= 128)) &&
                         d.N % 8 == 0 && d.ldc % 8 == 0 && (!d.res16 || (d.res16_lo && d.ldr16 % 8 == 0 && d.ldr16 >= d.N && asis_aligned16(d.res16) && asis_aligned16(d.res16_lo))) &&
@@ -305,8 +334,7 @@
     return 0;
   }
   static const int m16 = [] { const char* e = getenv("ASIS_GEMM_M16"); return e ? atoi(e) : 1; }();
-  static const int ph8 = [] { const char* e = getenv("ASIS_GEMM_8P"); return e ? atoi(e) : 1; }();
-  static const int ph8_mink = [] { const char* e = getenv("ASIS_GEMM_8P_MINK"); return e ? atoi(e) : 1024; }();
+  const int ph8 = ph8_rule();
   if (ph8 && (ph8 == 2 || d.K >= 2048 || (ph8 == 1 && d.K >= ph8_mink && (int64_t)((d.M + 255) / 256) * ((d.N + 255) / 256) * d.batch >= 128)) && big_mode && !d.conv && !d.stats && d.K % 64 == 0 && d.M >= 256 && d.N >= 256) {
     dim3 grid(((d.M + 255) / 256) * ((d.N + 255) / 256), d.batch), block(512);
     static const int ph8_m16 = [] { const char* e = getenv("ASIS_GEMM_8P_M16"); return e ? atoi(e) : 1; }();
@@ -360,6 +388,7 @@
 extern "C" int asis_gemm_set_option(const char* name, int value) {
   ASIS_REQUIRE(name != nullptr, "asis_gemm_set_option: null name");
   if (strcmp(name, "p8") == 0) { g_gemm_p8 = value; return ASIS_OK; }
+  if (strcmp(name, "8p") == 0) { g_gemm_8p = value; return ASIS_OK; }
   ASIS_FAIL(ASIS_EINVAL, "asis_gemm_set_option: unknown option '%s'", name);
 }
 
@@ -368,6 +397,18 @@
   ASIS_REQUIRE(dp != nullptr, "asis_gemm: null descriptor");
   asis_gemm_desc d = *dp;
   ASIS_REQUIRE(d.A && d.B && d.C, "asis_gemm: null operand pointer");
+  if (d.seg_B1 > 0 || d.seg_B2 > 0) {
+    ASIS_REQUIRE(d.seg_B1 > 0 && d.seg_N1 > 0 && d.seg_B2 >= 0 && (d.seg_B2 == 0 || d.seg_N2 > 0), "asis_gemm: bad batch segments (%d x %d, %d x %d)",
+                 d.seg_B1, d.seg_N1, d.seg_B2, d.seg_N2);
+    ASIS_REQUIRE(d.seg_round == 1 || d.seg_round == 4 || d.seg_round == 8, "asis_gemm: seg_round must be 1, 4 or 8 (got %d)", d.seg_round);
+    ASIS_REQUIRE(!d.conv && d.strideA == 0 && d.ksplit <= 1, "asis_gemm: a segmented batch shares a dense A operand");
+    ASIS_REQUIRE((int64_t)d.seg_B1 * d.seg_N1 + (int64_t)d.seg_B2 * d.seg_N2 + 8 < (1ll << 31), "asis_gemm: too many stacked rows");
+    const int n1 = (d.seg_N1 + d.seg_round - 1) / d.seg_round * d.seg_round, n2 = (d.seg_N2 + d.seg_round - 1) / d.seg_round * d.seg_round;
+    d.batch = d.seg_B1 + d.seg_B2;
+    d.N = (d.seg_B2 > 0 && n2 > n1) ? n2 : n1;
+    d.strideB = (int64_t)d.seg_N1 * d.ldb;
+    if (d.seg_B2 == 0) d.seg_B1 = d.seg_N1 = d.seg_N2 = d.seg_round = 0;
+  }
   ASIS_REQUIRE(d.M > 0 && d.N > 0 && d.K > 0, "asis_gemm: M,N,K must be positive (got %d,%d,%d)", d.M, d.N, d.K);
   ASIS_DT_OK(d.dtype, "asis_gemm");
   ASIS_REQUIRE(d.K % 8 == 0, "asis_gemm: K=%d must be a multiple of 8", d.K);
@@ -404,6 +445,9 @@
   ASIS_REQUIRE((!d.A_lo || asis_aligned16(d.A_lo)) && (!d.B_lo || asis_aligned16(d.B_lo)), "asis_gemm: split halves must be 16-byte aligned");
   int rc = 0;
   if (int bad = asis_dispatch16(d.dtype, "asis_gemm", [&](auto t) { rc = launch<decltype(t)>(s, d); })) return bad;
+  if (rc != 0 && d.seg_B2 > 0)
+    ASIS_FAIL(ASIS_EINVAL, "asis_gemm: two batch segments need the dense 8-phase form (include/asis_hip.h: K %% 64 == 0, K >= 1024, M >= 256, "
+                           "both column counts >= 256, >= 128 tiles, bias_m / ln_mr epilogue only)");
   if (rc != 0 && d.act == ASIS_ACT_SILU_MUL)
     ASIS_FAIL(ASIS_EINVAL, "asis_gemm: ASIS_ACT_SILU_MUL needs a dense 16-bit-output launch on the 8-phase form (include/asis_hip.h: K %% 64 == 0, "
                            "M >= 256, N >= 256, N %% 32 == 0, ldc %% 8 == 0, plain or MX split operands, bias only)");
diff --git a/adaptersis_amd/csrc/gemm_big.h b/adaptersis_amd/csrc/gemm_big.h
--- a/adaptersis_amd/csrc/gemm_big.h
+++ b/adaptersis_amd/csrc/gemm_big.h
@@ -7,9 +7,10 @@
 __device__ __attribute__((aligned(16))) uint4 g_zero_page[1];
 
 template <typename T, int WM, int WN, int TM, int TN, int NS, int DBG = 0, bool CONV = false, bool SPLIT = false, int BKT = 64,
-          int OCC = 2, bool PH8 = false, bool M16 = false, int LNF = 0, bool MXC = false>
+          int OCC = 2, bool PH8 = false, bool M16 = false, int LNF = 0, bool MXC = false, bool SEG = false>
 __global__ __launch_bounds__(WM * WN * 64, OCC) void gemm_big_kernel(const asis_gemm_desc d, const int GROUP_M_FLAGS) {
   const int GROUP_M = GROUP_M_FLAGS & 0xffff;
+  static_assert(!SEG || (PH8 && M16 && !CONV && !SPLIT && !MXC), "the segmented batch is built for the dense 8-phase form");
   static_assert(!PH8 || (WM == 2 && WN == 4 && TM == 4 && TN == 2 && NS == 2 && BKT == 64),
                 "the 8-phase main loop is written for the 256x256x64 tile, 2x4 waves of 128x64");
   static_assert(!MXC || (SPLIT && M16 && BKT == 64 && (CONV || PH8)), "the MX correction pass is built for split operands on 16x16 MFMAs");
@@ -40,8 +41,32 @@
   const int wm = wid / WN, wn = wid - wm * WN;
   uint64_t dbg_c0 = 0, dbg_r0 = 0;
   if (DBG & 4) asm volatile("s_memtime %0\n\ts_memrealtime %1\n\ts_waitcnt lgkmcnt(0)" : "=s"(dbg_c0), "=s"(dbg_r0)::"memory");
-  const int tiles_n = (d.N + BN2 - 1) / BN2;
-  const int bid = xcd_remap(blockIdx.x, gridDim.x);
+  int bz = blockIdx.y, dN = d.N, seg_row0 = 0, seg_bid = 0;
+  if constexpr (SEG) {
+    const int rnd = d.seg_round - 1;
+    const int n1 = (d.seg_N1 + rnd) & ~rnd, n2 = (d.seg_N2 + rnd) & ~rnd;
+    const int tm = (d.M + BM2 - 1) / BM2;
+    const int t1 = tm * ((n1 + BN2 - 1) / BN2), t2 = tm * ((n2 + BN2 - 1) / BN2);
+    const int xcd = blockIdx.x & 7, slot = blockIdx.x >> 3;
+    const int c1 = xcd < d.seg_B1 ? (d.seg_B1 - xcd + 7) >> 3 : 0;
+    int j, t;
+    if (slot < c1 * t1) {
+      j = slot / t1;
+      t = slot - j * t1;
+    } else {
+      const int s2 = slot - c1 * t1, j2 = s2 / t2;
+      j = c1 + j2;
+      t = s2 - j2 * t2;
+    }
+    bz = __builtin_amdgcn_readfirstlane(xcd + 8 * j);
+    if (bz >= d.seg_B1 + d.seg_B2) return;
+    const bool g2 = bz >= d.seg_B1;
+    dN = __builtin_amdgcn_readfirstlane(g2 ? n2 : n1);
+    seg_row0 = __builtin_amdgcn_readfirstlane(g2 ? d.seg_B1 * d.seg_N1 + (bz - d.seg_B1) * d.seg_N2 : bz * d.seg_N1);
+    seg_bid = __builtin_amdgcn_readfirstlane(t);
+  }
+  const int tiles_n = (dN + BN2 - 1) / BN2;
+  const int bid = SEG ? seg_bid : xcd_remap(blockIdx.x, gridDim.x);
   const int tiles_m = (d.M + BM2 - 1) / BM2;
   const int band = bid / (GROUP_M * tiles_n);
   const int first_m = band * GROUP_M;
@@ -50,9 +75,8 @@
   const int tile_n = in_band / band_m;
   const int tile_m = first_m + (in_band - tile_n * band_m);
   const int m0 = tile_m * BM2, n0 = tile_n * BN2;
-  const int bz = blockIdx.y;
   const T* __restrict__ A = reinterpret_cast<const T*>(d.A) + (int64_t)bz * d.strideA;
-  const T* __restrict__ B = reinterpret_cast<const T*>(d.B) + (int64_t)bz * d.strideB;
+  const T* __restrict__ B = reinterpret_cast<const T*>(d.B) + (SEG ? (int64_t)seg_row0 * d.ldb : (int64_t)bz * d.strideB);
 
   const T* asrc[GA];
   const T* bsrc[GB];
@@ -92,7 +116,7 @@
   for (int j = 0; j < GB; ++j) {
     const int row = grp_b(j) + lr;
     int gr = n0 + row;
-    gr = gr < d.N ? gr : d.N - 1;
+    gr = gr < dN ? gr : dN - 1;
     bsrc[j] = B + (int64_t)gr * d.ldb + ((lc ^ swz(row)) << 3);
     b_off[j] = (uint32_t)(gr * (int)d.ldb + ((lc ^ swz(row)) << 3));
   }
@@ -522,36 +546,36 @@
   }
   const int64_t cbase = (int64_t)bz * d.strideC;
   const float* __restrict__ res = d.res ? d.res + (int64_t)bz * d.strideR : nullptr;
-  const bool vec = ((d.N & 3) == 0) && ((d.ldc & 3) == 0) && ((cbase & 3) == 0) && (!res || (d.ldr & 3) == 0) &&
+  const bool vec = ((dN & 3) == 0) && ((d.ldc & 3) == 0) && ((cbase & 3) == 0) && (!res || (d.ldr & 3) == 0) &&
                    ((reinterpret_cast<uintptr_t>(d.C) & 15) == 0) && (!res || (reinterpret_cast<uintptr_t>(res) & 15) == 0) &&
                    (!d.bias_n || (reinterpret_cast<uintptr_t>(d.bias_n) & 15) == 0) &&
                    (!d.scale_n || (reinterpret_cast<uintptr_t>(d.scale_n) & 15) == 0);
   if constexpr (M16 && PH8) {
     if (vec && !d.out_f32 && !res && !d.res16 && !d.C_lo && !d.rowstats && !d.stats && !d.scale_n && d.act != ASIS_ACT_GELU_GRAD && !(DBG & 8) &&
-        (d.N & 7) == 0 && (d.ldc & 7) == 0 && (cbase & 7) == 0 && !(GROUP_M_FLAGS >> 16)) {
+        (dN & 7) == 0 && (d.ldc & 7) == 0 && (cbase & 7) == 0 && !(GROUP_M_FLAGS >> 16)) {
       constexpr int SW16 = TN * 32 + 8;
       __syncthreads();
       T* slab16 = reinterpret_cast<T*>(lds) + wid * (32 * SW16);
       const int r16 = lane & 15, q16 = lane >> 4;
       const int rr8 = lane >> 3, c8 = lane & 7;
       const bool ln_on = LNF != 0 && !CONV && d.ln_mr != nullptr, ln_c = ln_on && d.ln_cols != 0;
-      const float2* const mrp = reinterpret_cast<const float2*>(d.ln_mr) + (ln_c ? (int64_t)bz * (d.strideB / d.ldb) : 0);
+      const float2* const mrp = reinterpret_cast<const float2*>(d.ln_mr) + (ln_c ? (SEG ? (int64_t)seg_row0 : (int64_t)bz * (d.strideB / d.ldb)) : 0);
       float4 bj[TN * 2], cj[TN * 2];
       float2 mc[TN * 2][4];
 #pragma unroll
       for (int j = 0; j < TN * 2; ++j) {
         const int colj = n0 + (wn * TN * 2 + j) * 16 + 4 * q16;
-        bj[j] = (d.bias_n && kt_base == 0 && colj < d.N) ? *reinterpret_cast<const float4*>(d.bias_n + colj) : make_float4(0.f, 0.f, 0.f, 0.f);
-        cj[j] = (ln_on && !ln_c && colj < d.N) ? *reinterpret_cast<const float4*>(d.ln_cs + colj) : make_float4(0.f, 0.f, 0.f, 0.f);
+        bj[j] = (d.bias_n && kt_base == 0 && colj < dN) ? *reinterpret_cast<const float4*>(d.bias_n + colj) : make_float4(0.f, 0.f, 0.f, 0.f);
+        cj[j] = (ln_on && !ln_c && colj < dN) ? *reinterpret_cast<const float4*>(d.ln_cs + colj) : make_float4(0.f, 0.f, 0.f, 0.f);
 #pragma unroll
         for (int e = 0; e < 4; ++e) {
           mc[j][e] = make_float2(0.f, 1.f);
-          if (ln_c) mc[j][e] = mrp[colj + e < d.N ? colj + e : d.N - 1];
+          if (ln_c) mc[j][e] = mrp[colj + e < dN ? colj + e : dN - 1];
         }
       }
       const bool sg = d.act == ASIS_ACT_SILU_MUL;
       const int colr = sg ? (n0 >> 1) + wn * TN * 16 + (lane & 3) * 8 : n0 + wn * TN * 32 + c8 * 8;
-      const bool cokr = colr < (sg ? (d.N >> 1) : d.N);
+      const bool cokr = colr < (sg ? (dN >> 1) : dN);
       T* const Cw = reinterpret_cast<T*>(d.C) + cbase + colr;
 #pragma unroll
       for (int i = 0; i < TM; ++i) {
@@ -724,7 +748,7 @@
     float* slab = reinterpret_cast<float*>(lds) + wid * (32 * SW);
     const int rr = lane / LPR, ch = lane - rr * LPR;
     const int col = n0 + wn * TN * 32 + ch * 4;
-    const bool cok = col < d.N;
+    const bool cok = col < dN;
     float4 b4 = make_float4(0.f, 0.f, 0.f, 0.f), s4 = make_float4(1.f, 1.f, 1.f, 1.f);
     if (cok && d.bias_n && kt_base == 0) b4 = *reinterpret_cast<const float4*>(d.bias_n + col);
     if (cok && d.scale_n) s4 = *reinterpret_cast<const float4*>(d.scale_n + col);
@@ -865,7 +889,7 @@
 #pragma unroll
         for (int e = 0; e < 4; ++e) {
           const int c = n0 + (wn * TN * 2 + j) * 16 + 4 * (lane >> 4) + e;
-          if (c < d.N) scalar_out(row, c, acc16[i][j][e], bmv);
+          if (c < dN) scalar_out(row, c, acc16[i][j][e], bmv);
         }
     }
     return;
@@ -880,11 +904,11 @@
 #pragma unroll
       for (int g = 0; g < 4; ++g) {
         const int col = n0 + (wn * TN + j) * 32 + 8 * g + 4 * fh;
-        if (!rok || col >= d.N) continue;
+        if (!rok || col >= dN) continue;
 #pragma unroll
         for (int e = 0; e < 4; ++e) {
           const int c = col + e;
-          if (c < d.N) {
+          if (c < dN) {
             float x = acc[i][j][4 * g + e] + (d.bias_n ? d.bias_n[c] : 0.f) + bmv;
             if (d.act == ASIS_ACT_GELU) x = gelu_erf(x);
             else if (d.act == ASIS_ACT_RELU) x = fmaxf(x, 0.f);
diff --git a/adaptersis_amd/dinov2/layers/blocks.py b/adaptersis_amd/dinov2/layers/blocks.py
--- a/adaptersis_amd/dinov2/layers/blocks.py
+++ b/adaptersis_amd/dinov2/layers/blocks.py
@@ -256,7 +256,15 @@
             else:
                 qk = ops.gemm(xn, w[: 2 * D], bias_n=bias[: 2 * D], ln=(mr, cs[: 2 * D], False))
             r0 = b0 = 0
-            for B, N in segs:
+            if one_launch and config.vt_one_launch and ops.gemm_seg_supported(D, D, *segs[0], *segs[1], 8):
+                if spare < (-segs[1][1] % 8) * D:
+                    raise ValueError("attend_rows(ln=...): the hi plane needs 8 spare rows behind it")
+                with (torch.cuda.stream(side) if side is not None else contextlib.nullcontext()):
+                    ops.gemm(w[2 * D:], xn, out=vt_all, bias_m=bias[2 * D:], ln=(mr, cs[2 * D:], True), seg=(*segs[0], *segs[1], 8))
+                r0, segs_vt = xn.shape[0], ()
+            else:
+                segs_vt = segs
+            for B, N in segs_vt:
                 r1 = r0 + B * N
                 vt = vt_all[b0:b0 + B]
                 N4 = (N + 7) // 8 * 8
@@ -307,7 +315,13 @@
         else:
             qk = ops.gemm(xn, w[: 2 * D], bias_n=None if bias is None else bias[: 2 * D], b_lo=None if wlo is None else wlo[: 2 * D])
         r0 = b0 = 0
-        for B, N in segs:
+        segs_vt = segs
+        if (one_launch and config.vt_one_launch and wlo is None and spare >= 4 * D and xn.is_cuda
+                and ops.gemm_seg_supported(D, D, *segs[0], *segs[1], 4)):
+            with (torch.cuda.stream(side) if side is not None else contextlib.nullcontext()):
+                ops.gemm(w[2 * D:], xn, out=vt_all, bias_m=None if bias is None else bias[2 * D:], seg=(*segs[0], *segs[1], 4))
+            r0, segs_vt = xn.shape[0], ()
+        for B, N in segs_vt:
             r1 = r0 + B * N
             ldvt = ldv_all if one_launch else (N + 63) // 64 * 64
             vt = vt_all[b0:b0 + B] if one_launch else torch.empty((B, D, ldvt), device=xn.device, dtype=xn.dtype)
diff --git a/adaptersis_amd/ops.py b/adaptersis_amd/ops.py
--- a/adaptersis_amd/ops.py
+++ b/adaptersis_amd/ops.py
@@ -61,7 +61,8 @@
                scale_n: Optional[torch.Tensor] = None, res: Optional[torch.Tensor] = None, act: int = ACT_NONE,
                stats: Optional[torch.Tensor] = None, a_lo: Optional[torch.Tensor] = None,
                b_lo: Optional[torch.Tensor] = None, aux: Optional[torch.Tensor] = None,
-               out_lo: Optional[torch.Tensor] = None, rowstats: Optional[torch.Tensor] = None, res16=None, ln=None, mx=None):
+               out_lo: Optional[torch.Tensor] = None, rowstats: Optional[torch.Tensor] = None, res16=None, ln=None, mx=None,
+               seg=None):
     _dev(a, b, out, bias_n, bias_m, scale_n, res, stats, out_lo, rowstats)
     if a.dtype != b.dtype:
         raise ValueError("gemm operands must have the same 16-bit dtype")
@@ -70,6 +71,20 @@
         batch = a.shape[0] if a.dim() == 3 else b.shape[0]
     M, K = a.shape[-2], a.shape[-1]
     N = b.shape[-2]
+    seg_cols = None
+    if seg is not None:
+        B1, N1, B2, N2, rnd = (int(v) for v in seg)
+        if a.dim() != 2 or b.dim() != 2 or out is None or out.dim() != 3 or rnd not in (1, 4, 8) or B1 < 1 or B2 < 0 or N1 < 1 or (B2 and N2 < 1):
+            raise ValueError("gemm(seg=): a [M, K] and the stacked b [rows, K] are 2-D, out is [B1 + B2, M, cols]")
+        n1, n2 = (N1 + rnd - 1) // rnd * rnd, ((N2 + rnd - 1) // rnd * rnd if B2 else 0)
+        last = (n2 - N2) if B2 else (n1 - N1)
+        have = b.untyped_storage().nbytes() // b.element_size() - b.storage_offset()
+        if b.shape[0] < B1 * N1 + B2 * N2 or have < (B1 * N1 + B2 * N2 + last - 1) * b.stride(0) + K:
+            raise ValueError(f"gemm(seg=): b needs {B1 * N1 + B2 * N2} rows and {last} spare rows behind them")
+        batch, N = B1 + B2, max(n1, n2)
+        if out.shape[0] != batch or out.shape[-1] < N:
+            raise ValueError("gemm(seg=): out must be [B1 + B2, M, >= the rounded column count]")
+        seg_cols = B1 * n1 + B2 * n2
     if b.shape[-1] != K:
         raise ValueError(f"gemm: inner dims differ: a[...,{K}] vs b[...,{b.shape[-1]}]")
     if a.stride(-1) != 1 or b.stride(-1) != 1:
@@ -82,7 +97,7 @@
         out = torch.empty(shape, device=a.device, dtype=torch.float32 if out_f32 else a.dtype)
     else:
         out_f32 = out.dtype == torch.float32
-        if out.stride(-1) != 1 or out.shape[-1] != n_out:
+        if out.stride(-1) != 1 or (out.shape[-1] != n_out and seg is None):
             raise ValueError("gemm: out must be contiguous in its last dim, one column per output feature")
     d = GemmDesc()
     d.A, d.B, d.C = a.data_ptr(), b.data_ptr(), out.data_ptr()
@@ -104,6 +119,10 @@
             raise ValueError("gemm: aux must be a 16-bit [M, N] matrix of the operand dtype")
         d.aux, d.ld_aux = aux.data_ptr(), aux.stride(-2)
     flops = 2.0 * batch * M * N * K
+    if seg is not None:
+        d.seg_B1, d.seg_N1, d.seg_B2, d.seg_N2, d.seg_round = B1, N1, B2, N2, rnd
+        d.strideB = 0
+        flops = 2.0 * M * seg_cols * K
     if (a_lo is None) != (b_lo is None) and not (K % 64 == 0 and M >= 256 and N >= 32 and N % 4 == 0 and out.stride(-2) % 4 == 0):
         a_lo = b_lo = None
     if a_lo is not None:
@@ -136,10 +155,24 @@
     if ln is not None:
         mr, cs, cols = ln
         _dev(mr, cs)
+        if seg is not None and not cols:
+            raise ValueError("gemm(seg=): the LayerNorm statistics follow the stacked rows of b (ln = (mr, cs, True))")
+        if seg is not None and mr.untyped_storage().nbytes() // 4 - mr.storage_offset() < 2 * (B1 * N1 + B2 * N2 + last):
+            raise ValueError(f"gemm(seg=): mr needs {last} spare rows behind the stacked rows, like b")
         d.ln_mr, d.ln_cs, d.ln_cols = _f32c(mr).data_ptr(), _f32c(cs).data_ptr(), int(bool(cols))
     nbytes = batch * (2.0 * (M * K + N * K) + M * N * ((4 if (out_f32 or out_lo is not None) else 2) +
                                                     (4 if (res is not None or res16 is not None) else 0)))
+    if seg is not None:
+        nbytes = 2.0 * (batch * M * K + seg_cols * K) + M * seg_cols * (4 if out_f32 else 2)
     return d, out, flops, nbytes
+
+
+def gemm_seg_supported(M: int, K: int, B1: int, N1: int, B2: int, N2: int, rnd: int) -> bool:
+    if M < 256 or min(N1, N2) < 256 or K % 64 or B1 < 1 or B2 < 1:
+        return False
+    tm = (M + 255) // 256
+    tiles = sum(B * tm * (((N + rnd - 1) // rnd * rnd + 255) // 256) for B, N in ((B1, N1), (B2, N2)))
+    return K >= 2048 or (K >= 1024 and tiles >= 128)
 
 
 def gemm(a: torch.Tensor, b: torch.Tensor, **kw) -> torch.Tensor:
diff --git a/include/asis_hip.h b/include/asis_hip.h
--- a/include/asis_hip.h
+++ b/include/asis_hip.h
@@ -59,6 +59,7 @@
   const float* ln_mr;
   const float* ln_cs;
   int32_t ln_cols;
+  int32_t seg_B1, seg_N1, seg_B2, seg_N2, seg_round;
 } asis_gemm_desc;
 int asis_ln_stats_finalize(void* stream, const float* rowstats, int64_t rows, int groups, int D, float eps, float* mr);
 int asis_split_stats(void* stream, int dtype, const float* x, int64_t ldx, void* hi, void* lo, int64_t ld16, float* mr,
```

New measurement: 218.3 img/s, median of 6. Within noise of the previous version (+0.1%).
